# SamsungLabs/fcaf3d

Hardware: AMD Instinct MI355X
Metric: scenes/sec fwd+bwd, ScanNet 100k-pt 2cm voxels, 1/2/4/8 MI355X (higher is better)
Workload: dtype f32

## Files before the change

fcaf3d_amd/_lib.py:

```python
import ctypes
import os
import re
import threading
import time

import torch

_HERE = os.path.dirname(os.path.abspath(__file__))
LIB_PATH = os.environ.get('FC_LIB') or os.path.join(_HERE, 'libfcaf3d_hip.so')
HEADER = os.path.join(os.path.dirname(_HERE), 'include', 'fcaf3d_hip.h')

_SCALARS = {'int': ctypes.c_int, 'int64_t': ctypes.c_int64, 'float': ctypes.c_float,
            'hipStream_t': ctypes.c_void_p}


def parse_header(path=HEADER):
    txt = open(path).read()
    txt = re.sub(r'/\*.*?\*/', '', txt, flags=re.S)
    protos = {}
    for m in re.finditer(r'\b(int64_t|int)\s+(fc_\w+)\s*\(([^)]*)\)\s*;', txt):
        ret, name, args = m.group(1), m.group(2), m.group(3)
        argl = []
        for a in args.split(','):
            a = ' '.join(a.split())
            if not a or a == 'void':
                continue
            if '*' in a:
                argl.append((a.split('*')[-1].strip(), ctypes.c_void_p))
            else:
                ty, nm = a.rsplit(' ', 1)
                argl.append((nm, _SCALARS[ty.replace('const ', '')]))
        protos[name] = (_SCALARS[ret], argl)
    return protos


ABI_VERSION = 8
_lib = None
_protos = None


def lib():
    global _lib, _protos
    if _lib is None:
        if not os.path.exists(LIB_PATH):
            raise RuntimeError(
                f'{LIB_PATH} is missing: build it with `python -m fcaf3d_amd.build` '
                '(hipcc --offload-arch=gfx950).  There is no CPU fallback.')
        l = ctypes.CDLL(LIB_PATH)
        _protos = parse_header()
        for name, (ret, args) in _protos.items():
            fn = getattr(l, name)
            fn.restype = ret
            fn.argtypes = [t for _, t in args]
        if l.fc_abi_version() != ABI_VERSION:
            raise RuntimeError(f'{LIB_PATH} speaks ABI version {l.fc_abi_version()}, this host code was written for {ABI_VERSION}: rebuild '
                               'with `python -m fcaf3d_amd.build`')
        _lib = l
    return _lib


def ptr(t):
    if t is None:
        return None
    assert t.is_contiguous(), 'C ABI takes contiguous buffers'
    return t.data_ptr()


_raw_stream = getattr(torch._C, '_cuda_getCurrentRawStream', None)


def stream():
    if _raw_stream is not None:
        return _raw_stream(torch.cuda.current_device())
    return torch.cuda.current_stream().cuda_stream


_fns = {}


def call(name, *args):
    fn = _fns.get(name)
    if fn is None:
        fn = _fns[name] = getattr(lib(), name)
    rc = fn(*args)
    if rc != 0:
        kind = 'invalid argument' if rc == -1 else 'workspace too small' if rc == -2 else f'hipError {rc}'
        raise RuntimeError(f'{name} failed: {kind}')


_query_cache = {}


def query(name, *args):
    key = (name,) + args
    v = _query_cache.get(key)
    if v is None:
        if len(_query_cache) > 65536:
            _query_cache.clear()
        v = _query_cache[key] = int(getattr(lib(), name)(*args))
    return v


_ws_cache = {}


def workspace(nbytes, device):
    key = (device, stream())
    buf = _ws_cache.get(key)
    if buf is None or buf.numel() < nbytes:
        buf = torch.empty(max(int(nbytes), 1 << 20), dtype=torch.uint8, device=device)
        _ws_cache[key] = buf
    return buf


HOST_WAIT = [0.0]


class _PinnedRing:

    def __init__(self, n=16):
        self.bufs, self.evts, self.i = [None] * n, [None] * n, 0
        self.lock = threading.Lock()

    def upload(self, arr, device):
        with self.lock:
            i = self.i
            self.i = (i + 1) % len(self.bufs)
        if self.evts[i] is not None and not self.evts[i].query():
            t0 = time.perf_counter()
            self.evts[i].synchronize()
            HOST_WAIT[0] += time.perf_counter() - t0
        nb = max(int(arr.nbytes), 1)
        if self.bufs[i] is None or self.bufs[i].numel() < nb:
            self.bufs[i] = torch.empty(max(nb, 4096), dtype=torch.uint8).pin_memory()
        src = torch.from_numpy(arr)
        stage = self.bufs[i][:arr.nbytes].view(src.dtype).reshape(src.shape)
        stage.copy_(src)
        out = stage.to(device, non_blocking=True)
        e = torch.cuda.Event()
        e.record(torch.cuda.current_stream(out.device))
        self.evts[i] = e
        return out


_ring = _PinnedRing()


def upload(arr, device):
    return _ring.upload(arr, device)
```

fcaf3d_amd/csrc/exec.hip:

```cpp
#include "fc_common.h"
#include "../../include/fcaf3d_hip.h"
#include <vector>

namespace {

enum : int64_t {
  OP_STEM_FWD = 1, OP_COL_STATS, OP_NORM_FWD, OP_MAXPOOL_FWD, OP_CONV, OP_BN_FWD, OP_UNION_FWD, OP_HEAD_FWD, OP_RECORD, OP_WAIT,
  OP_HEAD_BWD, OP_WGRAD, OP_BN_BWD, OP_NORM_BWD, OP_MAXPOOL_BWD, OP_STEM_WGRAD, OP_GATHER, OP_ADD, OP_SMALL_GRADS,
  OP_PERMUTE_GENT, OP_HEAD_WFIN, OP_COPY, OP_COL_SUM, OP_ROW_SUM, OP_AMAX, OP_CLEAR
};
constexpr int OPW = 24;
constexpr int MAPW = 20;
constexpr int NSTREAM = 3;
constexpr int MAX_EVENTS = 64;

constexpr int MAX_DEVICES = 16;
hipEvent_t g_events_dev[MAX_DEVICES][MAX_EVENTS];
bool g_events_ready[MAX_DEVICES] = {};
thread_local hipEvent_t* g_events = nullptr;

int ensure_events() {
  int dev = 0;
  FC_HIP(hipGetDevice(&dev));
  if (dev < 0 || dev >= MAX_DEVICES) return FC_EINVAL;
  if (!g_events_ready[dev]) {
    for (int i = 0; i < MAX_EVENTS; ++i) FC_HIP(hipEventCreateWithFlags(&g_events_dev[dev][i], hipEventDisableTiming));
    g_events_ready[dev] = true;
  }
  g_events = g_events_dev[dev];
  return 0;
}

struct ProbeRec { hipEvent_t a, b; int64_t meta[8]; };
std::vector<ProbeRec> g_probe;
std::vector<hipEvent_t> g_probe_pool;

hipEvent_t probe_event() {
  if (!g_probe_pool.empty()) { hipEvent_t e = g_probe_pool.back(); g_probe_pool.pop_back(); return e; }
  hipEvent_t e = nullptr;
  if (hipEventCreate(&e) != hipSuccess) return nullptr;
  return e;
}

inline double as_double(int64_t v) { double d; __builtin_memcpy(&d, &v, 8); return d; }

__global__ void k_add_inplace(float* __restrict__ dst, const float* __restrict__ src, int64_t n4) {
  const int64_t t = (int64_t)blockIdx.x * blockDim.x + threadIdx.x;
  if (t >= n4) return;
  float4 a = reinterpret_cast<float4*>(dst)[t];
  const float4 b = reinterpret_cast<const float4*>(src)[t];
  a.x += b.x; a.y += b.y; a.z += b.z; a.w += b.w;
  reinterpret_cast<float4*>(dst)[t] = a;
}

__global__ void k_small_grads(const long long* __restrict__ desc, int n) {
  const int e = blockIdx.x;
  if (e >= n) return;
  const long long* d = desc + 8 * e;
  const float* src = reinterpret_cast<const float*>(d[0]);
  float* dst = reinterpret_cast<float*>(d[1]);
  const int C = (int)d[2], nseg = (int)d[3];
  const long long stride = d[4];
  for (int c = threadIdx.x; c < C; c += blockDim.x) {
    float s = 0.f;
    for (int k = 0; k < nseg; ++k) s += fc_ld(src + k * stride + c);
    dst[c] = s;
  }
}

__global__ void k_permute_gent(const float* __restrict__ src, float* __restrict__ dst, int Cin, int Cout) {
  const int64_t t = (int64_t)blockIdx.x * blockDim.x + threadIdx.x;
  const int64_t total = (int64_t)8 * Cin * Cout;
  if (t >= total) return;
  const int d = (int)(t % Cout), c = (int)((t / Cout) % Cin), k = (int)(t / ((int64_t)Cout * Cin));
  dst[t] = src[(int64_t)c * 8 * Cout + (int64_t)k * Cout + d];
}

__global__ void k_head_wfin(const float* __restrict__ part, int nl, int R, int ld, int n_reg, int n_cls, float* __restrict__ g_cent,
                            float* __restrict__ g_reg, float* __restrict__ g_cls, const float* __restrict__ bias_part,
                            float* __restrict__ g_bias) {
  const int t = blockIdx.x * blockDim.x + threadIdx.x;
  const int ncol = 1 + n_reg + n_cls;
  if (g_bias && t < n_cls) {
    float b = 0.f;
    for (int l = 0; l < nl; ++l) b += fc_ld(&bias_part[l * n_cls + t]);
    g_bias[t] = b;
  }
  if (t >= R * ncol) return;
  const int r = t / ncol, c = t % ncol;
  float s = 0.f;
  for (int l = 0; l < nl; ++l) s += part[((int64_t)l * R + r) * ld + c];
  if (c == 0) g_cent[r] = s;
  else if (c <= n_reg) g_reg[r * n_reg + c - 1] = s;
  else g_cls[r * n_cls + c - 1 - n_reg] = s;
}

__global__ __launch_bounds__(1024) void k_col_sum(const float* __restrict__ x, int64_t n, int C, float* __restrict__ dst) {
  __shared__ float red[1024];
  const int c = blockIdx.x;
  float a0 = 0.f, a1 = 0.f, a2 = 0.f, a3 = 0.f;
  int64_t r = threadIdx.x;
  for (; r + 3 * 1024 < n; r += 4 * 1024) {
    a0 += x[r * C + c]; a1 += x[(r + 1024) * C + c]; a2 += x[(r + 2048) * C + c]; a3 += x[(r + 3072) * C + c];
  }
  for (; r < n; r += 1024) a0 += x[r * C + c];
  red[threadIdx.x] = (a0 + a1) + (a2 + a3);
  __syncthreads();
  for (int w = 512; w > 0; w >>= 1) {
    if ((int)threadIdx.x < w) red[threadIdx.x] += red[threadIdx.x + w];
    __syncthreads();
  }
  if (threadIdx.x == 0) dst[c] = red[0];
}

struct Ctx {
  const int64_t* ops;
  const int64_t* addr;
  const int64_t* dims;
  const int64_t* maps;
  hipStream_t streams[NSTREAM];
  void* ws[NSTREAM];
  int64_t ws_bytes[NSTREAM];
  int64_t need[NSTREAM];
  bool dry;
  bool probe;
  int64_t bn_small_elems;
  int flags;
};

int run_op_impl(Ctx& c, const int64_t* op);

int run_op(Ctx& c, const int64_t* op) {
  if (c.dry || !c.probe || (op[0] != OP_CONV && op[0] != OP_AMAX)) return run_op_impl(c, op);
  ProbeRec r;
  r.a = probe_event(); r.b = probe_event();
  if (!r.a || !r.b) return run_op_impl(c, op);
  hipStream_t st = c.streams[op[1]];
  const int64_t Cin = op[8], Cout = op[9];
  if (op[0] == OP_AMAX) {
    const int64_t m[8] = {-2, 0, c.dims[op[3]], 0, 0, op[4], 0, 0};
    __builtin_memcpy(r.meta, m, sizeof m);
  } else if (op[4] < 0) {
    const int64_t n = c.dims[op[7]];
    const int64_t m[8] = {-1, op[5], n, n, 1, Cin, Cout, 0};
    __builtin_memcpy(r.meta, m, sizeof m);
  } else {
    const int64_t* mp = c.maps + op[4] * MAPW;
    const bool bwd = op[5] != 0;
    const int64_t m[8] = {op[4], op[5], bwd ? mp[1] : mp[0], bwd ? mp[0] : mp[1], mp[2], Cin, Cout, (mp[19] & (bwd ? 2 : 1)) ? 1 : 0};
    __builtin_memcpy(r.meta, m, sizeof m);
  }
  FC_HIP(hipEventRecord(r.a, st));
  const int rc = run_op_impl(c, op);
  FC_HIP(hipEventRecord(r.b, st));
  g_probe.push_back(r);
  return rc;
}

template <class T>
inline T* P(const Ctx& c, int64_t idx) { return idx < 0 ? nullptr : reinterpret_cast<T*>(c.addr[idx]); }

int64_t stats_blocks_of(const Ctx& c, const int64_t* pop) {
  const int Cin = (int)pop[8], Cout = (int)pop[9];
  const int fl = c.flags | FC_CONV_SPLIT | FC_CONV_IMAGE;
  if (pop[4] < 0) return fc_conv_stats_blocks(c.dims[pop[7]], 1, Cin, Cout, fl, 0);
  const int64_t* m = c.maps + pop[4] * MAPW;
  const bool bwd = pop[5] != 0;
  return fc_conv_stats_blocks(bwd ? m[0] : m[1], (int)m[2], Cin, Cout, fl, (m[19] & (bwd ? 2 : 1)) ? 1 : 0);
}

inline bool want_ws(Ctx& c, int s, int64_t bytes) {
  if (bytes > c.need[s]) c.need[s] = bytes;
  return !c.dry;
}

int run_op_impl(Ctx& c, const int64_t* op) {
  const int s = (int)op[1];
  hipStream_t st = c.streams[s];
#ifdef FC_KO_EXEC
  {
    static const int ko = getenv("FC_KO_OPS") ? atoi(getenv("FC_KO_OPS")) : 0;
    const int64_t o = op[0];
    if (!c.dry && (((ko & 1) && (o == OP_WGRAD || o == OP_STEM_WGRAD)) || ((ko & 2) && o == OP_CONV) ||
                   ((ko & 4) && (o == OP_BN_FWD || o == OP_BN_BWD || o == OP_NORM_FWD || o == OP_NORM_BWD || o == OP_COL_STATS))))
      return 0;
  }
#endif
  switch (op[0]) {
    case OP_STEM_FWD: {
      const int64_t* m = c.maps + op[4] * MAPW;
      if (c.dry) return 0;
      return fc_stem_conv_fwd(P<const float>(c, op[2]), P<const float>(c, op[3]), reinterpret_cast<const int*>(m[3]), P<float>(c, op[5]),
                              P<float>(c, op[6]), m[0], m[1], (int)m[2], st);
    }
    case OP_COL_STATS: {
      const int64_t n = c.dims[op[4]];
      const int C = (int)op[5], nseg = (int)c.dims[op[6]];
      if (!want_ws(c, s, fc_col_stats_ws_bytes(n, C, nseg))) return 0;
      return fc_col_stats(P<const float>(c, op[2]), P<const int>(c, op[3]), op[3] >= 0 ? 4 : 0, n, C, nseg, P<float>(c, op[7]),
                          P<float>(c, op[8]), P<float>(c, op[9]), c.ws[s], c.ws_bytes[s], st);
    }
    case OP_NORM_FWD: {
      if (c.dry) return 0;
      return fc_norm_act_fwd(P<const float>(c, op[2]), P<const int>(c, op[3]), op[3] >= 0 ? 4 : 0, c.dims[op[4]], (int)op[5],
                             P<const float>(c, op[6]), P<const float>(c, op[7]), (float)as_double(op[8]), P<const float>(c, op[9]),
                             P<const float>(c, op[10]), P<const float>(c, op[11]), (int)op[12], P<float>(c, op[13]), st);
    }
    case OP_MAXPOOL_FWD: {
      const int64_t* m = c.maps + op[3] * MAPW;
      if (c.dry) return 0;
      if (op[7] > 0) fc_amax_out_hint(P<unsigned>(c, op[7] - 1));
      return fc_maxpool_fwd(P<const float>(c, op[2]), reinterpret_cast<const int*>(m[3]), m[1], (int)m[2], (int)op[4], P<float>(c, op[5]),
                            P<int>(c, op[6]), st);
    }
    case OP_CONV: {
      const int Cin = (int)op[8], Cout = (int)op[9];
      const int fl = c.flags | FC_CONV_SPLIT | FC_CONV_IMAGE;
      float* stats = (op[10] > 0 && stats_blocks_of(c, op) > 0) ? P<float>(c, op[10] - 1) : nullptr;
      const float* bnx = (stats && op[11] > 0) ? P<const float>(c, op[11] - 1) : nullptr;
      const float *bmean = P<const float>(c, op[12]), *bvar = P<const float>(c, op[13]), *bga = P<const float>(c, op[14]),
                  *bbe = P<const float>(c, op[15]);
      const float beps = (float)as_double(op[16]);
      const int bact = (int)op[17];
      const float* badd = op[18] > 0 ? P<const float>(c, op[18] - 1) : nullptr;
      const float* bny = op[19] > 0 ? P<const float>(c, op[19] - 1) : nullptr;
      const float* in = P<const float>(c, op[2]);
      const float* img = P<const float>(c, op[3]);
      float* out = P<float>(c, op[6]);
      if (!c.dry && op[20] > 0) fc_conv_amax_hint(P<const unsigned>(c, op[20] - 1), nullptr);
      if (op[4] < 0) {
        const int64_t n = c.dims[op[7]];
        if (!want_ws(c, s, fc_conv_fwd_ws_bytes(n, 1, Cin, Cout, fl))) return 0;
        if (bnx)
          return fc_conv_fwd_bn_bwd_stats(in, img, nullptr, nullptr, out, n, n, 1, Cin, Cout, fl, c.ws[s], c.ws_bytes[s], stats, bnx, bmean, bvar,
                                          bga, bbe, beps, bact, badd, bny, st);
        return fc_conv_fwd_stats(in, img, nullptr, nullptr, out, n, n, 1, Cin, Cout, fl, c.ws[s], c.ws_bytes[s], stats, st);
      }
      const int64_t* m = c.maps + op[4] * MAPW;
      const bool bwd = op[5] != 0;
      const int64_t n_in = bwd ? m[1] : m[0], n_out = bwd ? m[0] : m[1];
      const int K = (int)m[2];
      if (m[19] & (bwd ? 2 : 1)) {
        const int b = bwd ? 14 : 9;
        const int *pi = reinterpret_cast<const int*>(m[b]), *pc = reinterpret_cast<const int*>(m[b + 3]),
                  *pp = reinterpret_cast<const int*>(m[b + 2]);
        if (!want_ws(c, s, fc_conv_fwd_pairs_ws_bytes(n_out, K, Cout))) return 0;
        if (bnx)
          return fc_conv_fwd_pairs_tiles_bn_bwd_stats(in, img, pi, pc, pp, out, n_in, n_out, K, Cin, Cout, m[b + 4], fl, c.ws[s], c.ws_bytes[s],
                                                      stats, bnx, bmean, bvar, bga, bbe, beps, bact, badd, bny, st);
        return fc_conv_fwd_pairs_tiles_stats(in, img, pi, pc, pp, out, n_in, n_out, K, Cin, Cout, m[b + 4], fl, c.ws[s], c.ws_bytes[s], stats,
                                             st);
      }
      const int *tab = reinterpret_cast<const int*>(m[bwd ? 7 : 5]), *oidx = reinterpret_cast<const int*>(m[bwd ? 8 : 6]);
      if (!want_ws(c, s, fc_conv_fwd_ws_bytes(n_out, K, Cin, Cout, fl))) return 0;
      if (bnx)
        return fc_conv_fwd_bn_bwd_stats(in, img, tab, oidx, out, n_in, n_out, K, Cin, Cout, fl, c.ws[s], c.ws_bytes[s], stats, bnx, bmean, bvar,
                                        bga, bbe, beps, bact, badd, bny, st);
      return fc_conv_fwd_stats(in, img, tab, oidx, out, n_in, n_out, K, Cin, Cout, fl, c.ws[s], c.ws_bytes[s], stats, st);
    }
    case OP_BN_FWD: {
      const int64_t n = c.dims[op[3]];
      const int C = (int)op[4];
      const float eps = (float)as_double(op[5]), mom = (float)as_double(op[10]);
      if (!op[18]) {
        if (c.dry) return 0;
        if (op[21] > 0) fc_amax_out_hint(P<unsigned>(c, op[21] - 1));
        return fc_norm_act_fwd(P<const float>(c, op[2]), nullptr, 0, n, C, P<const float>(c, op[15]), P<const float>(c, op[16]), eps,
                               P<const float>(c, op[6]), P<const float>(c, op[7]), P<const float>(c, op[8]), (int)op[9], P<float>(c, op[11]),
                               st);
      }
      const float* part = nullptr;
      int64_t nbp = 0;
      if (op[19] > 0) {
        const int64_t* pop = c.ops + (op[19] - 1) * OPW;
        nbp = pop[10] > 0 ? stats_blocks_of(c, pop) : 0;
        if (nbp > 0) part = P<const float>(c, pop[10] - 1);
      }
      if (!want_ws(c, s, fc_bn_train_ws_bytes(n, C))) return 0;
      if (op[21] > 0) fc_amax_out_hint(P<unsigned>(c, op[21] - 1));
      return fc_bn_train_fwd(P<const float>(c, op[2]), n, C, eps, P<const float>(c, op[6]), P<const float>(c, op[7]),
                             P<const float>(c, op[8]), (int)op[9], mom, P<float>(c, op[11]), P<float>(c, op[12]), P<float>(c, op[13]),
                             P<float>(c, op[14]), P<float>(c, op[15]), P<float>(c, op[16]), P<long long>(c, op[17]), part, nbp,
                             op[20] > 0 ? (int)op[20] : 1, c.bn_small_elems, c.ws[s], c.ws_bytes[s], st);
    }
    case OP_UNION_FWD: {
      if (c.dry) return 0;
      const int64_t n_a = c.dims[op[5]], n_b = c.dims[op[6]], n_u = c.dims[op[7]];
      const int C = (int)op[8];
      float* out = P<float>(c, op[9]);
      FC_HIP(hipMemcpyAsync(out, P<const float>(c, op[2]), sizeof(float) * n_a * C, hipMemcpyDeviceToDevice, st));
      if (n_u > n_a) FC_HIP(hipMemsetAsync(out + n_a * C, 0, sizeof(float) * (n_u - n_a) * C, st));
      return fc_scatter_rows_add(P<const float>(c, op[3]), P<const int>(c, op[4]), n_b, C, out, st);
    }
    case OP_HEAD_FWD: {
      if (c.dry) return 0;
      return fc_head_split_fwd(P<const float>(c, op[2]), (int)op[3], P<const float>(c, op[4]), P<const float>(c, op[5]), c.dims[op[6]],
                               (int)op[7], (int)op[8], P<float>(c, op[9]), P<float>(c, op[10]), P<float>(c, op[11]), P<float>(c, op[12]), st);
    }
    case OP_RECORD:
      if (c.dry) return 0;
      FC_HIP(hipEventRecord(g_events[op[2]], st));
      return 0;
    case OP_WAIT:
      if (c.dry) return 0;
      FC_HIP(hipStreamWaitEvent(st, g_events[op[2]], 0));
      return 0;
    case OP_HEAD_BWD: {
      if (op[13] < 0) {
        const int64_t n = c.dims[op[9]];
        if (!want_ws(c, s, fc_head_split_bwd_sums_ws_bytes(n))) return 0;
        if (op[16] > 0) fc_amax_out_hint(P<unsigned>(c, op[16] - 1));
        return fc_head_split_bwd_sums(P<const float>(c, op[2]), (int)op[3], P<const float>(c, op[4]), P<const float>(c, op[5]),
                                      P<const float>(c, op[6]), P<const float>(c, op[7]), P<const float>(c, op[8]), n, (int)op[10],
                                      (int)op[11], P<float>(c, op[12]), P<float>(c, op[15]), P<float>(c, op[14]), c.ws[s],
                                      c.ws_bytes[s], st);
      }
      if (c.dry) return 0;
      return fc_head_split_bwd(P<const float>(c, op[2]), (int)op[3], P<const float>(c, op[4]), P<const float>(c, op[5]),
                               P<const float>(c, op[6]), P<const float>(c, op[7]), P<const float>(c, op[8]), c.dims[op[9]], (int)op[10],
                               (int)op[11], P<float>(c, op[12]), P<float>(c, op[13]), st);
    }
    case OP_WGRAD: {
      const int Cin = (int)op[7], Cout = (int)op[8];
      const int fl = c.flags | FC_CONV_SPLIT;
      if (!c.dry && (op[9] > 0 || op[10] > 0))
        fc_conv_amax_hint(op[9] > 0 ? P<const unsigned>(c, op[9] - 1) : nullptr, op[10] > 0 ? P<const unsigned>(c, op[10] - 1) : nullptr);
      if (op[4] < 0) {
        const int64_t n = c.dims[op[6]];
        if (!want_ws(c, s, fc_conv_wgrad_ws_bytes(n, 1, Cin, Cout, fl))) return 0;
        return fc_conv_wgrad(P<const float>(c, op[2]), P<const float>(c, op[3]), nullptr, nullptr, P<float>(c, op[5]), n, n, 1, Cin, Cout, fl,
                             c.ws[s], c.ws_bytes[s], st);
      }
      const int64_t* m = c.maps + op[4] * MAPW;
      const int K = (int)m[2];
      if (!want_ws(c, s, fc_conv_wgrad_ws_bytes(m[1], K, Cin, Cout, fl))) return 0;
      if ((m[19] & 4) && Cin % 64 == 0 && Cout % 64 == 0)
        return fc_conv_wgrad_pairs(P<const float>(c, op[2]), P<const float>(c, op[3]), reinterpret_cast<const int*>(m[9]),
                                   reinterpret_cast<const int*>(m[10]), reinterpret_cast<const int*>(m[12]), P<float>(c, op[5]), m[0], m[1],
                                   K, Cin, Cout, fl, c.ws[s], c.ws_bytes[s], st);
      return fc_conv_wgrad(P<const float>(c, op[2]), P<const float>(c, op[3]), reinterpret_cast<const int*>(m[3]), nullptr,
                           P<float>(c, op[5]), m[0], m[1], K, Cin, Cout, fl, c.ws[s], c.ws_bytes[s], st);
    }
    case OP_BN_BWD: {
      const int64_t n = c.dims[op[5]];
      const int C = (int)op[6];
      const float eps = (float)as_double(op[10]);
      const float* part = nullptr;
      int64_t nbp = 0;
      if (op[18] > 0) {
        const int64_t* pop = c.ops + (op[18] - 1) * OPW;
        nbp = (pop[10] > 0 && pop[11] > 0) ? stats_blocks_of(c, pop) : 0;
        if (nbp > 0) part = P<const float>(c, pop[10] - 1);
      }
      if (!want_ws(c, s, fc_bn_train_ws_bytes(n, C))) return 0;
      if (op[19] > 0) fc_amax_out_hint(P<unsigned>(c, op[19] - 1));
      return fc_bn_train_bwd(P<const float>(c, op[2]), P<const float>(c, op[3]), P<const float>(c, op[4]),
                             op[17] > 0 ? P<const float>(c, op[17] - 1) : nullptr, n, C, P<const float>(c, op[7]), P<const float>(c, op[8]),
                             P<const float>(c, op[9]), eps, P<const float>(c, op[11]), P<const float>(c, op[12]), (int)op[13],
                             P<float>(c, op[14]), P<float>(c, op[15]), P<float>(c, op[16]), part, nbp, c.bn_small_elems, c.ws[s],
                             c.ws_bytes[s], st);
    }
    case OP_NORM_BWD: {
      const int64_t n = c.dims[op[6]];
      const int C = (int)op[7], nseg = (int)c.dims[op[8]];
      if (!want_ws(c, s, fc_norm_act_bwd_ws_bytes(n, C, nseg))) return 0;
      return fc_norm_act_bwd(P<const float>(c, op[2]), P<const float>(c, op[3]), P<const float>(c, op[4]), P<const int>(c, op[5]),
                             op[5] >= 0 ? 4 : 0, n, C, nseg, P<const float>(c, op[9]), P<const float>(c, op[10]), P<const float>(c, op[11]),
                             (float)as_double(op[12]), P<const float>(c, op[13]), P<const float>(c, op[14]), (int)op[15], P<float>(c, op[16]),
                             P<float>(c, op[17]), P<float>(c, op[18]), c.ws[s], c.ws_bytes[s], st);
    }
    case OP_MAXPOOL_BWD: {
      const int64_t* m = c.maps + op[4] * MAPW;
      if (c.dry) return 0;
      const int C = (int)op[5];
      FC_HIP(hipMemsetAsync(P<float>(c, op[6]), 0, sizeof(float) * m[0] * C, st));
      return fc_maxpool_bwd(P<const float>(c, op[2]), P<const int>(c, op[3]), m[1], C, P<float>(c, op[6]), st);
    }
    case OP_STEM_WGRAD: {
      const int64_t* m = c.maps + op[4] * MAPW;
      if (!want_ws(c, s, fc_stem_conv_wgrad_ws_bytes(m[1], (int)m[2]))) return 0;
      return fc_stem_conv_wgrad(P<const float>(c, op[2]), P<const float>(c, op[3]), P<float>(c, op[5]), m[1], (int)m[2], c.ws[s],
                                c.ws_bytes[s], st);
    }
    case OP_GATHER: {
      if (c.dry) return 0;
      return fc_gather_rows(P<const float>(c, op[2]), P<const int>(c, op[3]), c.dims[op[4]], (int)op[5], P<float>(c, op[6]), st);
    }
    case OP_ADD: {
      if (c.dry) return 0;
      const int64_t n4 = c.dims[op[4]] * op[5] / 4;
      if (n4 > 0) k_add_inplace<<<(unsigned)fc_cdiv(n4, 256), 256, 0, st>>>(P<float>(c, op[2]), P<const float>(c, op[3]), n4);
      FC_CHECK_LAUNCH();
      return 0;
    }
    case OP_SMALL_GRADS: {
      if (c.dry) return 0;
      if (op[4] > 0) k_small_grads<<<(unsigned)op[4], 128, 0, st>>>(P<const long long>(c, op[2]) + 8 * op[3], (int)op[4]);
      FC_CHECK_LAUNCH();
      return 0;
    }
    case OP_COL_SUM: {
      if (c.dry) return 0;
      k_col_sum<<<(unsigned)op[4], 1024, 0, st>>>(P<const float>(c, op[2]), c.dims[op[3]], (int)op[4], P<float>(c, op[5]));
      FC_CHECK_LAUNCH();
      return 0;
    }
    case OP_ROW_SUM: {
      if (c.dry) return 0;
      k_col_sum<<<1, 1024, 0, st>>>(P<const float>(c, op[2]), c.dims[op[3]], 1, P<float>(c, op[4]));
      FC_CHECK_LAUNCH();
      return 0;
    }
    case OP_PERMUTE_GENT: {
      if (c.dry) return 0;
      const int64_t total = 8 * op[4] * op[5];
      k_permute_gent<<<(unsigned)fc_cdiv(total, 256), 256, 0, st>>>(P<const float>(c, op[2]), P<float>(c, op[3]), (int)op[4], (int)op[5]);
      FC_CHECK_LAUNCH();
      return 0;
    }
    case OP_HEAD_WFIN: {
      if (c.dry) return 0;
      const int total = (int)(op[4] * (1 + op[6] + op[7]));
      k_head_wfin<<<(unsigned)fc_cdiv(total, 256), 256, 0, st>>>(P<const float>(c, op[2]), (int)op[3], (int)op[4], (int)op[5], (int)op[6],
                                                                 (int)op[7], P<float>(c, op[8]), P<float>(c, op[9]), P<float>(c, op[10]),
                                                                 P<const float>(c, op[11]), P<float>(c, op[12]));
      FC_CHECK_LAUNCH();
      return 0;
    }
    case OP_AMAX: {
      if (c.dry) return 0;
      return fc_amax(P<const float>(c, op[2]), c.dims[op[3]] * op[4], P<unsigned>(c, op[5]), st);
    }
    case OP_CLEAR: {
      if (c.dry) return 0;
      FC_HIP(hipMemsetAsync(P<void>(c, op[2]), 0, (size_t)op[3], st));
      return 0;
    }
    case OP_COPY: {
      if (c.dry) return 0;
      FC_HIP(hipMemcpyAsync(P<float>(c, op[2]), P<const float>(c, op[3]), sizeof(float) * c.dims[op[4]] * op[5], hipMemcpyDeviceToDevice, st));
      return 0;
    }
    default:
      return FC_EINVAL;
  }
}

}

extern "C" {

int fc_exec_op_words(void) { return OPW; }
int fc_exec_map_words(void) { return MAPW; }

int fc_exec(const int64_t* ops, int64_t op_begin, int64_t op_end, const int64_t* addr, const int64_t* dims, const int64_t* maps,
            const int64_t* streams, const int64_t* ws, const int64_t* ws_bytes, int64_t* ws_need, const int64_t* cfg) {
  if (!ops || op_begin < 0 || op_end < op_begin) return FC_EINVAL;
  int rc = ensure_events();
  if (rc) return rc;
  Ctx c;
  c.ops = ops;
  c.addr = addr; c.dims = dims; c.maps = maps;
  for (int i = 0; i < NSTREAM; ++i) {
    c.streams[i] = reinterpret_cast<hipStream_t>(streams[i]);
    c.ws[i] = reinterpret_cast<void*>(ws[i]);
    c.ws_bytes[i] = ws_bytes[i];
    c.need[i] = 0;
  }
  c.bn_small_elems = cfg[0];
  c.flags = (int)cfg[1];
  c.probe = cfg[2] != 0;
  c.dry = true;
  for (int64_t i = op_begin; i < op_end; ++i) {
    rc = run_op(c, ops + i * OPW);
    if (rc) return rc;
  }
  bool ok = true;
  for (int i = 0; i < NSTREAM; ++i) {
    if (ws_need) ws_need[i] = c.need[i];
    if (c.need[i] > c.ws_bytes[i]) ok = false;
  }
  if (!ok) return FC_EWS;
  if (cfg[3]) return 0;
  c.dry = false;
  for (int64_t i = op_begin; i < op_end; ++i) {
    rc = run_op(c, ops + i * OPW);
    if (rc) return rc;
  }
  return 0;
}

int64_t fc_exec_probe_read(float* ms, int64_t* meta, int64_t cap) {
  const int64_t n = (int64_t)g_probe.size();
  for (int64_t i = 0; i < n; ++i) {
    ProbeRec& r = g_probe[i];
    if (i < cap) {
      float t = 0.f;
      if (hipEventElapsedTime(&t, r.a, r.b) != hipSuccess) t = -1.f;
      ms[i] = t;
      __builtin_memcpy(meta + 8 * i, r.meta, sizeof r.meta);
    }
    g_probe_pool.push_back(r.a);
    g_probe_pool.push_back(r.b);
  }
  g_probe.clear();
  return n;
}

}
```

fcaf3d_amd/csrc/norm.hip:

```cpp
#include "fc_common.h"
#include "../../include/fcaf3d_hip.h"

#define MAXSEG 64
#define MAXBLOCKS 1024

__device__ static inline int seg_of(const int* seg, int seg_stride, int64_t row) {
  return seg ? seg[row * seg_stride] : 0;
}

__device__ static inline void seg_range(const int* seg, int seg_stride, int64_t r0, int64_t r1, int* lo, int* hi,
                                        int* sh ) {
  if (!seg) { *lo = 0; *hi = 0; return; }
  if (threadIdx.x == 0) { sh[0] = 0x7fffffff; sh[1] = -1; }
  __syncthreads();
  int l = 0x7fffffff, h = -1;
  for (int64_t r = r0 + threadIdx.x; r < r1; r += blockDim.x) {
    int s = seg[r * seg_stride];
    l = s < l ? s : l;
    h = s > h ? s : h;
  }
  if (h >= 0) { atomicMin(&sh[0], l); atomicMax(&sh[1], h); }
  __syncthreads();
  *lo = sh[0]; *hi = sh[1];
  __syncthreads();
}

__global__ void k_stats_partial(const float* __restrict__ x, const int* __restrict__ seg, int seg_stride, int64_t n, int C,
                                int nseg, const float* __restrict__ mean, int mode, int64_t rpb, float* __restrict__ part,
                                float* __restrict__ part_cnt) {
  extern __shared__ float sm[];
  __shared__ int srange[2];
  const int c4n = C / 4;
  const int cl = threadIdx.x % c4n, rl = threadIdx.x / c4n;
  const int nrl = blockDim.x / c4n;
  const int64_t r0 = (int64_t)blockIdx.x * rpb;
  int64_t r1 = r0 + rpb;
  if (r1 > n) r1 = n;
  int s_lo, s_hi;
  seg_range(seg, seg_stride, r0, r1, &s_lo, &s_hi, srange);
  const bool chk = seg && s_lo != s_hi;
  for (int s = 0; s < nseg; ++s) {
    float4 acc[4];
    float4 sq = make_float4(0.f, 0.f, 0.f, 0.f);
    float cnt = 0.f;
#pragma unroll
    for (int u = 0; u < 4; ++u) acc[u] = make_float4(0.f, 0.f, 0.f, 0.f);
    if (s >= s_lo && s <= s_hi) {
      float4 mu = make_float4(0.f, 0.f, 0.f, 0.f);
      if (mode == 1) mu = *reinterpret_cast<const float4*>(mean + (int64_t)s * C + cl * 4);
      for (int64_t rb = r0 + rl; rb < r1; rb += 4 * nrl) {
        float4 vv[4];
        bool ok[4];
#pragma unroll
        for (int u = 0; u < 4; ++u) {
          const int64_t r = rb + (int64_t)u * nrl;
          ok[u] = r < r1;
          const int64_t rc = ok[u] ? r : r0;
          if (chk) ok[u] = ok[u] && seg[rc * seg_stride] == s;
          vv[u] = *reinterpret_cast<const float4*>(x + rc * C + cl * 4);
        }
#pragma unroll
        for (int u = 0; u < 4; ++u) {
          if (!ok[u]) continue;
          float4 v = vv[u];
          if (mode == 1) {
            v.x -= mu.x; v.y -= mu.y; v.z -= mu.z; v.w -= mu.w;
            v.x *= v.x; v.y *= v.y; v.z *= v.z; v.w *= v.w;
          }
          if (mode == 2) { sq.x += v.x * v.x; sq.y += v.y * v.y; sq.z += v.z * v.z; sq.w += v.w * v.w; }
          acc[u].x += v.x; acc[u].y += v.y; acc[u].z += v.z; acc[u].w += v.w;
          cnt += 1.f;
        }
      }
    }
    float4 a;
    a.x = (acc[0].x + acc[1].x) + (acc[2].x + acc[3].x);
    a.y = (acc[0].y + acc[1].y) + (acc[2].y + acc[3].y);
    a.z = (acc[0].z + acc[1].z) + (acc[2].z + acc[3].z);
    a.w = (acc[0].w + acc[1].w) + (acc[2].w + acc[3].w);
    __syncthreads();
    *reinterpret_cast<float4*>(&sm[(rl * c4n + cl) * 4]) = a;
    float* smc = sm + nrl * C;
    if (cl == 0) smc[rl] = cnt;
    __syncthreads();
    const int64_t slot = (int64_t)blockIdx.x * nseg + s;
    float* dst = mode == 2 ? part + slot * 2 * C : part + slot * C;
    if (rl == 0) {
      float4 t = make_float4(0.f, 0.f, 0.f, 0.f);
      for (int j = 0; j < nrl; ++j) {
        float4 u = *reinterpret_cast<const float4*>(&sm[(j * c4n + cl) * 4]);
        t.x += u.x; t.y += u.y; t.z += u.z; t.w += u.w;
      }
      *reinterpret_cast<float4*>(dst + cl * 4) = t;
      if (cl == 0 && part_cnt) {
        float c = 0.f;
        for (int j = 0; j < nrl; ++j) c += smc[j];
        part_cnt[slot] = c;
      }
    }
    if (mode == 2) {
      __syncthreads();
      *reinterpret_cast<float4*>(&sm[(rl * c4n + cl) * 4]) = sq;
      __syncthreads();
      if (rl == 0) {
        float4 t = make_float4(0.f, 0.f, 0.f, 0.f);
        for (int j = 0; j < nrl; ++j) {
          float4 u = *reinterpret_cast<const float4*>(&sm[(j * c4n + cl) * 4]);
          t.x += u.x; t.y += u.y; t.z += u.z; t.w += u.w;
        }
        *reinterpret_cast<float4*>(dst + C + cl * 4) = t;
      }
    }
  }
}

__global__ __launch_bounds__(256) void k_seg_meanvar_final(const float* __restrict__ part, const float* __restrict__ part_cnt,
                                                           int64_t nblocks, int nseg, int C, float* __restrict__ mean,
                                                           float* __restrict__ var, float* __restrict__ cnt_out) {
  __shared__ double r1[64][5], r2[64][5], rc[64];
  const int cgroups = (C + 3) / 4;
  const int s = blockIdx.x / cgroups, cg = blockIdx.x % cgroups;
  const int cl = threadIdx.x & 3, j = threadIdx.x >> 2;
  const int c = cg * 4 + cl;
  double a1 = 0., a2 = 0., ac = 0.;
  if (c < C) {
    for (int64_t b = j; b < nblocks; b += 64) {
      const float* src = part + ((b * nseg + s) * 2) * C;
      a1 += fc_ld(&src[c]);
      a2 += fc_ld(&src[C + c]);
      if (cl == 0) ac += fc_ld(&part_cnt[b * nseg + s]);
    }
  }
  r1[j][cl] = a1; r2[j][cl] = a2;
  if (cl == 0) rc[j] = ac;
  __syncthreads();
  if (j == 0 && c < C) {
    double s1 = 0., s2 = 0., n = 0.;
    for (int q = 0; q < 64; ++q) { s1 += r1[q][cl]; s2 += r2[q][cl]; n += rc[q]; }
    double m = 0., v = 0.;
    if (n > 0.) {
      m = s1 / n;
      v = s2 / n - m * m;
      if (v < 0.) v = 0.;
    }
    mean[(int64_t)s * C + c] = (float)m;
    var[(int64_t)s * C + c] = (float)v;
    if (c == 0) cnt_out[s] = (float)n;
  }
}

#define FIN_CB 4
#define FIN_SL 64
__global__ __launch_bounds__(256) void k_stats_final(const float* __restrict__ part, const float* __restrict__ part_cnt,
                                                      int64_t nblocks, int nseg, int C, int mode, float* __restrict__ out,
                                                      float* __restrict__ cnt_io) {
  __shared__ float red[FIN_SL][FIN_CB + 1];
  __shared__ float redc[FIN_SL];
  const int cgroups = (C + FIN_CB - 1) / FIN_CB;
  const int s = blockIdx.x / cgroups, cg = blockIdx.x % cgroups;
  const int cl = threadIdx.x & (FIN_CB - 1), j = threadIdx.x / FIN_CB;
  const int c = cg * FIN_CB + cl;
  float a0 = 0.f, a1 = 0.f, a2 = 0.f, a3 = 0.f;
  if (c < C) {
    int64_t b = j;
    for (; b + 3 * FIN_SL < nblocks; b += 4 * FIN_SL) {
      const float v0 = fc_ld(&part[(b * nseg + s) * C + c]), v1 = fc_ld(&part[((b + FIN_SL) * nseg + s) * C + c]);
      const float v2 = fc_ld(&part[((b + 2 * FIN_SL) * nseg + s) * C + c]), v3 = fc_ld(&part[((b + 3 * FIN_SL) * nseg + s) * C + c]);
      a0 += v0; a1 += v1; a2 += v2; a3 += v3;
    }
    for (; b < nblocks; b += FIN_SL) a0 += fc_ld(&part[(b * nseg + s) * C + c]);
  }
  float acc = (a0 + a1) + (a2 + a3);
  red[j][cl] = acc;
  if (mode == 0 && cl == 0) {
    float cc = 0.f;
    for (int64_t b = j; b < nblocks; b += FIN_SL) cc += fc_ld(&part_cnt[b * nseg + s]);
    redc[j] = cc;
  }
  __syncthreads();
  if (j == 0 && c < C) {
    float t = 0.f;
    for (int q = 0; q < FIN_SL; ++q) t += red[q][cl];
    float cnt = 1.f;
    if (mode == 0) {
      float cc = 0.f;
      for (int q = 0; q < FIN_SL; ++q) cc += redc[q];
      if (c == 0) cnt_io[s] = cc;
      cnt = cc;
    } else if (mode == 1) {
      cnt = cnt_io[s];
    }
    out[(int64_t)s * C + c] = (mode == 2) ? t : (cnt > 0.f ? t / cnt : 0.f);
  }
}

__device__ static inline float act_fwd(float v, int act) {
  if (act == 1) return v > 0.f ? v : 0.f;
  if (act == 2) return v > 0.f ? v : expm1f(v);
  return v;
}
__device__ static inline float act_bwd_from_y(float y, int act) {
  if (act == 1) return y > 0.f ? 1.f : 0.f;
  if (act == 2) return y > 0.f ? 1.f : y + 1.f;
  return 1.f;
}

__device__ static inline float bn_pre(float v, float mu, float is, float g, float b) { return fmaf((v - mu) * is, g, b); }
__device__ static inline float act_bwd_from_pre(float p, int act) {
  if (act == 1) return p > 0.f ? 1.f : 0.f;
  if (act == 2) return p > 0.f ? 1.f : expf(p);
  return 1.f;
}

thread_local unsigned* t_fc_amax_out = nullptr;

__global__ void k_norm_act_fwd(const float* __restrict__ x, const int* __restrict__ seg, int seg_stride, int64_t n, int C,
                               const float* __restrict__ mean, const float* __restrict__ var, float eps,
                               const float* __restrict__ gamma, const float* __restrict__ beta,
                               const float* __restrict__ residual, int act, float* __restrict__ y, unsigned* __restrict__ amax_out) {
  int64_t t = (int64_t)blockIdx.x * blockDim.x + threadIdx.x;
  const int c4n = C / 4;
  unsigned am = 0u;
  if (t < n * c4n) {
  int64_t r = t / c4n;
  int c = (int)(t % c4n) * 4;
  int s = seg_of(seg, seg_stride, r);
  float4 v = *reinterpret_cast<const float4*>(x + r * C + c);
  float4 mu = *reinterpret_cast<const float4*>(mean + (int64_t)s * C + c);
  float4 va = *reinterpret_cast<const float4*>(var + (int64_t)s * C + c);
  float4 g = gamma ? *reinterpret_cast<const float4*>(gamma + c) : make_float4(1.f, 1.f, 1.f, 1.f);
  float4 b = beta ? *reinterpret_cast<const float4*>(beta + c) : make_float4(0.f, 0.f, 0.f, 0.f);
  float4 o;
  o.x = bn_pre(v.x, mu.x, 1.f / sqrtf(va.x + eps), g.x, b.x);
  o.y = bn_pre(v.y, mu.y, 1.f / sqrtf(va.y + eps), g.y, b.y);
  o.z = bn_pre(v.z, mu.z, 1.f / sqrtf(va.z + eps), g.z, b.z);
  o.w = bn_pre(v.w, mu.w, 1.f / sqrtf(va.w + eps), g.w, b.w);
  if (residual) {
    float4 rs = *reinterpret_cast<const float4*>(residual + r * C + c);
    o.x += rs.x; o.y += rs.y; o.z += rs.z; o.w += rs.w;
  }
  o.x = act_fwd(o.x, act); o.y = act_fwd(o.y, act); o.z = act_fwd(o.z, act); o.w = act_fwd(o.w, act);
  *reinterpret_cast<float4*>(y + r * C + c) = o;
  amax_fold(am, o.x); amax_fold(am, o.y); amax_fold(am, o.z); amax_fold(am, o.w);
  }
  if (amax_out) amax_commit(am, amax_out);
}

__global__ void k_norm_bwd_partial(const float* __restrict__ x, const float* __restrict__ y, const float* __restrict__ gy,
                                   const float* __restrict__ gy2, const int* __restrict__ seg, int seg_stride, int64_t n, int C, int nseg,
                                   const float* __restrict__ mean, const float* __restrict__ var, float eps, int act,
                                   const float* __restrict__ gamma, const float* __restrict__ beta,
                                   int64_t rpb, float* __restrict__ part) {
  extern __shared__ float sm[];
  __shared__ int srange[2];
  const int c4n = C / 4;
  const int cl = threadIdx.x % c4n, rl = threadIdx.x / c4n;
  const int nrl = blockDim.x / c4n;
  const int64_t r0 = (int64_t)blockIdx.x * rpb;
  int64_t r1 = r0 + rpb;
  if (r1 > n) r1 = n;
  int s_lo, s_hi;
  seg_range(seg, seg_stride, r0, r1, &s_lo, &s_hi, srange);
  const bool chk = seg && s_lo != s_hi;
  for (int s = 0; s < nseg; ++s) {
    float4 a1[4], a2[4];
#pragma unroll
    for (int u = 0; u < 4; ++u) { a1[u] = make_float4(0.f, 0.f, 0.f, 0.f); a2[u] = a1[u]; }
    if (s >= s_lo && s <= s_hi) {
      float4 mu = *reinterpret_cast<const float4*>(mean + (int64_t)s * C + cl * 4);
      float4 va = *reinterpret_cast<const float4*>(var + (int64_t)s * C + cl * 4);
      float4 is = make_float4(1.f / sqrtf(va.x + eps), 1.f / sqrtf(va.y + eps), 1.f / sqrtf(va.z + eps),
                              1.f / sqrtf(va.w + eps));
      const float4 gm = gamma ? *reinterpret_cast<const float4*>(gamma + cl * 4) : make_float4(1.f, 1.f, 1.f, 1.f);
      const float4 bt = beta ? *reinterpret_cast<const float4*>(beta + cl * 4) : make_float4(0.f, 0.f, 0.f, 0.f);
      const bool from_y = act && y;
      for (int64_t rb = r0 + rl; rb < r1; rb += 4 * nrl) {
        float4 xv[4], gv[4], yv[4], g2[4];
        bool ok[4];
#pragma unroll
        for (int u = 0; u < 4; ++u) {
          const int64_t r = rb + (int64_t)u * nrl;
          ok[u] = r < r1;
          const int64_t rc = ok[u] ? r : r0;
          if (chk) ok[u] = ok[u] && seg[rc * seg_stride] == s;
          xv[u] = *reinterpret_cast<const float4*>(x + rc * C + cl * 4);
          gv[u] = *reinterpret_cast<const float4*>(gy + rc * C + cl * 4);
          if (gy2) g2[u] = *reinterpret_cast<const float4*>(gy2 + rc * C + cl * 4);
          if (from_y) yv[u] = *reinterpret_cast<const float4*>(y + rc * C + cl * 4);
        }
#pragma unroll
        for (int u = 0; u < 4; ++u) {
          if (!ok[u]) continue;
          float4 g = gv[u];
          if (gy2) { g.x += g2[u].x; g.y += g2[u].y; g.z += g2[u].z; g.w += g2[u].w; }
          if (from_y) {
            g.x *= act_bwd_from_y(yv[u].x, act); g.y *= act_bwd_from_y(yv[u].y, act);
            g.z *= act_bwd_from_y(yv[u].z, act); g.w *= act_bwd_from_y(yv[u].w, act);
          } else if (act) {
            g.x *= act_bwd_from_pre(bn_pre(xv[u].x, mu.x, is.x, gm.x, bt.x), act);
            g.y *= act_bwd_from_pre(bn_pre(xv[u].y, mu.y, is.y, gm.y, bt.y), act);
            g.z *= act_bwd_from_pre(bn_pre(xv[u].z, mu.z, is.z, gm.z, bt.z), act);
            g.w *= act_bwd_from_pre(bn_pre(xv[u].w, mu.w, is.w, gm.w, bt.w), act);
          }
          a1[u].x += g.x; a1[u].y += g.y; a1[u].z += g.z; a1[u].w += g.w;
          a2[u].x += g.x * (xv[u].x - mu.x) * is.x; a2[u].y += g.y * (xv[u].y - mu.y) * is.y;
          a2[u].z += g.z * (xv[u].z - mu.z) * is.z; a2[u].w += g.w * (xv[u].w - mu.w) * is.w;
        }
      }
    }
    float4 b1 = make_float4((a1[0].x + a1[1].x) + (a1[2].x + a1[3].x), (a1[0].y + a1[1].y) + (a1[2].y + a1[3].y),
                            (a1[0].z + a1[1].z) + (a1[2].z + a1[3].z), (a1[0].w + a1[1].w) + (a1[2].w + a1[3].w));
    float4 b2 = make_float4((a2[0].x + a2[1].x) + (a2[2].x + a2[3].x), (a2[0].y + a2[1].y) + (a2[2].y + a2[3].y),
                            (a2[0].z + a2[1].z) + (a2[2].z + a2[3].z), (a2[0].w + a2[1].w) + (a2[2].w + a2[3].w));
    __syncthreads();
    *reinterpret_cast<float4*>(&sm[(rl * 2 + 0) * C + cl * 4]) = b1;
    *reinterpret_cast<float4*>(&sm[(rl * 2 + 1) * C + cl * 4]) = b2;
    __syncthreads();
    if (rl == 0) {
      float4 t1 = make_float4(0.f, 0.f, 0.f, 0.f), t2 = t1;
      for (int j = 0; j < nrl; ++j) {
        float4 u = *reinterpret_cast<const float4*>(&sm[(j * 2 + 0) * C + cl * 4]);
        float4 w = *reinterpret_cast<const float4*>(&sm[(j * 2 + 1) * C + cl * 4]);
        t1.x += u.x; t1.y += u.y; t1.z += u.z; t1.w += u.w;
        t2.x += w.x; t2.y += w.y; t2.z += w.z; t2.w += w.w;
      }
      float* dst = part + (((int64_t)blockIdx.x * nseg + s) * 2) * C;
      *reinterpret_cast<float4*>(dst + cl * 4) = t1;
      *reinterpret_cast<float4*>(dst + C + cl * 4) = t2;
    }
  }
}

__global__ void k_norm_bwd_apply(const float* __restrict__ x, const float* __restrict__ y, const float* __restrict__ gy,
                                 const float* __restrict__ gy2, const int* __restrict__ seg, int seg_stride, int64_t n, int C,
                                 const float* __restrict__ mean, const float* __restrict__ var, float eps,
                                 const float* __restrict__ gamma, const float* __restrict__ beta,
                                 const float* __restrict__ sums ,
                                 const float* __restrict__ cnt, int act, float* __restrict__ gx, float* __restrict__ gres,
                                 unsigned* __restrict__ amax_out) {
  int64_t t = (int64_t)blockIdx.x * blockDim.x + threadIdx.x;
  const int c4n = C / 4;
  unsigned am = 0u;
  if (t < n * c4n) {
  int64_t r = t / c4n;
  int c = (int)(t % c4n) * 4;
  int s = seg_of(seg, seg_stride, r);
  float inv_n = 1.f / cnt[s];
  float xv[4], gv[4], muv[4], vav[4], gam[4], bet[4] = {0.f, 0.f, 0.f, 0.f}, s1[4], s2[4], yv[4], o[4], gr[4];
  *reinterpret_cast<float4*>(xv) = *reinterpret_cast<const float4*>(x + r * C + c);
  *reinterpret_cast<float4*>(gv) = *reinterpret_cast<const float4*>(gy + r * C + c);
  if (gy2) {
    const float4 t2 = *reinterpret_cast<const float4*>(gy2 + r * C + c);
    gv[0] += t2.x; gv[1] += t2.y; gv[2] += t2.z; gv[3] += t2.w;
  }
  *reinterpret_cast<float4*>(muv) = *reinterpret_cast<const float4*>(mean + (int64_t)s * C + c);
  *reinterpret_cast<float4*>(vav) = *reinterpret_cast<const float4*>(var + (int64_t)s * C + c);
  *reinterpret_cast<float4*>(s1) = *reinterpret_cast<const float4*>(sums + ((int64_t)s * 2) * C + c);
  *reinterpret_cast<float4*>(s2) = *reinterpret_cast<const float4*>(sums + ((int64_t)s * 2 + 1) * C + c);
  if (gamma) *reinterpret_cast<float4*>(gam) = *reinterpret_cast<const float4*>(gamma + c);
  else gam[0] = gam[1] = gam[2] = gam[3] = 1.f;
  const bool from_y = act && y;
  if (from_y) *reinterpret_cast<float4*>(yv) = *reinterpret_cast<const float4*>(y + r * C + c);
  if (beta) *reinterpret_cast<float4*>(bet) = *reinterpret_cast<const float4*>(beta + c);
#pragma unroll
  for (int j = 0; j < 4; ++j) {
    float g = gv[j];
    float is = 1.f / sqrtf(vav[j] + eps);
    if (from_y) g *= act_bwd_from_y(yv[j], act);
    else if (act) g *= act_bwd_from_pre(bn_pre(xv[j], muv[j], is, gam[j], bet[j]), act);
    float xh = (xv[j] - muv[j]) * is;
    gr[j] = g;
    o[j] = gam[j] * is * (g - s1[j] * inv_n - xh * s2[j] * inv_n);
  }
  *reinterpret_cast<float4*>(gx + r * C + c) = *reinterpret_cast<float4*>(o);
  if (gres) *reinterpret_cast<float4*>(gres + r * C + c) = *reinterpret_cast<float4*>(gr);
#pragma unroll
  for (int j = 0; j < 4; ++j) amax_fold(am, o[j]);
  }
  if (amax_out) amax_commit(am, amax_out);
}

__global__ void k_maxpool_fwd(const float* __restrict__ in, const int* __restrict__ nbr, int64_t n_out, int K, int C,
                              float* __restrict__ out, int* __restrict__ argrow) {
  int64_t t = (int64_t)blockIdx.x * blockDim.x + threadIdx.x;
  if (t >= n_out * C) return;
  int64_t o = t / C;
  int c = (int)(t % C);
  float best = -INFINITY;
  int arg = -1;
  for (int k = 0; k < K; ++k) {
    int i = nbr[(int64_t)k * n_out + o];
    if (i < 0) continue;
    float v = in[(int64_t)i * C + c];
    if (arg < 0 || v > best) { best = v; arg = i; }
  }
  out[t] = arg < 0 ? 0.f : best;
  argrow[t] = arg;
}

__global__ void k_maxpool8_fwd(const float* __restrict__ in, const int* __restrict__ nbr, int64_t n_out, int C,
                               float* __restrict__ out, int* __restrict__ argrow, unsigned* __restrict__ amax_out) {
  const int c4n = C / 4;
  int64_t t = (int64_t)blockIdx.x * blockDim.x + threadIdx.x;
  unsigned am = 0u;
  if (t < n_out * c4n) {
  const int64_t o = t / c4n;
  const int c = (int)(t % c4n) * 4;
  int idx[8];
#pragma unroll
  for (int k = 0; k < 8; ++k) idx[k] = nbr[(int64_t)k * n_out + o];
  float4 v[8];
#pragma unroll
  for (int k = 0; k < 8; ++k) {
    const int i = idx[k] < 0 ? 0 : idx[k];
    v[k] = *reinterpret_cast<const float4*>(in + (int64_t)i * C + c);
  }
  float best[4] = {-INFINITY, -INFINITY, -INFINITY, -INFINITY};
  int arg[4] = {-1, -1, -1, -1};
#pragma unroll
  for (int k = 0; k < 8; ++k) {
    if (idx[k] < 0) continue;
    const float e[4] = {v[k].x, v[k].y, v[k].z, v[k].w};
#pragma unroll
    for (int j = 0; j < 4; ++j)
      if (arg[j] < 0 || e[j] > best[j]) { best[j] = e[j]; arg[j] = idx[k]; }
  }
  float4 ob = make_float4(arg[0] < 0 ? 0.f : best[0], arg[1] < 0 ? 0.f : best[1], arg[2] < 0 ? 0.f : best[2], arg[3] < 0 ? 0.f : best[3]);
  *reinterpret_cast<float4*>(out + o * C + c) = ob;
  *reinterpret_cast<int4*>(argrow + o * C + c) = make_int4(arg[0], arg[1], arg[2], arg[3]);
  amax_fold(am, ob.x); amax_fold(am, ob.y); amax_fold(am, ob.z); amax_fold(am, ob.w);
  }
  if (amax_out) amax_commit(am, amax_out);
}

__global__ void k_maxpool_bwd(const float* __restrict__ gout, const int* __restrict__ argrow, int64_t n_out, int C,
                              float* __restrict__ gin) {
  int64_t t = (int64_t)blockIdx.x * blockDim.x + threadIdx.x;
  if (t >= n_out * C) return;
  int i = argrow[t];
  if (i >= 0) gin[(int64_t)i * C + (t % C)] = gout[t];
}

__global__ void k_gather_rows(const float* __restrict__ src, const int* __restrict__ idx, int64_t n, int C,
                              float* __restrict__ dst) {
  int64_t t = (int64_t)blockIdx.x * blockDim.x + threadIdx.x;
  if (t >= n * C) return;
  int64_t r = t / C;
  int i = idx[r];
  dst[t] = i >= 0 ? src[(int64_t)i * C + (t % C)] : 0.f;
}

__global__ void k_scatter_rows_add(const float* __restrict__ src, const int* __restrict__ idx, int64_t n, int C,
                                   float* __restrict__ dst) {
  int64_t t = (int64_t)blockIdx.x * blockDim.x + threadIdx.x;
  if (t >= n * C) return;
  int64_t r = t / C;
  int i = idx[r];
  if (i >= 0) dst[(int64_t)i * C + (t % C)] += src[t];
}

#define BN1_MAXB 64

__global__ void k_bn1_partial(const float* __restrict__ x, int64_t n, int C, int64_t rpb, float* __restrict__ part) {
  extern __shared__ float sm[];
  const int c4n = C / 4;
  const int cl = threadIdx.x % c4n, rl = threadIdx.x / c4n;
  const int nrl = blockDim.x / c4n;
  const int64_t r0 = (int64_t)blockIdx.x * rpb;
  int64_t r1 = r0 + rpb;
  if (r1 > n) r1 = n;
  const float4 sh = *reinterpret_cast<const float4*>(x + cl * 4);
  float4 a1 = make_float4(0.f, 0.f, 0.f, 0.f), a2 = a1;
  for (int64_t rb = r0 + rl; rb < r1; rb += 4 * (int64_t)nrl) {
    float4 v[4];
#pragma unroll
    for (int u = 0; u < 4; ++u) {
      const int64_t r = rb + (int64_t)u * nrl;
      v[u] = r < r1 ? *reinterpret_cast<const float4*>(x + r * C + cl * 4) : sh;
    }
#pragma unroll
    for (int u = 0; u < 4; ++u) {
      v[u].x -= sh.x; v[u].y -= sh.y; v[u].z -= sh.z; v[u].w -= sh.w;
      a1.x += v[u].x; a1.y += v[u].y; a1.z += v[u].z; a1.w += v[u].w;
      a2.x += v[u].x * v[u].x; a2.y += v[u].y * v[u].y; a2.z += v[u].z * v[u].z; a2.w += v[u].w * v[u].w;
    }
  }
  *reinterpret_cast<float4*>(&sm[(rl * 2 + 0) * C + cl * 4]) = a1;
  *reinterpret_cast<float4*>(&sm[(rl * 2 + 1) * C + cl * 4]) = a2;
  __syncthreads();
  if (rl == 0) {
    float4 t1 = make_float4(0.f, 0.f, 0.f, 0.f), t2 = t1;
    for (int j = 0; j < nrl; ++j) {
      float4 u = *reinterpret_cast<const float4*>(&sm[(j * 2 + 0) * C + cl * 4]);
      float4 w = *reinterpret_cast<const float4*>(&sm[(j * 2 + 1) * C + cl * 4]);
      t1.x += u.x; t1.y += u.y; t1.z += u.z; t1.w += u.w;
      t2.x += w.x; t2.y += w.y; t2.z += w.z; t2.w += w.w;
    }
    float* dst = part + ((int64_t)blockIdx.x * 2) * C;
    *reinterpret_cast<float4*>(dst + cl * 4) = t1;
    *reinterpret_cast<float4*>(dst + C + cl * 4) = t2;
  }
}

__device__ static inline void bn1_reduce_parts(const float* __restrict__ part, int nb, int C, int cl, int rl, int nrl,
                                               float* sm , float4* s1, float4* s2, int CG, int c0) {
  float4 a1 = make_float4(0.f, 0.f, 0.f, 0.f), a2 = a1;
  const bool past_l1 = (int64_t)nb * C * 8 <= 32768;
  for (int b = rl; b < nb; b += nrl) {
    const float* src = part + ((int64_t)b * 2) * C + c0;
    float4 u = past_l1 ? fc_ld4(src + cl * 4) : *reinterpret_cast<const float4*>(src + cl * 4);
    float4 w = past_l1 ? fc_ld4(src + C + cl * 4) : *reinterpret_cast<const float4*>(src + C + cl * 4);
    a1.x += u.x; a1.y += u.y; a1.z += u.z; a1.w += u.w;
    a2.x += w.x; a2.y += w.y; a2.z += w.z; a2.w += w.w;
  }
  *reinterpret_cast<float4*>(&sm[(rl * 2 + 0) * CG + cl * 4]) = a1;
  *reinterpret_cast<float4*>(&sm[(rl * 2 + 1) * CG + cl * 4]) = a2;
  __syncthreads();
  float4 t1 = make_float4(0.f, 0.f, 0.f, 0.f), t2 = t1;
  for (int j = 0; j < nrl; ++j) {
    float4 u = *reinterpret_cast<const float4*>(&sm[(j * 2 + 0) * CG + cl * 4]);
    float4 w = *reinterpret_cast<const float4*>(&sm[(j * 2 + 1) * CG + cl * 4]);
    t1.x += u.x; t1.y += u.y; t1.z += u.z; t1.w += u.w;
    t2.x += w.x; t2.y += w.y; t2.z += w.z; t2.w += w.w;
  }
  *s1 = t1; *s2 = t2;
}

__global__ void k_bn1_apply(const float* __restrict__ x, int64_t n, int C, int64_t rpb, const float* __restrict__ part, int nb,
                            float eps, const float* __restrict__ gamma, const float* __restrict__ beta,
                            const float* __restrict__ residual, int act, float momentum, float* __restrict__ y,
                            float* __restrict__ mean_out, float* __restrict__ var_out, float* __restrict__ cnt_out,
                            float* __restrict__ rmean, float* __restrict__ rvar, long long* __restrict__ nbt) {
  extern __shared__ float sm[];
  const int c4n = C / 4;
  const int cl = threadIdx.x % c4n, rl = threadIdx.x / c4n;
  const int nrl = blockDim.x / c4n;
  float4 s1, s2;
  bn1_reduce_parts(part, nb, C, cl, rl, nrl, sm, &s1, &s2, C, 0);
  const float4 sh = *reinterpret_cast<const float4*>(x + cl * 4);
  const float inv_n = 1.f / (float)n;
  float d[4] = {s1.x * inv_n, s1.y * inv_n, s1.z * inv_n, s1.w * inv_n};
  float q[4] = {s2.x * inv_n, s2.y * inv_n, s2.z * inv_n, s2.w * inv_n};
  float shv[4] = {sh.x, sh.y, sh.z, sh.w};
  float mu[4], va[4], is[4], g[4], bt[4];
#pragma unroll
  for (int j = 0; j < 4; ++j) {
    mu[j] = shv[j] + d[j];
    va[j] = fmaxf(q[j] - d[j] * d[j], 0.f);
    is[j] = 1.f / sqrtf(va[j] + eps);
    g[j] = gamma ? gamma[cl * 4 + j] : 1.f;
    bt[j] = beta ? beta[cl * 4 + j] : 0.f;
  }
  if (blockIdx.x == 0 && rl == 0) {
    *reinterpret_cast<float4*>(mean_out + cl * 4) = make_float4(mu[0], mu[1], mu[2], mu[3]);
    *reinterpret_cast<float4*>(var_out + cl * 4) = make_float4(va[0], va[1], va[2], va[3]);
    if (cl == 0) { cnt_out[0] = (float)n; if (nbt) nbt[0] += 1; }
    if (rmean) {
      float unbias = (float)n / fmaxf((float)n - 1.f, 1.f);
#pragma unroll
      for (int j = 0; j < 4; ++j) {
        rmean[cl * 4 + j] = (1.f - momentum) * rmean[cl * 4 + j] + momentum * mu[j];
        rvar[cl * 4 + j] = (1.f - momentum) * rvar[cl * 4 + j] + momentum * va[j] * unbias;
      }
    }
  }
  const int64_t r0 = (int64_t)blockIdx.x * rpb;
  int64_t r1 = r0 + rpb;
  if (r1 > n) r1 = n;
  for (int64_t rb = r0 + rl; rb < r1; rb += 4 * (int64_t)nrl) {
    float v[4][4], rs[4][4];
#pragma unroll
    for (int u = 0; u < 4; ++u) {
      const int64_t r = rb + (int64_t)u * nrl;
      const int64_t rc = r < r1 ? r : r0;
      *reinterpret_cast<float4*>(v[u]) = *reinterpret_cast<const float4*>(x + rc * C + cl * 4);
      if (residual) *reinterpret_cast<float4*>(rs[u]) = *reinterpret_cast<const float4*>(residual + rc * C + cl * 4);
    }
#pragma unroll
    for (int u = 0; u < 4; ++u) {
      const int64_t r = rb + (int64_t)u * nrl;
      if (r >= r1) continue;
      float o[4];
#pragma unroll
      for (int j = 0; j < 4; ++j) {
        o[j] = bn_pre(v[u][j], mu[j], is[j], g[j], bt[j]);
        if (residual) o[j] += rs[u][j];
        o[j] = act_fwd(o[j], act);
      }
      *reinterpret_cast<float4*>(y + r * C + cl * 4) = *reinterpret_cast<float4*>(o);
    }
  }
}

__global__ __launch_bounds__(1024) void k_bn_finalize(const float* __restrict__ part, int nb, int C, int64_t n,
                                                      const float* __restrict__ x, float momentum, float* __restrict__ mean,
                                                      float* __restrict__ var, float* __restrict__ cnt,
                                                      float* __restrict__ rmean, float* __restrict__ rvar,
                                                      long long* __restrict__ nbt) {
  __shared__ float r1[16][65], r2[16][65];
  const int c = blockIdx.x * 64 + (threadIdx.x & 63), j = threadIdx.x >> 6;
  float a1 = 0.f, a2 = 0.f;
  if (c < C) {
    float p1[4] = {0.f, 0.f, 0.f, 0.f}, p2[4] = {0.f, 0.f, 0.f, 0.f};
    int b = j;
    for (; b + 48 < nb; b += 64) {
      float u[4], w[4];
#pragma unroll
      for (int q = 0; q < 4; ++q) {
        u[q] = fc_ld(&part[((int64_t)(b + 16 * q) * 2) * C + c]);
        w[q] = fc_ld(&part[((int64_t)(b + 16 * q) * 2 + 1) * C + c]);
      }
#pragma unroll
      for (int q = 0; q < 4; ++q) { p1[q] += u[q]; p2[q] += w[q]; }
    }
    for (; b < nb; b += 16) {
      p1[0] += fc_ld(&part[((int64_t)b * 2) * C + c]);
      p2[0] += fc_ld(&part[((int64_t)b * 2 + 1) * C + c]);
    }
    a1 = (p1[0] + p1[1]) + (p1[2] + p1[3]);
    a2 = (p2[0] + p2[1]) + (p2[2] + p2[3]);
  }
  r1[j][threadIdx.x & 63] = a1;
  r2[j][threadIdx.x & 63] = a2;
  __syncthreads();
  if (j == 0 && c < C) {
    float s1 = 0.f, s2 = 0.f;
    for (int q = 0; q < 16; ++q) { s1 += r1[q][threadIdx.x & 63]; s2 += r2[q][threadIdx.x & 63]; }
    const float inv_n = 1.f / (float)n;
    float d = s1 * inv_n;
    float mu = x[c] + d;
    float va = fmaxf(s2 * inv_n - d * d, 0.f);
    mean[c] = mu;
    var[c] = va;
    if (c == 0) { cnt[0] = (float)n; if (nbt) nbt[0] += 1; }
    if (rmean) {
      float unbias = (float)n / fmaxf((float)n - 1.f, 1.f);
      rmean[c] = (1.f - momentum) * rmean[c] + momentum * mu;
      rvar[c] = (1.f - momentum) * rvar[c] + momentum * va * unbias;
    }
  }
}

__global__ void k_bn1_bwd_apply(const float* __restrict__ x, const float* __restrict__ y, const float* __restrict__ gy,
                                const float* __restrict__ gy2, int64_t n, int C, int64_t rpb, const float* __restrict__ part, int nb,
                                const float* __restrict__ mean, const float* __restrict__ var, float eps,
                                const float* __restrict__ gamma, const float* __restrict__ beta, int act,
                                float* __restrict__ gx, float* __restrict__ gres, float* __restrict__ sums , int CG,
                                unsigned* __restrict__ amax_out) {
  extern __shared__ float sm[];
  const int c0 = blockIdx.y * CG;
  x += c0; gy += c0; gx += c0; mean += c0; var += c0;
  if (y) y += c0;
  if (gy2) gy2 += c0;
  if (gres) gres += c0;
  if (gamma) gamma += c0;
  if (beta) beta += c0;
  const int c4n = CG / 4;
  const int cl = threadIdx.x % c4n, rl = threadIdx.x / c4n;
  const int nrl = blockDim.x / c4n;
  float4 t1, t2;
  bn1_reduce_parts(part, nb, C, cl, rl, nrl, sm, &t1, &t2, CG, c0);
  if (blockIdx.x == 0 && rl == 0) {
    *reinterpret_cast<float4*>(sums + c0 + cl * 4) = t1;
    *reinterpret_cast<float4*>(sums + C + c0 + cl * 4) = t2;
  }
  const float inv_n = 1.f / (float)n;
  float s1[4] = {t1.x * inv_n, t1.y * inv_n, t1.z * inv_n, t1.w * inv_n};
  float s2[4] = {t2.x * inv_n, t2.y * inv_n, t2.z * inv_n, t2.w * inv_n};
  float mu[4], is[4], g[4], bt[4];
#pragma unroll
  for (int j = 0; j < 4; ++j) {
    mu[j] = mean[cl * 4 + j];
    is[j] = 1.f / sqrtf(var[cl * 4 + j] + eps);
    g[j] = gamma ? gamma[cl * 4 + j] : 1.f;
    bt[j] = beta ? beta[cl * 4 + j] : 0.f;
  }
  const bool from_y = act && y;
  const int64_t r0 = (int64_t)blockIdx.x * rpb;
  int64_t r1 = r0 + rpb;
  if (r1 > n) r1 = n;
  unsigned am = 0u;
  for (int64_t rb = r0 + rl; rb < r1; rb += 4 * (int64_t)nrl) {
    float xv[4][4], gv[4][4], yv[4][4];
#pragma unroll
    for (int u = 0; u < 4; ++u) {
      const int64_t r = rb + (int64_t)u * nrl;
      const int64_t rc = r < r1 ? r : r0;
      *reinterpret_cast<float4*>(xv[u]) = *reinterpret_cast<const float4*>(x + rc * C + cl * 4);
      *reinterpret_cast<float4*>(gv[u]) = *reinterpret_cast<const float4*>(gy + rc * C + cl * 4);
      if (gy2) {
        const float4 t2 = *reinterpret_cast<const float4*>(gy2 + rc * C + cl * 4);
        gv[u][0] += t2.x; gv[u][1] += t2.y; gv[u][2] += t2.z; gv[u][3] += t2.w;
      }
      if (from_y) *reinterpret_cast<float4*>(yv[u]) = *reinterpret_cast<const float4*>(y + rc * C + cl * 4);
    }
#pragma unroll
    for (int u = 0; u < 4; ++u) {
      const int64_t r = rb + (int64_t)u * nrl;
      if (r >= r1) continue;
      float o[4], gr[4];
#pragma unroll
      for (int j = 0; j < 4; ++j) {
        float gg = gv[u][j];
        if (from_y) gg *= act_bwd_from_y(yv[u][j], act);
        else if (act) gg *= act_bwd_from_pre(bn_pre(xv[u][j], mu[j], is[j], g[j], bt[j]), act);
        float xh = (xv[u][j] - mu[j]) * is[j];
        gr[j] = gg;
        o[j] = g[j] * is[j] * (gg - s1[j] - xh * s2[j]);
      }
      *reinterpret_cast<float4*>(gx + r * C + cl * 4) = *reinterpret_cast<float4*>(o);
      if (gres) *reinterpret_cast<float4*>(gres + r * C + cl * 4) = *reinterpret_cast<float4*>(gr);
#pragma unroll
      for (int j = 0; j < 4; ++j) amax_fold(am, o[j]);
    }
  }
  if (amax_out) amax_commit(am, amax_out);
}

__device__ static inline void bn2_stats(double s1, double s2, int64_t n, float* mu, float* va) {
  const double m = s1 / (double)n;
  double v = s2 / (double)n - m * m;
  if (v < 0.0) v = 0.0;
  *mu = (float)m;
  *va = (float)v;
}

__global__ void k_bn2_apply(const float* __restrict__ x, int64_t n, int C, int64_t rpb, const float* __restrict__ part, int nb, int G,
                            float eps, const float* __restrict__ gamma, const float* __restrict__ beta,
                            const float* __restrict__ residual, int act, float momentum, float* __restrict__ y,
                            float* __restrict__ mean_out, float* __restrict__ var_out, float* __restrict__ cnt_out,
                            float* __restrict__ rmean, float* __restrict__ rvar, long long* __restrict__ nbt, int CG,
                            unsigned* __restrict__ amax_out) {
  extern __shared__ double smd[];
  const int c0 = blockIdx.y * CG;
  x += c0; y += c0; part += c0; mean_out += c0; var_out += c0;
  if (residual) residual += c0;
  if (gamma) gamma += c0;
  if (beta) beta += c0;
  if (rmean) { rmean += c0; rvar += c0; }
  const int c4n = CG / 4;
  const int cl = threadIdx.x % c4n, rl = threadIdx.x / c4n;
  const int nrl = blockDim.x / c4n;
  double a1[4] = {0., 0., 0., 0.}, a2[4] = {0., 0., 0., 0.};
  const int GC = G * C;
  for (int t = rl; t < nb * G; t += nrl) {
    const int b = t / G, g = t % G;
    const float* src = part + ((int64_t)b * 2) * GC + g * C + cl * 4;
    const float4 u = fc_ld4(src), w = fc_ld4(src + GC);
    a1[0] += u.x; a1[1] += u.y; a1[2] += u.z; a1[3] += u.w;
    a2[0] += w.x; a2[1] += w.y; a2[2] += w.z; a2[3] += w.w;
  }
#pragma unroll
  for (int j = 0; j < 4; ++j) {
    smd[(rl * 2 + 0) * CG + cl * 4 + j] = a1[j];
    smd[(rl * 2 + 1) * CG + cl * 4 + j] = a2[j];
  }
  __syncthreads();
  float mu[4], va[4], is[4], g[4], bt[4];
#pragma unroll
  for (int j = 0; j < 4; ++j) {
    double t1 = 0., t2 = 0.;
    for (int q = 0; q < nrl; ++q) { t1 += smd[(q * 2 + 0) * CG + cl * 4 + j]; t2 += smd[(q * 2 + 1) * CG + cl * 4 + j]; }
    bn2_stats(t1, t2, n, &mu[j], &va[j]);
    is[j] = 1.f / sqrtf(va[j] + eps);
    g[j] = gamma ? gamma[cl * 4 + j] : 1.f;
    bt[j] = beta ? beta[cl * 4 + j] : 0.f;
  }
  if (blockIdx.x == 0 && rl == 0) {
    *reinterpret_cast<float4*>(mean_out + cl * 4) = make_float4(mu[0], mu[1], mu[2], mu[3]);
    *reinterpret_cast<float4*>(var_out + cl * 4) = make_float4(va[0], va[1], va[2], va[3]);
    if (cl == 0 && blockIdx.y == 0) { cnt_out[0] = (float)n; if (nbt) nbt[0] += 1; }
    if (rmean) {
      float unbias = (float)n / fmaxf((float)n - 1.f, 1.f);
#pragma unroll
      for (int j = 0; j < 4; ++j) {
        rmean[cl * 4 + j] = (1.f - momentum) * rmean[cl * 4 + j] + momentum * mu[j];
        rvar[cl * 4 + j] = (1.f - momentum) * rvar[cl * 4 + j] + momentum * va[j] * unbias;
      }
    }
  }
  const int64_t r0 = (int64_t)blockIdx.x * rpb;
  int64_t r1 = r0 + rpb;
  if (r1 > n) r1 = n;
  unsigned am = 0u;
  for (int64_t rb = r0 + rl; rb < r1; rb += 4 * (int64_t)nrl) {
    float v[4][4], rs[4][4];
#pragma unroll
    for (int u = 0; u < 4; ++u) {
      const int64_t r = rb + (int64_t)u * nrl;
      const int64_t rc = r < r1 ? r : r0;
      *reinterpret_cast<float4*>(v[u]) = *reinterpret_cast<const float4*>(x + rc * C + cl * 4);
      if (residual) *reinterpret_cast<float4*>(rs[u]) = *reinterpret_cast<const float4*>(residual + rc * C + cl * 4);
    }
#pragma unroll
    for (int u = 0; u < 4; ++u) {
      const int64_t r = rb + (int64_t)u * nrl;
      if (r >= r1) continue;
      float o[4];
#pragma unroll
      for (int j = 0; j < 4; ++j) {
        o[j] = bn_pre(v[u][j], mu[j], is[j], g[j], bt[j]);
        if (residual) o[j] += rs[u][j];
        o[j] = act_fwd(o[j], act);
      }
      *reinterpret_cast<float4*>(y + r * C + cl * 4) = *reinterpret_cast<float4*>(o);
#pragma unroll
      for (int j = 0; j < 4; ++j) amax_fold(am, o[j]);
    }
  }
  if (amax_out) amax_commit(am, amax_out);
}

__global__ __launch_bounds__(256) void k_bn2_finalize(const float* __restrict__ part, int nb, int C, int G, int64_t n, float momentum,
                                                       float* __restrict__ mean, float* __restrict__ var, float* __restrict__ cnt,
                                                       float* __restrict__ rmean, float* __restrict__ rvar,
                                                       long long* __restrict__ nbt) {
  __shared__ double r1[FIN_SL][FIN_CB + 1], r2[FIN_SL][FIN_CB + 1];
  const int cl = threadIdx.x & (FIN_CB - 1), j = threadIdx.x / FIN_CB;
  const int c = blockIdx.x * FIN_CB + cl;
  const int GC = G * C;
  double a1 = 0., a2 = 0.;
  if (c < C) {
    double p1[4] = {0., 0., 0., 0.}, p2[4] = {0., 0., 0., 0.};
    const int total = nb * G;
    int t = j;
    for (; t + 3 * FIN_SL < total; t += 4 * FIN_SL) {
      float u[4], w[4];
#pragma unroll
      for (int q = 0; q < 4; ++q) {
        const int tt = t + FIN_SL * q, b = tt / G, g = tt % G;
        u[q] = fc_ld(&part[((int64_t)b * 2) * GC + g * C + c]);
        w[q] = fc_ld(&part[((int64_t)b * 2 + 1) * GC + g * C + c]);
      }
#pragma unroll
      for (int q = 0; q < 4; ++q) { p1[q] += u[q]; p2[q] += w[q]; }
    }
    for (; t < total; t += FIN_SL) {
      const int b = t / G, g = t % G;
      p1[0] += fc_ld(&part[((int64_t)b * 2) * GC + g * C + c]);
      p2[0] += fc_ld(&part[((int64_t)b * 2 + 1) * GC + g * C + c]);
    }
    a1 = (p1[0] + p1[1]) + (p1[2] + p1[3]);
    a2 = (p2[0] + p2[1]) + (p2[2] + p2[3]);
  }
  r1[j][cl] = a1;
  r2[j][cl] = a2;
  __syncthreads();
  if (j == 0 && c < C) {
    double s1 = 0., s2 = 0.;
    for (int q = 0; q < FIN_SL; ++q) { s1 += r1[q][cl]; s2 += r2[q][cl]; }
    float mu, va;
    bn2_stats(s1, s2, n, &mu, &va);
    mean[c] = mu;
    var[c] = va;
    if (c == 0) { cnt[0] = (float)n; if (nbt) nbt[0] += 1; }
    if (rmean) {
      float unbias = (float)n / fmaxf((float)n - 1.f, 1.f);
      rmean[c] = (1.f - momentum) * rmean[c] + momentum * mu;
      rvar[c] = (1.f - momentum) * rvar[c] + momentum * va * unbias;
    }
  }
}

extern "C" {

static int stats_geometry(int C, int* threads, size_t* smem_fwd, size_t* smem_bwd) {
  if (C < 4 || C % 4 || C > 1024) return FC_EINVAL;
  int c4n = C / 4;
  int nrl = 256 / c4n;
  if (nrl < 1) nrl = 1;
  if (nrl > 16) nrl = 16;
  *threads = nrl * c4n;
  *smem_fwd = (size_t)(nrl * C + nrl) * sizeof(float);
  *smem_bwd = (size_t)(nrl * 2 * C) * sizeof(float);
  return FC_OK;
}

static void red_plan(int64_t n, int64_t* nb, int64_t* rpb) {
  int64_t m = n > 0 ? n : 1;
  int64_t g = fc_cdiv(m, 64);
  if (g > MAXBLOCKS) g = MAXBLOCKS;
  *rpb = fc_cdiv(m, g);
  *nb = fc_cdiv(m, *rpb);
}

int64_t fc_col_stats_ws_bytes(int64_t n, int C, int nseg) {
  int64_t nb, rpb;
  red_plan(n, &nb, &rpb);
  return nb * nseg * (2 * (int64_t)C + 1) * (int64_t)sizeof(float);
}

int fc_col_stats(const float* x, const int* seg, int seg_stride, int64_t n, int C, int nseg, float* mean, float* var,
                 float* cnt, void* ws, int64_t ws_bytes, hipStream_t stream) {
  if (n < 0 || nseg < 1 || nseg > MAXSEG) return FC_EINVAL;
  int threads; size_t sf, sb;
  if (stats_geometry(C, &threads, &sf, &sb)) return FC_EINVAL;
  if (ws_bytes < fc_col_stats_ws_bytes(n, C, nseg)) return FC_EWS;
  int64_t nb, rpb;
  red_plan(n, &nb, &rpb);
  float* part = (float*)ws;
  float* part_cnt = part + nb * nseg * 2 * C;
  if (n == 0) {
    FC_HIP(hipMemsetAsync(mean, 0, sizeof(float) * nseg * C, stream));
    FC_HIP(hipMemsetAsync(var, 0, sizeof(float) * nseg * C, stream));
    FC_HIP(hipMemsetAsync(cnt, 0, sizeof(float) * nseg, stream));
    return FC_OK;
  }
  k_stats_partial<<<(unsigned)nb, threads, sf, stream>>>(x, seg, seg_stride, n, C, nseg, nullptr, 2, rpb, part, part_cnt);
  FC_CHECK_LAUNCH();
  k_seg_meanvar_final<<<(unsigned)(nseg * ((C + 3) / 4)), 256, 0, stream>>>(part, part_cnt, nb, nseg, C, mean, var, cnt);
  FC_CHECK_LAUNCH();
  return FC_OK;
}

int fc_seg_col_sums(const float* x, const int* seg, int seg_stride, int64_t n, int C, int nseg, float* out, void* ws,
                    int64_t ws_bytes, hipStream_t stream) {
  if (n < 0 || nseg < 1 || nseg > MAXSEG) return FC_EINVAL;
  int threads; size_t sf, sb;
  if (stats_geometry(C, &threads, &sf, &sb)) return FC_EINVAL;
  if (ws_bytes < fc_col_stats_ws_bytes(n, C, nseg)) return FC_EWS;
  if (n == 0) {
    FC_HIP(hipMemsetAsync(out, 0, sizeof(float) * nseg * C, stream));
    return FC_OK;
  }
  int64_t nb, rpb;
  red_plan(n, &nb, &rpb);
  float* part = (float*)ws;
  k_stats_partial<<<(unsigned)nb, threads, sf, stream>>>(x, seg, seg_stride, n, C, nseg, nullptr, 0, rpb, part, nullptr);
  FC_CHECK_LAUNCH();
  k_stats_final<<<(unsigned)(nseg * ((C + FIN_CB - 1) / FIN_CB)), FIN_CB * FIN_SL, 0, stream>>>(part, nullptr, nb, nseg, C, 2, out, nullptr);
  FC_CHECK_LAUNCH();
  return FC_OK;
}

__global__ void k_bn_running(const float* __restrict__ mean, const float* __restrict__ var, const float* __restrict__ cnt,
                             float momentum, int C, float* __restrict__ rmean, float* __restrict__ rvar,
                             long long* __restrict__ nbt) {
  int c = blockIdx.x * blockDim.x + threadIdx.x;
  if (c == 0 && nbt) nbt[0] += 1;
  if (c >= C) return;
  float n = cnt[0];
  float unbias = n / fmaxf(n - 1.f, 1.f);
  rmean[c] = (1.f - momentum) * rmean[c] + momentum * mean[c];
  rvar[c] = (1.f - momentum) * rvar[c] + momentum * var[c] * unbias;
}

int fc_bn_running_update(const float* mean, const float* var, const float* cnt, float momentum, int C, float* running_mean,
                         float* running_var, long long* num_batches_tracked, hipStream_t stream) {
  if (C < 1) return FC_EINVAL;
  k_bn_running<<<(unsigned)fc_cdiv(C, 256), 256, 0, stream>>>(mean, var, cnt, momentum, C, running_mean, running_var,
                                                             num_batches_tracked);
  FC_CHECK_LAUNCH();
  return FC_OK;
}

static void bn1_plan(int64_t n, int64_t* nb, int64_t* rpb) {
  int64_t m = n > 0 ? n : 1;
  int64_t g = fc_cdiv(m, 64);
  if (g > BN1_MAXB) g = BN1_MAXB;
  *rpb = fc_cdiv(m, g);
  *nb = fc_cdiv(m, *rpb);
}

int64_t fc_bn_small_ws_bytes(int C) { return (int64_t)BN1_MAXB * 2 * C * (int64_t)sizeof(float); }

int64_t fc_bn_stats_ws_bytes(int64_t n, int C) {
  int64_t nb, rpb;
  red_plan(n, &nb, &rpb);
  return nb * 2 * (int64_t)C * (int64_t)sizeof(float);
}

int fc_bn_stats_train(const float* x, int64_t n, int C, float momentum, float* mean, float* var, float* cnt,
                      float* running_mean, float* running_var, long long* num_batches_tracked, void* ws,
                      int64_t ws_bytes, hipStream_t stream) {
  if (n < 1) return FC_EINVAL;
  int threads; size_t sf, sb;
  if (stats_geometry(C, &threads, &sf, &sb)) return FC_EINVAL;
  if (ws_bytes < fc_bn_stats_ws_bytes(n, C)) return FC_EWS;
  int64_t nb, rpb;
  red_plan(n, &nb, &rpb);
  float* part = (float*)ws;
  k_bn1_partial<<<(unsigned)nb, threads, sb, stream>>>(x, n, C, rpb, part);
  FC_CHECK_LAUNCH();
  k_bn_finalize<<<(unsigned)((C + 63) / 64), 1024, 0, stream>>>(part, (int)nb, C, n, x, momentum, mean, var, cnt, running_mean,
                                                                running_var, num_batches_tracked);
  FC_CHECK_LAUNCH();
  return FC_OK;
}

int fc_bn_act_train_fwd(const float* x, int64_t n, int C, float eps, const float* gamma, const float* beta,
                        const float* residual, int act, float momentum, float* y, float* mean, float* var, float* cnt,
                        float* running_mean, float* running_var, long long* num_batches_tracked, void* ws,
                        int64_t ws_bytes, hipStream_t stream) {
  if (n < 1 || act < 0 || act > 2) return FC_EINVAL;
  int threads; size_t sf, sb;
  if (stats_geometry(C, &threads, &sf, &sb)) return FC_EINVAL;
  if (ws_bytes < fc_bn_small_ws_bytes(C)) return FC_EWS;
  int64_t nb, rpb;
  bn1_plan(n, &nb, &rpb);
  float* part = (float*)ws;
  k_bn1_partial<<<(unsigned)nb, threads, sb, stream>>>(x, n, C, rpb, part);
  FC_CHECK_LAUNCH();
  k_bn1_apply<<<(unsigned)nb, threads, sb, stream>>>(x, n, C, rpb, part, (int)nb, eps, gamma, beta, residual, act, momentum, y,
                                                    mean, var, cnt, running_mean, running_var, num_batches_tracked);
  FC_CHECK_LAUNCH();
  return FC_OK;
}

int fc_bn_act_train_bwd(const float* x, const float* y, const float* gy, int64_t n, int C, const float* mean,
                        const float* var, float eps, const float* gamma, const float* beta, int act, float* gx, float* gres,
                        float* sums, void* ws, int64_t ws_bytes, hipStream_t stream) {
  if (n < 1 || act < 0 || act > 2) return FC_EINVAL;
  int threads; size_t sf, sb;
  if (stats_geometry(C, &threads, &sf, &sb)) return FC_EINVAL;
  if (ws_bytes < fc_bn_small_ws_bytes(C)) return FC_EWS;
  int64_t nb, rpb;
  bn1_plan(n, &nb, &rpb);
  float* part = (float*)ws;
  k_norm_bwd_partial<<<(unsigned)nb, threads, sb, stream>>>(x, y, gy, nullptr, nullptr, 0, n, C, 1, mean, var, eps, act, gamma, beta, rpb, part);
  FC_CHECK_LAUNCH();
  unsigned* ao = take_amax_out();
  k_bn1_bwd_apply<<<(unsigned)nb, threads, sb, stream>>>(x, y, gy, nullptr, n, C, rpb, part, (int)nb, mean, var, eps, gamma, beta, act, gx,
                                                        gres, sums, C, ao);
  FC_CHECK_LAUNCH();
  return FC_OK;
}

int fc_norm_act_fwd(const float* x, const int* seg, int seg_stride, int64_t n, int C, const float* mean, const float* var,
                    float eps, const float* gamma, const float* beta, const float* residual, int act, float* y,
                    hipStream_t stream) {
  unsigned* ao = take_amax_out();
  if (n < 0 || C < 4 || C % 4 || act < 0 || act > 2) return FC_EINVAL;
  if (n == 0) return FC_OK;
  k_norm_act_fwd<<<(unsigned)fc_cdiv(n * (C / 4), 256), 256, 0, stream>>>(x, seg, seg_stride, n, C, mean, var, eps, gamma,
                                                                         beta, residual, act, y, ao);
  FC_CHECK_LAUNCH();
  return FC_OK;
}

int64_t fc_norm_act_bwd_ws_bytes(int64_t n, int C, int nseg) {
  int64_t nb, rpb;
  red_plan(n, &nb, &rpb);
  return nb * nseg * 2 * (int64_t)C * (int64_t)sizeof(float);
}

int fc_norm_act_bwd(const float* x, const float* y, const float* gy, const int* seg, int seg_stride, int64_t n, int C,
                    int nseg, const float* mean, const float* var, const float* cnt, float eps, const float* gamma,
                    const float* beta, int act, float* gx, float* gres, float* sums, void* ws, int64_t ws_bytes,
                    hipStream_t stream) {
  unsigned* ao = take_amax_out();
  if (n < 0 || nseg < 1 || nseg > MAXSEG || act < 0 || act > 2) return FC_EINVAL;
  int threads; size_t sf, sb;
  if (stats_geometry(C, &threads, &sf, &sb)) return FC_EINVAL;
  if (ws_bytes < fc_norm_act_bwd_ws_bytes(n, C, nseg)) return FC_EWS;
  if (n == 0) {
    FC_HIP(hipMemsetAsync(sums, 0, sizeof(float) * nseg * 2 * C, stream));
    return FC_OK;
  }
  int64_t nb, rpb;
  red_plan(n, &nb, &rpb);
  float* part = (float*)ws;
  k_norm_bwd_partial<<<(unsigned)nb, threads, sb, stream>>>(x, y, gy, nullptr, seg, seg_stride, n, C, nseg, mean, var, eps, act, gamma,
                                                          beta, rpb, part);
  FC_CHECK_LAUNCH();
  k_stats_final<<<(unsigned)(nseg * ((2 * C + FIN_CB - 1) / FIN_CB)), FIN_CB * FIN_SL, 0, stream>>>(part, nullptr, nb, nseg, 2 * C, 2, sums, nullptr);
  FC_CHECK_LAUNCH();
  k_norm_bwd_apply<<<(unsigned)fc_cdiv(n * (C / 4), 256), 256, 0, stream>>>(x, y, gy, nullptr, seg, seg_stride, n, C, mean, var, eps,
                                                                           gamma, beta, sums, cnt, act, gx, gres, ao);
  FC_CHECK_LAUNCH();
  return FC_OK;
}

static int ap_window(int64_t n, int C) { return (C >= 128 && C % 64 == 0 && fc_cdiv(n > 0 ? n : 1, 64) * (C / 64) <= 1024 && fc_cdiv(n > 0 ? n : 1, 64) < 128) ? 64 : C; }
static void ap_plan(int64_t n, int64_t* nb, int64_t* rpb) {
  int64_t m = n > 0 ? n : 1;
  int64_t g = fc_cdiv(m, 64);
  if (g > 256) g = 256;
  *rpb = fc_cdiv(m, g);
  *nb = fc_cdiv(m, *rpb);
}

int64_t fc_bn_train_ws_bytes(int64_t n, int C) {
  const int64_t a = fc_bn_stats_ws_bytes(n, C), b = fc_norm_act_bwd_ws_bytes(n, C, 1), c = fc_bn_small_ws_bytes(C);
  return a > b ? (a > c ? a : c) : (b > c ? b : c);
}

int fc_bn_train_fwd(const float* x, int64_t n, int C, float eps, const float* gamma, const float* beta, const float* residual,
                    int act, float momentum, float* y, float* mean, float* var, float* cnt, float* running_mean,
                    float* running_var, long long* num_batches_tracked, const float* part, int64_t nb_part, int groups,
                    int64_t small_elems, void* ws, int64_t ws_bytes, hipStream_t stream) {
  unsigned* ao = take_amax_out();
  if (n < 1 || act < 0 || act > 2) return FC_EINVAL;
  if (!part) {
    if (n * C <= small_elems) {
      int rc = fc_bn_act_train_fwd(x, n, C, eps, gamma, beta, residual, act, momentum, y, mean, var, cnt, running_mean, running_var,
                                   num_batches_tracked, ws, ws_bytes, stream);
      if (rc == FC_OK && ao) rc = fc_amax(y, n * (int64_t)C, ao, stream);
      return rc;
    }
    int rc = fc_bn_stats_train(x, n, C, momentum, mean, var, cnt, running_mean, running_var, num_batches_tracked, ws, ws_bytes, stream);
    if (rc) return rc;
    t_fc_amax_out = ao;
    return fc_norm_act_fwd(x, nullptr, 0, n, C, mean, var, eps, gamma, beta, residual, act, y, stream);
  }
  int threads; size_t sf, sb;
  if (stats_geometry(C, &threads, &sf, &sb)) return FC_EINVAL;
  if (nb_part < 1 || nb_part > 0x7fffffff / 64 || groups < 1 || groups > 64) return FC_EINVAL;
  if (nb_part <= BN1_MAXB) {
    int64_t nb, rpb;
    ap_plan(n, &nb, &rpb);
    const int CG = ap_window(n, C);
    if (CG != C && stats_geometry(CG, &threads, &sf, &sb)) return FC_EINVAL;
    const size_t smem = (size_t)(threads / (CG / 4)) * 2 * CG * sizeof(double);
    k_bn2_apply<<<dim3((unsigned)nb, C / CG), threads, smem, stream>>>(x, n, C, rpb, part, (int)nb_part, groups, eps, gamma, beta, residual, act,
                                                        momentum, y, mean, var, cnt, running_mean, running_var, num_batches_tracked, CG, ao);
    FC_CHECK_LAUNCH();
    return FC_OK;
  }
  k_bn2_finalize<<<(unsigned)((C + FIN_CB - 1) / FIN_CB), FIN_CB * FIN_SL, 0, stream>>>(part, (int)nb_part, C, groups, n, momentum, mean, var, cnt,
                                                                 running_mean, running_var, num_batches_tracked);
  FC_CHECK_LAUNCH();
  t_fc_amax_out = ao;
  return fc_norm_act_fwd(x, nullptr, 0, n, C, mean, var, eps, gamma, beta, residual, act, y, stream);
}

int fc_bn_train_bwd(const float* x, const float* y, const float* gy, const float* gy2, int64_t n, int C, const float* mean,
                    const float* var, const float* cnt, float eps, const float* gamma, const float* beta, int act, float* gx,
                    float* gres, float* sums, const float* part, int64_t nb_part, int64_t small_elems, void* ws, int64_t ws_bytes,
                    hipStream_t stream) {
  unsigned* ao = take_amax_out();
  if (n < 1 || act < 0 || act > 2) return FC_EINVAL;
  int threads; size_t sf, sb;
  if (stats_geometry(C, &threads, &sf, &sb)) return FC_EINVAL;
  const float* p = part;
  int64_t np = nb_part;
  if (!p) {
    const bool small = n * C <= small_elems;
    if (ws_bytes < (small ? fc_bn_small_ws_bytes(C) : fc_norm_act_bwd_ws_bytes(n, C, 1))) return FC_EWS;
    int64_t rpb;
    if (small) bn1_plan(n, &np, &rpb); else red_plan(n, &np, &rpb);
    k_norm_bwd_partial<<<(unsigned)np, threads, sb, stream>>>(x, y, gy, gy2, nullptr, 0, n, C, 1, mean, var, eps, act, gamma, beta, rpb,
                                                            (float*)ws);
    FC_CHECK_LAUNCH();
    p = (const float*)ws;
  }
  if (np < 1) return FC_EINVAL;
  if (np <= BN1_MAXB) {
    int64_t nb, rpb;
    if (!part) bn1_plan(n, &nb, &rpb); else ap_plan(n, &nb, &rpb);
    const int CG = ap_window(n, C);
    if (CG != C && stats_geometry(CG, &threads, &sf, &sb)) return FC_EINVAL;
    k_bn1_bwd_apply<<<dim3((unsigned)nb, C / CG), threads, sb, stream>>>(x, y, gy, gy2, n, C, rpb, p, (int)np, mean, var, eps, gamma, beta, act, gx,
                                                          gres, sums, CG, ao);
    FC_CHECK_LAUNCH();
    return FC_OK;
  }
  k_stats_final<<<(unsigned)((2 * C + FIN_CB - 1) / FIN_CB), FIN_CB * FIN_SL, 0, stream>>>(p, nullptr, np, 1, 2 * C, 2, sums, nullptr);
  FC_CHECK_LAUNCH();
  k_norm_bwd_apply<<<(unsigned)fc_cdiv(n * (C / 4), 256), 256, 0, stream>>>(x, y, gy, gy2, nullptr, 0, n, C, mean, var, eps, gamma, beta,
                                                                           sums, cnt, act, gx, gres, ao);
  FC_CHECK_LAUNCH();
  return FC_OK;
}

int fc_amax_out_hint(unsigned* amax_word) {
  t_fc_amax_out = amax_word;
  return FC_OK;
}

int fc_maxpool_fwd(const float* in, const int* nbr, int64_t n_out, int K, int C, float* out, int* argrow,
                   hipStream_t stream) {
  unsigned* ao = take_amax_out();
  if (n_out < 0 || K < 1 || C < 1) return FC_EINVAL;
  if (n_out == 0) return FC_OK;
  if (K == 8 && C % 4 == 0) k_maxpool8_fwd<<<(unsigned)fc_cdiv(n_out * (C / 4), 256), 256, 0, stream>>>(in, nbr, n_out, C, out, argrow, ao);
  else k_maxpool_fwd<<<(unsigned)fc_cdiv(n_out * C, 256), 256, 0, stream>>>(in, nbr, n_out, K, C, out, argrow);
  FC_CHECK_LAUNCH();
  if (ao && !(K == 8 && C % 4 == 0)) return fc_amax(out, n_out * (int64_t)C, ao, stream);
  return FC_OK;
}

int fc_maxpool_bwd(const float* gout, const int* argrow, int64_t n_out, int C, float* gin, hipStream_t stream) {
  if (n_out < 0 || C < 1) return FC_EINVAL;
  if (n_out == 0) return FC_OK;
  k_maxpool_bwd<<<(unsigned)fc_cdiv(n_out * C, 256), 256, 0, stream>>>(gout, argrow, n_out, C, gin);
  FC_CHECK_LAUNCH();
  return FC_OK;
}

int fc_gather_rows(const float* src, const int* idx, int64_t n, int C, float* dst, hipStream_t stream) {
  if (n < 0 || C < 1) return FC_EINVAL;
  if (n == 0) return FC_OK;
  k_gather_rows<<<(unsigned)fc_cdiv(n * C, 256), 256, 0, stream>>>(src, idx, n, C, dst);
  FC_CHECK_LAUNCH();
  return FC_OK;
}

int fc_scatter_rows_add(const float* src, const int* idx, int64_t n, int C, float* dst, hipStream_t stream) {
  if (n < 0 || C < 1) return FC_EINVAL;
  if (n == 0) return FC_OK;
  k_scatter_rows_add<<<(unsigned)fc_cdiv(n * C, 256), 256, 0, stream>>>(src, idx, n, C, dst);
  FC_CHECK_LAUNCH();
  return FC_OK;
}

}
```

fcaf3d_amd/executor.py:

```python
import os
import struct

import numpy as np
import torch

from . import _lib as L
from . import functional as Fn
from . import nn as MEnn

ENABLED = os.environ.get('FC_EXEC', '1') != '0'
PROBE = None
TRUSTED = None
KEEP_STATE = False

(OP_STEM_FWD, OP_COL_STATS, OP_NORM_FWD, OP_MAXPOOL_FWD, OP_CONV, OP_BN_FWD, OP_UNION_FWD, OP_HEAD_FWD, OP_RECORD, OP_WAIT,
 OP_HEAD_BWD, OP_WGRAD, OP_BN_BWD, OP_NORM_BWD, OP_MAXPOOL_BWD, OP_STEM_WGRAD, OP_GATHER, OP_ADD, OP_SMALL_GRADS,
 OP_PERMUTE_GENT, OP_HEAD_WFIN, OP_COPY, OP_COL_SUM, OP_ROW_SUM, OP_AMAX, OP_CLEAR) = range(1, 27)
OPW, MAPW = 24, 20
ALIGN = 256
S_MAIN, S_HEAD, S_WGRAD = 0, 1, 2
EV_FORK, EV_HEAD_DONE, EV_W0, EV_W1, EV_WEND, EV_BWD0, EV_HB = 0, 8, 9, 10, 11, 12, 16


def _f(x):
    return struct.unpack('<q', struct.pack('<d', float(x)))[0]


def supported(det):
    bb, nh = det.backbone, det.neck_with_head
    if not (ENABLED and Fn.X6 and not (Fn.FLAGS & Fn.CONV_FMA) and Fn.STEM_COL and Fn.DGRAD_WT):
        return False
    if getattr(bb.BLOCK, 'expansion', 1) != 1 or det.spatial_sort:
        return False
    if 1 + nh.n_reg_outs + nh.n_classes > 64 or bb.conv1[0].in_channels != 3:
        return False
    return type(nh).forward_single is _FORWARD_SINGLE and type(nh).forward is _NECK_FORWARD


_FORWARD_SINGLE = _NECK_FORWARD = None


class NetProgram:
    def __init__(self, det, training, wgrad_async, head_overlap, tail0=False):
        self.det = det
        self.tail0 = tail0
        self.training = training
        self.wgrad_async = wgrad_async and training
        bb, nh = det.backbone, det.neck_with_head
        self.nl = min(bb.n_outs, 4)
        self.head_overlap = head_overlap and self.nl > 1
        self.dev = next(det.parameters()).device
        self.ops_f, self.ops_b = [], []
        self.n_addr = 0
        self.static = []
        self.arena = {'f': [], 'b': []}
        self.alias = []
        self.dyn = {}
        self.dim_names = {}
        self.map_names = {}
        self.grad_refs = []
        self.keep = []
        self._params = [p for p in det.parameters() if p.requires_grad]
        self._goff, off = {}, 0
        flat = getattr(self._params[0], '_fc_flat', None)
        self.flat = flat[0] if flat is not None else None
        for p in self._params:
            if self.flat is not None:
                assert p._fc_flat[0] is self.flat
                self._goff[id(p)] = p._fc_flat[1]
            else:
                self._goff[id(p)] = off
                off += -(-p.numel() // 64) * 64
        self._gtotal = self.flat.n if self.flat is not None else off
        self._sig = self.signature(det)
        self._build_weights()
        self._build()
        self._finalise()

    @staticmethod
    def signature(det):
        from .flat import GENERATION
        return GENERATION[0]

    def _new(self):
        self.n_addr += 1
        return self.n_addr - 1

    def D(self, name):
        if name not in self.dim_names:
            self.dim_names[name] = len(self.dim_names)
        return self.dim_names[name]

    def M(self, name):
        if name not in self.map_names:
            self.map_names[name] = len(self.map_names)
        return self.map_names[name]

    def T(self, rows, cols, arena='f', elem=4, extra=0):
        i = self._new()
        self.arena[arena].append((i, self.D(rows), cols * elem, extra))
        return i

    def S(self, tensor):
        i = self._new()
        self.static.append((i, tensor.data_ptr()))
        self.keep.append(tensor)
        return i

    def SA(self, address):
        i = self._new()
        self.static.append((i, int(address)))
        return i

    def DY(self, name):
        if name not in self.dyn:
            self.dyn[name] = self._new()
        return self.dyn[name]

    def AL(self, parent, off_dim, cols, elem=4):
        i = self._new()
        self.alias.append((i, parent, self.D(off_dim), cols * elem))
        return i

    def G(self, p):
        i = self._new()
        self.grad_refs.append((i, self._goff[id(p)]))
        return i

    def emit(self, lst, *words):
        w = list(words) + [0] * (OPW - len(words))
        assert len(w) == OPW, len(w)
        lst.append(w)

    AMAX_SLOTS = 1024
    AMAX_SLOT_BYTES = 2048

    def amax_slot(self):
        if getattr(self, '_amax_buf', None) is None:
            self._amax_buf = torch.zeros(self.AMAX_SLOTS * self.AMAX_SLOT_BYTES // 4, dtype=torch.int32, device=self.dev)
            self._amax_used = 0
            self.keep.append(self._amax_buf)
        assert self._amax_used < self.AMAX_SLOTS
        i = self.SA(self._amax_buf.data_ptr() + self.AMAX_SLOT_BYTES * self._amax_used)
        self._amax_used += 1
        return i

    def amax_op(self, lst, stream, x, rows, cols):
        slot = self.amax_slot()
        self.emit(lst, OP_AMAX, stream, x, self.D(rows), cols, slot)
        return slot

    def _build_weights(self):
        holder = self.det.__dict__.get('_exec_weights')
        if holder is None or holder.sig != self._sig:
            holder = self.det.__dict__['_exec_weights'] = _Weights(self.det, self.dev, self._sig)
        self.w = holder
        self.packed, self.gent_w, self.gents, self.images, self.ncol = holder.packed, holder.gent_w, holder.gents, holder.images, holder.ncol

    @property
    def weights_fresh(self):
        return self.w.fresh

    @weights_fresh.setter
    def weights_fresh(self, v):
        self.w.fresh = v

    def refresh_weights(self):
        self.w.refresh()

    def IMG(self, w, transposed):
        v = self.w.img_of[w.data_ptr()]
        assert v is not None and v[1 if transposed else 0] is not None, 'no split-bf16 image for this kernel shape'
        return self.S(v[1 if transposed else 0])

    def _build(self):
        det = self.det
        bb, nh = det.backbone, det.neck_with_head
        tr = self.training
        F, Bk = self.ops_f, self.ops_b
        tape = []
        self.relu_outs = []
        self.small = []
        relu, elu, none = Fn.ACT['relu'], Fn.ACT['elu'], Fn.ACT['none']
        grad = {}
        head_grads = {}
        self._pready = {}
        small_rows = []
        flushed = [0]

        head_lvl = [None]
        head_written = {}

        def wrote(*params):
            for prm in params:
                self._pready[id(prm)] = len(Bk)
            if head_lvl[0] is not None:
                head_written.setdefault(head_lvl[0], []).extend(params)

        def flush_small(stream):
            n = len(small_rows) - flushed[0]
            if n:
                self.emit(Bk, OP_SMALL_GRADS, stream, self.DY('small_desc'), 2 * flushed[0], 2 * n)
                for _, _, _, w_, b_ in small_rows[flushed[0]:]:
                    wrote(w_, b_)
                flushed[0] = len(small_rows)
        head_wgrads = [0]

        def head_wfin(stream):
            lo = 1 if self.tail0 else 0
            self.emit(Bk, OP_HEAD_WFIN, stream, self.SA(head_part[lo].data_ptr()), self.nl - lo, Cn, 64, n_reg, n_cls,
                      self.G(nh.centerness_conv.kernel), self.G(nh.reg_conv.kernel), self.G(nh.cls_conv.kernel),
                      self.SA(bias_part[lo].data_ptr()), self.G(nh.cls_conv.bias))
            wrote(nh.centerness_conv.kernel, nh.reg_conv.kernel, nh.cls_conv.kernel, nh.cls_conv.bias)

        def wstream(cur):
            return S_WGRAD if self.wgrad_async else cur

        grad2 = {}

        def flush2(t):
            g2, rows, cols, stream = grad2.pop(t)
            self.emit(Bk, OP_ADD, stream, grad[t], g2, self.D(rows), cols)
            grad_src.pop(grad[t], None)
            amax_of.pop(grad[t], None)

        def accumulate(t, g, rows, cols, stream):
            if t not in grad:
                grad[t] = g
            elif Fn.BN_FUSE and t not in grad2:
                grad2[t] = (g, rows, cols, stream)
            else:
                if t in grad2:
                    flush2(t)
                self.emit(Bk, OP_ADD, stream, grad[t], g, self.D(rows), cols)
                grad_src.pop(grad[t], None)
                amax_of.pop(grad[t], None)

        def take(t, rows, cols, pair=False):
            if t in head_grads:
                g, lvl = head_grads.pop(t)
                self.emit(Bk, OP_WAIT, S_MAIN, EV_HB + lvl)
                for prm in head_written.pop(lvl, ()):
                    self._pready[id(prm)] = max(self._pready[id(prm)], len(Bk))
                accumulate(t, g, rows, cols, S_MAIN)
            if pair:
                return grad[t], (grad2.pop(t)[0] if t in grad2 else None)
            if t in grad2:
                flush2(t)
            return grad[t]

        def got(t):
            if t in grad2:
                flush2(t)
            return grad[t]

        def emit_wgrad(cur, *words):
            if self.wgrad_async:
                ev = EV_W0 if cur == S_MAIN else EV_W1
                self.emit(Bk, OP_RECORD, cur, ev)
                self.emit(Bk, OP_WAIT, S_WGRAD, ev)
            self.emit(Bk, OP_WGRAD, wstream(cur), *words)

        AMAX = Fn.X6 and Fn.split_mode() == 2
        amax_f = {}
        amax_of = {}
        if AMAX:
            self.amax_slot()
            self.emit(F, OP_CLEAR, S_MAIN, self.SA(self._amax_buf.data_ptr()), 0)

        def fwd_amax(x, rows, cols, stream):
            if not AMAX:
                return -1
            if x in amax_of:
                return amax_of[x]
            if (x, stream) not in amax_f:
                amax_f[(x, stream)] = self.amax_op(F, stream, x, rows, cols)
            return amax_f[(x, stream)]

        producer = {}
        grad_src = {}

        def conv(x, mod, mname, rows_in, rows_out, stream=S_MAIN):
            Cin, Cout = mod.in_channels, mod.out_channels
            y = self.T(rows_out, Cout)
            m = self.M(mname)
            ax = fwd_amax(x, rows_in, Cin, stream)
            self.emit(F, OP_CONV, stream, x, self.IMG(mod.kernel, False), m, 0, y, -1, Cin, Cout, *([0] * 10), ax + 1)
            producer[y] = (len(F) - 1, rows_out, Cout)
            if tr:
                def bwd():
                    gy = take(y, rows_out, Cout) if stream == S_MAIN else got(y)
                    gx = self.T(rows_in, Cin, 'b')
                    ag = (amax_of[gy] if gy in amax_of else self.amax_op(Bk, stream, gy, rows_out, Cout)) if AMAX else -1
                    self.emit(Bk, OP_CONV, stream, gy, self.IMG(mod.kernel, True), m, 1, gx, -1, Cout, Cin, *([0] * 10), ag + 1)
                    grad_src[gx] = (len(Bk) - 1, rows_in, Cin, stream)
                    emit_wgrad(stream, x, gy, m, self.G(mod.kernel), -1, Cin, Cout, ax + 1, ag + 1)
                    wrote(mod.kernel)
                    accumulate(x, gx, rows_in, Cin, stream)
                tape.append((stream, bwd))
            return y

        def gemm(x, w_tensor, rows, Cin, Cout, gw_dst, stream=S_MAIN):
            y = self.T(rows, Cout)
            ax = fwd_amax(x, rows, Cin, stream)
            self.emit(F, OP_CONV, stream, x, self.IMG(w_tensor, False), -1, 0, y, self.D(rows), Cin, Cout, *([0] * 10), ax + 1)
            producer[y] = (len(F) - 1, rows, Cout)
            if tr:
                def bwd():
                    gy = take(y, rows, Cout) if stream == S_MAIN else got(y)
                    gx = self.T(rows, Cin, 'b')
                    ag = (amax_of[gy] if gy in amax_of else self.amax_op(Bk, stream, gy, rows, Cout)) if AMAX else -1
                    self.emit(Bk, OP_CONV, stream, gy, self.IMG(w_tensor, True), -1, 1, gx, self.D(rows), Cout, Cin, *([0] * 10), ag + 1)
                    grad_src[gx] = (len(Bk) - 1, rows, Cin, stream)
                    emit_wgrad(stream, x, gy, -1, gw_dst, self.D(rows), Cin, Cout, ax + 1, ag + 1)
                    if w_tensor is self.packed:
                        head_wgrads[0] += 1
                        if head_wgrads[0] == self.nl - (1 if self.tail0 else 0) and self.wgrad_async:
                            head_wfin(S_WGRAD)
                    accumulate(x, gx, rows, Cin, stream)
                tape.append((stream, bwd))
            return y

        def bn(x, mod, act, rows, res=None, stream=S_MAIN):
            b = mod.bn
            C = b.num_features
            y = self.T(rows, C)
            mean, var, cnt = (self.T('one', C), self.T('one', C), self.T('one', 1)) if tr else (-1, -1, -1)
            if act == relu:
                self.relu_outs.append((y, rows, C))
            prod_word, groups = 0, 1
            if tr and Fn.BN_FUSE and x in producer:
                pi, prows, pcols = producer[x]
                groups = pcols // C
                assert pcols == groups * C and groups in (1, 8)
                F[pi][10] = self.T(prows, pcols // 8, extra=8 * pcols + 256) + 1
                prod_word = pi + 1
            ay = -1
            if AMAX:
                ay = amax_of[y] = self.amax_slot()
            self.emit(F, OP_BN_FWD, stream, x, self.D(rows), C, _f(b.eps), self.S(b.weight), self.S(b.bias), -1 if res is None else res, act,
                      _f(b.momentum), y, mean, var, cnt, self.S(b.running_mean), self.S(b.running_var), self.S(b.num_batches_tracked),
                      1 if tr else 0, prod_word, groups, ay + 1)
            if tr:
                sums = torch.zeros((2, C), dtype=torch.float32, device=self.dev)
                si = self.S(sums)

                def bwd():
                    small_rows.append((sums.data_ptr(), None, C, b.weight, b.bias))
                    gy, gy2 = take(y, rows, C, pair=True) if stream == S_MAIN else (got(y), None)
                    gx = self.T(rows, C, 'b')
                    gres = self.T(rows, C, 'b') if res is not None else -1
                    prod = 0
                    last, first = (gy, None) if gy2 is None else (gy2, gy)
                    src = grad_src.get(last)
                    if Fn.BN_FUSE and src is not None and src[3] == stream and src[1:3] == (rows, C):
                        pi = src[0]
                        Bk[pi][10] = self.T(rows, C // 8, 'b', extra=8 * C + 256) + 1
                        Bk[pi][11:20] = [x + 1, mean, var, self.S(b.weight), self.S(b.bias), _f(b.eps), act,
                                         0 if first is None else first + 1, 0 if res is None else y + 1]
                        prod = pi + 1
                    agx = -1
                    if AMAX:
                        agx = amax_of[gx] = self.amax_slot()
                    self.emit(Bk, OP_BN_BWD, stream, x, y if res is not None else -1, gy, self.D(rows), C, mean, var, cnt, _f(b.eps),
                              self.S(b.weight), self.S(b.bias), act, gx, gres, si, 0 if gy2 is None else gy2 + 1, prod, agx + 1)
                    accumulate(x, gx, rows, C, stream)
                    if res is not None:
                        accumulate(res, gres, rows, C, stream)
                tape.append((stream, bwd))
            return y

        x0 = self.DY('x0')
        seg1 = self.DY('seg1')
        stem, inorm = bb.conv1[0], bb.conv1[1]
        t_stem = self.T('n1', 64)
        col = self.T('n1', 84) if tr else -1
        self.emit(F, OP_STEM_FWD, S_MAIN, x0, self.S(stem.kernel), self.M('stem'), t_stem, col)
        mean_in, var_in, cnt_in = self.T('B', 64), self.T('B', 64), self.T('B', 1)
        self.emit(F, OP_COL_STATS, S_MAIN, t_stem, seg1, self.D('n1'), 64, self.D('B'), mean_in, var_in, cnt_in)
        t_in = self.T('n1', 64)
        self.emit(F, OP_NORM_FWD, S_MAIN, t_stem, seg1, self.D('n1'), 64, mean_in, var_in, _f(inorm.eps), self.S(inorm.weight),
                  self.S(inorm.bias), -1, relu, t_in)
        self.relu_outs.append((t_in, 'n1', 64))
        t_pool, arg = self.T('n2', 64), self.T('n2', 64)
        self.pool_arg = (arg, 'n2', 64)
        ap = -1
        if AMAX:
            ap = amax_of[t_pool] = self.amax_slot()
        self.emit(F, OP_MAXPOOL_FWD, S_MAIN, t_in, self.M('pool'), 64, t_pool, arg, ap + 1)
        if tr:
            in_sums = self.T('B', 2 * 64, 'b')
            self.in_sums = in_sums

            def bwd_stem():
                small_rows.append((None, 'B', 64, inorm.weight, inorm.bias))
                g_pool = take(t_pool, 'n2', 64)
                g_in = self.T('n1', 64, 'b')
                self.emit(Bk, OP_MAXPOOL_BWD, S_MAIN, g_pool, arg, self.M('pool'), 64, g_in)
                g_stem = self.T('n1', 64, 'b')
                self.emit(Bk, OP_NORM_BWD, S_MAIN, t_stem, -1, g_in, seg1, self.D('n1'), 64, self.D('B'), mean_in, var_in, cnt_in,
                          _f(inorm.eps), self.S(inorm.weight), self.S(inorm.bias), relu, g_stem, -1, in_sums)
                if self.wgrad_async:
                    self.emit(Bk, OP_RECORD, S_MAIN, EV_W0)
                    self.emit(Bk, OP_WAIT, S_WGRAD, EV_W0)
                self.emit(Bk, OP_STEM_WGRAD, wstream(S_MAIN), col, g_stem, self.M('stem'), self.G(stem.kernel))
                wrote(stem.kernel)
            tape.append((S_MAIN, bwd_stem))
        cur, cur_rows, cur_C = t_pool, 'n2', 64
        levels = []
        for li in range(1, self.nl + 1):
            rows = f'L{li}'
            if tr:
                tape.append((S_MAIN, lambda: flush_small(S_MAIN)))
            for j, blk in enumerate(getattr(bb, f'layer{li}')):
                planes = blk.conv1.out_channels
                if j == 0:
                    assert blk.downsample is not None and blk.conv1.stride == 2
                    t_ds = conv(cur, blk.downsample[0], f'ds{li}', cur_rows, rows)
                    res = bn(t_ds, blk.downsample[1], none, rows)
                    t1 = conv(cur, blk.conv1, f'down{li}', cur_rows, rows)
                else:
                    assert blk.downsample is None
                    res = cur
                    t1 = conv(cur, blk.conv1, f'same{li}', rows, rows)
                t1 = bn(t1, blk.norm1, relu, rows)
                t2 = conv(t1, blk.conv2, f'same{li}', rows, rows)
                cur = bn(t2, blk.norm2, relu, rows, res=res)
                cur_rows, cur_C = rows, planes
            levels.append((cur, rows, cur_C))
        n_reg, n_cls = nh.n_reg_outs, nh.n_classes
        Cn = nh.centerness_conv.in_channels
        cent_all, bbox_all = self.T('Nall', 1), self.T('Nall', n_reg)
        cls_all, cmax_all = self.T('Nall', n_cls), self.T('Nall', 1)
        self.out_idx = (cent_all, bbox_all, cls_all, cmax_all)
        head_part = None
        if tr:
            tape.append((S_MAIN, lambda: flush_small(S_MAIN)))
            self.gout_idx = (self.DY('g_cent'), self.DY('g_bbox'), self.DY('g_cls'))
            head_part = torch.zeros((self.nl, Cn, 64), dtype=torch.float32, device=self.dev)
            bias_part = torch.zeros((self.nl, n_cls), dtype=torch.float32, device=self.dev)
            self.keep += [head_part, bias_part]
        x, x_rows, x_C = levels[-1]
        for i in range(self.nl - 1, -1, -1):
            if i < self.nl - 1:
                up = getattr(nh, f'up_block_{i + 1}')
                gi = self.gents.index(up[0])
                g_rows = f'g{i}'
                Ci = up[0].out_channels
                gw_tmp = torch.zeros((x_C, 8 * Ci), dtype=torch.float32, device=self.dev)
                self.keep.append(gw_tmp)
                gw_i = self.S(gw_tmp)
                if tr:
                    def bwd_perm(gw_i=gw_i, mod=up[0], Cin=x_C, Ci=Ci):
                        self.emit(Bk, OP_PERMUTE_GENT, wstream(S_MAIN), gw_i, self.G(mod.kernel), Cin, Ci)
                        wrote(mod.kernel)
                        flush_small(S_MAIN)
                    tape.append((S_MAIN, bwd_perm))
                t = gemm(x, self.gent_w[gi], x_rows, x_C, 8 * Ci, gw_i)
                t = bn(t, up[1], elu, g_rows)
                t = conv(t, up[3], f'gsame{i}', g_rows, g_rows)
                t = bn(t, up[4], elu, g_rows)
                fb, fb_rows, fb_C = levels[i]
                u = self.T(g_rows, Ci)
                rows_i = self.DY(f'rows{i}')
                self.emit(F, OP_UNION_FWD, S_MAIN, t, fb, rows_i, self.D(g_rows), self.D(fb_rows), self.D(g_rows), Ci, u)
                if AMAX:
                    amax_of[u] = self.amax_op(F, S_MAIN, u, g_rows, Ci)
                if tr:
                    def bwd_union(u=u, t=t, fb=fb, fb_rows=fb_rows, rows_i=rows_i, g_rows=g_rows, Ci=Ci):
                        gu = take(u, g_rows, Ci)
                        accumulate(t, gu, g_rows, Ci, S_MAIN)
                        gfb = self.T(fb_rows, Ci, 'b')
                        self.emit(Bk, OP_GATHER, S_MAIN, gu, rows_i, self.D(fb_rows), Ci, gfb)
                        accumulate(fb, gfb, fb_rows, Ci, S_MAIN)
                    tape.append((S_MAIN, bwd_union))
                x, x_rows, x_C = u, g_rows, Ci
                kname = f'gsame{i}'
            else:
                kname = f'same{self.nl}'
            if i == 0 and self.tail0:
                self.x0_idx = (x, x_rows, x_C)
                if tr:
                    grad[x] = self.DY('g_x0')
                continue
            hs = S_HEAD if (self.head_overlap and i > 0) else S_MAIN
            if hs == S_HEAD:
                self.emit(F, OP_RECORD, S_MAIN, EV_FORK + i)
                self.emit(F, OP_WAIT, S_HEAD, EV_FORK + i)
            ob = getattr(nh, f'out_block_{i}')
            o = conv(x, ob[0], kname, x_rows, x_rows, stream=hs)
            o = bn(o, ob[1], elu, x_rows, stream=hs)
            gw_head = self.SA(head_part[i].data_ptr()) if tr else -1
            y = gemm(o, self.packed, x_rows, Cn, 64, gw_head, stream=hs)
            off = f'off{i}'
            outs = [self.AL(cent_all, off, 1), self.AL(bbox_all, off, n_reg), self.AL(cls_all, off, n_cls), self.AL(cmax_all, off, 1)]
            self.emit(F, OP_HEAD_FWD, hs, y, 64, self.S(nh.cls_conv.bias), self.S(nh.scales[i].scale), self.D(x_rows), n_reg, n_cls, *outs)
            if tr:
                def bwd_head(y=y, outs=outs, off=off, hs=hs, rows=x_rows, lvl=i):
                    gy = self.T(rows, 64, 'b')
                    gin = [self.AL(g, off, c) for g, c in zip(self.gout_idx, (1, n_reg, n_cls))]
                    agy = -1
                    if AMAX:
                        agy = amax_of[gy] = self.amax_slot()
                    self.emit(Bk, OP_HEAD_BWD, hs, y, 64, self.S(nh.scales[lvl].scale), outs[1], gin[0], gin[1], gin[2], self.D(rows), n_reg,
                              n_cls, gy, -1, self.G(nh.scales[lvl].scale), self.SA(bias_part[lvl].data_ptr()), agy + 1)
                    wrote(nh.scales[lvl].scale)
                    grad[y] = gy
                tape.append((hs, bwd_head))
                if hs == S_HEAD:
                    tape.append((S_HEAD, ('join', x, x_rows, x_C, i)))
        if self.head_overlap:
            self.emit(F, OP_RECORD, S_HEAD, EV_HEAD_DONE)
            self.emit(F, OP_WAIT, S_MAIN, EV_HEAD_DONE)
        if AMAX:
            n_fwd_slots = self._amax_used
            F[0][3] = self.AMAX_SLOT_BYTES * n_fwd_slots
            if tr:
                self.emit(Bk, OP_CLEAR, S_MAIN, self.SA(self._amax_buf.data_ptr() + self.AMAX_SLOT_BYTES * n_fwd_slots), 0)
                clear_b = len(Bk) - 1
        if tr:
            if self.head_overlap:
                self.emit(Bk, OP_RECORD, S_MAIN, EV_BWD0)
                self.emit(Bk, OP_WAIT, S_HEAD, EV_BWD0)
                branches, cur_b = [], None
                for s, e in reversed(tape):
                    if s != S_HEAD:
                        continue
                    if isinstance(e, tuple):
                        cur_b = [e, []]
                        branches.append(cur_b)
                    else:
                        cur_b[1].append(e)
                for (_, xt, rows, C, lvl), ems in sorted(branches, key=lambda b: b[0][4]):
                    saved = grad.pop(xt, None)
                    assert saved is None
                    head_lvl[0] = lvl
                    for e in ems:
                        e()
                    flush_small(S_HEAD)
                    head_lvl[0] = None
                    self.emit(Bk, OP_RECORD, S_HEAD, EV_HB + lvl)
                    head_grads[xt] = (got(xt), lvl)
                    grad.pop(xt)
            for s, e in reversed(tape):
                if s == S_MAIN:
                    e()
            assert not head_grads and not head_written, 'a head branch was never joined'
            if not self.wgrad_async:
                head_wfin(S_MAIN)
            flush_small(S_MAIN)
            assert head_wgrads[0] == self.nl - (1 if self.tail0 else 0)
            self.small = small_rows
            missing = [n for n, prm in det.named_parameters() if prm.requires_grad and id(prm) not in self._pready]
            if self.tail0:
                missing = [n for n in missing if not (n.startswith('neck_with_head.out_block_0.') or n == 'neck_with_head.scales.0.scale')]
            assert not missing, missing
            if self.wgrad_async:
                self.emit(Bk, OP_RECORD, S_WGRAD, EV_WEND)
                self.emit(Bk, OP_WAIT, S_MAIN, EV_WEND)
            if AMAX:
                Bk[clear_b][3] = self.AMAX_SLOT_BYTES * (self._amax_used - n_fwd_slots)

    def _finalise(self):
        self.ops_f = np.ascontiguousarray(np.asarray(self.ops_f, dtype=np.int64).reshape(-1, OPW))
        self.ops_b = np.ascontiguousarray(np.asarray(self.ops_b, dtype=np.int64).reshape(-1, OPW)) if self.ops_b else np.zeros((0, OPW), np.int64)
        self.addr0 = np.zeros(self.n_addr, dtype=np.int64)
        for i, a in self.static:
            self.addr0[i] = a
        self._ar = {}
        for k in ('f', 'b'):
            a = self.arena[k]
            self._ar[k] = (np.array([t[0] for t in a], dtype=np.int64), np.array([t[1] for t in a], dtype=np.int64),
                           np.array([t[2] for t in a], dtype=np.int64), np.array([t[3] for t in a], dtype=np.int64))
        self._al = (np.array([t[0] for t in self.alias], dtype=np.int64), np.array([t[1] for t in self.alias], dtype=np.int64),
                    np.array([t[2] for t in self.alias], dtype=np.int64), np.array([t[3] for t in self.alias], dtype=np.int64))
        self._gr = (np.array([t[0] for t in self.grad_refs], dtype=np.int64), np.array([t[1] for t in self.grad_refs], dtype=np.int64) * 4)
        self.n_dims, self.n_maps = len(self.dim_names), len(self.map_names)
        self._ws = [None, None, None]
        self._need = np.zeros(3, dtype=np.int64)
        self._cfg = np.array([Fn.BN_SMALL_ELEMS, Fn.FLAGS, 0, 0], dtype=np.int64)
        self.n_conv_f = int((self.ops_f[:, 0] == OP_CONV).sum())
        self.n_conv_b = int((self.ops_b[:, 0] == OP_CONV).sum()) if len(self.ops_b) else 0
        self.n_amax = int((self.ops_f[:, 0] == OP_AMAX).sum()) + (int((self.ops_b[:, 0] == OP_AMAX).sum()) if len(self.ops_b) else 0)
        self._anchor = torch.zeros(1, device=self.dev, requires_grad=True)
        if self.training:
            n = len(self.small)
            self._small = np.zeros((2 * n, 8), dtype=np.int64)
            self._small_goff = np.zeros(2 * n, dtype=np.int64)
            self._small_in = None
            for k, (src, nseg, C, w, b) in enumerate(self.small):
                for h, p in ((0, b), (1, w)):
                    r = 2 * k + h
                    self._small[r, 2], self._small[r, 3], self._small[r, 4] = C, 1, 2 * C
                    self._small_goff[r] = self._goff[id(p)] * 4
                    if src is not None:
                        self._small[r, 0] = src + 4 * C * h
                    else:
                        self._small_in = (2 * k, C)

    def _fill_arena(self, addr, dims, which, base):
        idx, di, bpr, ext = self._ar[which]
        if len(idx) == 0:
            return
        sizes = (dims[di] * bpr + ext + (ALIGN - 1)) // ALIGN * ALIGN
        offs = np.cumsum(sizes) - sizes
        addr[idx] = base + offs

    def _arena_bytes(self, dims, which):
        idx, di, bpr, ext = self._ar[which]
        return int(((dims[di] * bpr + ext + (ALIGN - 1)) // ALIGN * ALIGN).sum()) + ALIGN

    def bind(self, x, batch_size, backward):
        nl = self.nl
        cm0 = x.cmap
        dims = np.zeros(self.n_dims, dtype=np.int64)
        maps = np.zeros((self.n_maps, MAPW), dtype=np.int64)
        dn, mn = self.dim_names, self.map_names

        def setd(k, v):
            if k in dn:
                dims[dn[k]] = v
        m1 = cm0.strided(2)
        m2 = m1.strided(2)
        maps[mn['stem']] = cm0.kernel_map(m1, 3).desc(conv=False)
        maps[mn['pool']] = m1.kernel_map(m2, 2).desc(conv=False)
        kms = {}
        setd('n0', cm0.n); setd('n1', m1.n); setd('n2', m2.n); setd('B', batch_size); setd('one', 1)
        prev, lv = m2, []
        for li in range(1, nl + 1):
            mi = prev.strided(2)
            kms[f'down{li}'], kms[f'ds{li}'], kms[f'same{li}'] = prev.kernel_map(mi, 3), prev.kernel_map(mi, 1), mi.kernel_map(mi, 3)
            for k in (f'down{li}', f'ds{li}', f'same{li}'):
                maps[mn[k]] = kms[k].desc(True, backward)
            setd(f'L{li}', mi.n)
            lv.append(mi)
            prev = mi
        xm = lv[-1]
        head_maps = [xm]
        dyn = {}
        for i in range(nl - 2, -1, -1):
            g = xm.generate()
            u, rows, swapped = lv[i].union(g)
            if not swapped or u is not g:
                return None
            kms[f'gsame{i}'] = g.kernel_map(g, 3)
            maps[mn[f'gsame{i}']] = kms[f'gsame{i}'].desc(True, backward)
            setd(f'g{i}', g.n)
            dyn[f'rows{i}'] = rows
            xm = g
            head_maps.append(g)
        head_maps = head_maps[::-1]
        off = 0
        for i, cm in enumerate(head_maps):
            if i == 0 and self.tail0:
                continue
            setd(f'off{i}', off)
            off += cm.n
        setd('Nall', off)
        st = dict(dims=dims, maps=maps, dyn=dyn, head_maps=head_maps, x=x, seg1=m1.coords, n_all=off)
        if PROBE is not None:
            from .sparse import _rec
            st['pairs'] = {mn[k]: _rec(km._pairs[3].sum() if km._pairs is not None else (km.nbr >= 0).sum()) for k, km in kms.items()}
            PROBE.append(dict(pairs=st['pairs'], nf=self.n_conv_f, nb=self.n_conv_b, na=self.n_amax))
        return st

    def _streams(self):
        dev = self.dev
        nh = self.det.neck_with_head
        main = L.stream()
        head = nh._head_stream(dev).cuda_stream if self.head_overlap else main
        wg = Fn.wgrad_stream(dev).cuda_stream if self.wgrad_async else main
        return np.array([main, head, wg], dtype=np.int64)

    def _run(self, ops, addr, st, begin=0, end=None, size_only=False):
        streams = self._streams()
        self._cfg[2] = 1 if 'pairs' in st else 0
        self._cfg[3] = 1 if size_only else 0
        end = len(ops) if end is None else end
        while True:
            ws = np.array([w.data_ptr() if w is not None else 0 for w in self._ws], dtype=np.int64)
            wsb = np.array([w.numel() if w is not None else 0 for w in self._ws], dtype=np.int64)
            rc = L.lib().fc_exec(ops.ctypes.data, begin, end, addr.ctypes.data, st['dims'].ctypes.data, st['maps'].ctypes.data,
                                 streams.ctypes.data, ws.ctypes.data, wsb.ctypes.data, self._need.ctypes.data, self._cfg.ctypes.data)
            if rc == -2:
                for i in range(3):
                    if self._need[i] > wsb[i]:
                        self._ws[i] = torch.empty(int(self._need[i] * 5 // 4) + (1 << 20), dtype=torch.uint8, device=self.dev)
                continue
            if rc != 0:
                raise RuntimeError(f'fc_exec failed: {"invalid argument" if rc == -1 else "hipError %d" % rc}')
            return

    def decisions(self, st):
        fa, addr, dims = st['fa'], st['addr'], st['dims']

        def view(idx, rows, C, dtype):
            n = int(dims[self.dim_names[rows]])
            o = int(addr[idx] - fa.data_ptr())
            return fa[o:o + n * C * 4].view(dtype).view(n, C)
        relu = [(view(t, r, C, torch.float32) > 0).cpu() for t, r, C in self.relu_outs]
        return relu, view(*self.pool_arg, torch.int32).cpu()

    def forward(self, st):
        trusted = (TRUSTED is not None and TRUSTED.w is self.w) or (not self.training and getattr(self.det, 'static_weights', False))
        if not (self.weights_fresh and trusted):
            self.refresh_weights()
        ev = self.images.event
        if ev is not None:
            torch.cuda.current_stream().wait_event(ev)
        if self.training:
            return _NetFn.apply(self._anchor, self, st)
        return self._forward(st)

    def _forward(self, st):
        dims = st['dims']
        fa = torch.empty(self._arena_bytes(dims, 'f'), dtype=torch.uint8, device=self.dev)
        addr = self.addr0.copy()
        base = (fa.data_ptr() + ALIGN - 1) // ALIGN * ALIGN
        self._fill_arena(addr, dims, 'f', base)
        addr[self.dyn['x0']] = st['x'].F.data_ptr()
        addr[self.dyn['seg1']] = st['seg1'].data_ptr()
        for k, t in st['dyn'].items():
            addr[self.dyn[k]] = t.data_ptr()
        ai, ap, ad, ab = self._al
        fwd_alias = addr[ap] != 0
        addr[ai[fwd_alias]] = addr[ap[fwd_alias]] + dims[ad[fwd_alias]] * ab[fwd_alias]
        st['fa'], st['addr'] = fa, addr
        self._run(self.ops_f, addr, st)
        n = st['n_all']
        nh = self.det.neck_with_head
        outs = []
        for idx, c in zip(self.out_idx, (1, nh.n_reg_outs, nh.n_classes, 1)):
            o = int(addr[idx] - fa.data_ptr())
            outs.append(fa[o:o + n * c * 4].view(torch.float32).view(n, c))
        if self.tail0:
            t, rows, C = self.x0_idx
            n0 = int(dims[self.dim_names[rows]])
            o = int(addr[t] - fa.data_ptr())
            outs.append(fa[o:o + n0 * C * 4].view(torch.float32).view(n0, C))
        return tuple(outs)

    def _backward(self, st, g_cent, g_bbox, g_cls, g_x0=None):
        dims, addr = st['dims'], st['addr']
        n = st['n_all']
        nh = self.det.neck_with_head
        gs = []
        for g, c in zip((g_cent, g_bbox, g_cls), (1, nh.n_reg_outs, nh.n_classes)):
            gs.append(g.contiguous() if g is not None else torch.zeros((n, c), dtype=torch.float32, device=self.dev))
        if self.tail0:
            t, rows, C = self.x0_idx
            n0 = int(dims[self.dim_names[rows]])
            g_x0 = g_x0.contiguous() if g_x0 is not None else torch.zeros((n0, C), dtype=torch.float32, device=self.dev)
            gs.append(g_x0)
        ba = torch.empty(self._arena_bytes(dims, 'b'), dtype=torch.uint8, device=self.dev)
        base = (ba.data_ptr() + ALIGN - 1) // ALIGN * ALIGN
        self._fill_arena(addr, dims, 'b', base)
        for k, g in zip(('g_cent', 'g_bbox', 'g_cls', 'g_x0'), gs):
            addr[self.dyn[k]] = g.data_ptr()
        ai, ap, ad, ab = self._al
        addr[ai] = addr[ap] + dims[ad] * ab
        own = self._own_params()
        pre = [(p, p.grad) for p in own if p.grad is not None]
        aliased = self.flat is not None and any(g.data_ptr() == self.flat.grad_view(p).data_ptr() for p, g in pre)
        accum = bool(pre) and (self.flat is None or aliased or len(pre) > 16)
        if self.flat is not None and not accum:
            gbuf = self.flat.grad
        else:
            gbuf = torch.zeros(self._gtotal, dtype=torch.float32, device=self.dev)
        gi, go = self._gr
        addr[gi] = gbuf.data_ptr() + go
        desc = self._small.copy()
        desc[:, 1] = gbuf.data_ptr() + self._small_goff
        r, C = self._small_in
        B = int(dims[self.dim_names['B']])
        desc[r, 0], desc[r + 1, 0] = addr[self.in_sums], addr[self.in_sums] + 4 * C
        desc[r:r + 2, 3] = B
        desc_dev = L.upload(desc, self.dev)
        addr[self.dyn['small_desc']] = desc_dev.data_ptr()
        gv = self._grad_views(gbuf)
        if not accum:
            for p in own:
                p.grad = gv[id(p)]
        from . import dist as D
        av = D.ACTIVE
        if av is not None and av.buckets and av.flat is self.flat and self.flat is not None and not accum and not self.tail0:
            pos = 0
            self._run(self.ops_b, addr, st, size_only=True)
            for upto in self._bucket_ready(av):
                if upto > pos:
                    self._run(self.ops_b, addr, st, pos, upto)
                    pos = upto
                av.launch_next()
            if pos < len(self.ops_b):
                self._run(self.ops_b, addr, st, pos, len(self.ops_b))
        else:
            self._run(self.ops_b, addr, st)
        if accum:
            for p in own:
                if p.grad is None:
                    p.grad = gv[id(p)]
                else:
                    p.grad.add_(gv[id(p)])
        else:
            for p, g0 in pre:
                gv[id(p)].add_(g0)
            if self.flat is not None and not self.tail0:
                self.flat.complete = True
        st['ba'] = ba

    def _own_params(self):
        c = getattr(self, '_own', None)
        if c is None:
            c = self._own = [p for p in self._params if id(p) in self._pready]
        return c

    def _bucket_ready(self, av):
        key = id(av)
        c = getattr(self, '_br', None)
        if c is None or c[0] != key:
            out, run = [], 0
            for b in av.buckets:
                run = max(run, max(self._pready[id(p)] for p in b))
                out.append(run)
            c = self._br = (key, out)
        return c[1]

    def _grad_views(self, gbuf):
        key = gbuf.data_ptr()
        cache = getattr(self, '_gv', None)
        if cache is None or cache[0] != key:
            views = {id(p): gbuf[self._goff[id(p)]:self._goff[id(p)] + p.numel()].view(p.shape) for p in self._params}
            cache = self._gv = (key, views, gbuf)
        return cache[1]


class _Weights:

    def __init__(self, det, dev, sig):
        nh = det.neck_with_head
        self.det, self.sig = det, sig
        head = (nh.centerness_conv, nh.reg_conv, nh.cls_conv)
        convs = [m for m in det.modules() if isinstance(m, MEnn.MinkowskiConvolution) and m not in head]
        self.gents = [m for m in det.modules() if isinstance(m, MEnn.MinkowskiGenerativeConvolutionTranspose)]
        C = nh.centerness_conv.in_channels
        self.ncol = 1 + nh.n_reg_outs + nh.n_classes
        self.packed = torch.zeros((1, C, 64), dtype=torch.float32, device=dev)
        self.gent_w = [torch.empty((1, m.in_channels, 8 * m.out_channels), dtype=torch.float32, device=dev) for m in self.gents]
        ws = [m.kernel for m in convs] + [self.packed] + self.gent_w
        self.images = Fn.WeightImages(ws)
        self.img_of = {}
        for w in ws:
            K = 1 if w.dim() == 2 else w.shape[0]
            self.img_of[w.data_ptr()] = self.images.table.get((w.data_ptr(), K, w.shape[-2], w.shape[-1]))
        self.fresh = False

    @torch.no_grad()
    def refresh(self):
        nh = self.det.neck_with_head
        torch.cat((nh.centerness_conv.kernel, nh.reg_conv.kernel, nh.cls_conv.kernel), dim=1, out=self.packed[0][:, :self.ncol])
        for m, w in zip(self.gents, self.gent_w):
            w.view(m.in_channels, 8, m.out_channels).copy_(m.kernel.permute(1, 0, 2))
        self.images.build()
        self.fresh = True


class _NetFn(torch.autograd.Function):

    @staticmethod
    def forward(ctx, anchor, prog, st):
        ctx.prog, ctx.st = prog, st
        outs = prog._forward(st)
        ctx.mark_non_differentiable(outs[3])
        return outs

    @staticmethod
    def backward(ctx, g_cent, g_bbox, g_cls, _g_max, g_x0=None):
        ctx.prog._backward(ctx.st, g_cent, g_bbox, g_cls, g_x0)
        return None, None, None


def program_for(det, training, tail0=False):
    if not supported(det):
        return None
    nh = det.neck_with_head
    if tail0 and min(det.backbone.n_outs, 4) < 2:
        return None
    key = (bool(training), bool(Fn.WGRAD_ASYNC), bool(nh.head_overlap), bool(tail0))
    fuse = bool(Fn.BN_FUSE)
    mode = Fn.split_mode() if Fn.X6 else -1
    cache = det.__dict__.setdefault('_programs', {})
    sig = NetProgram.signature(det)
    prog = cache.get(key + (fuse, mode))
    if prog is None or prog._sig != sig:
        prog = cache[key + (fuse, mode)] = NetProgram(det, *key)
    if getattr(prog.w, 'split_mode', mode) != mode:
        prog.w.fresh = False
    prog.w.split_mode = mode
    return prog
```

include/fcaf3d_hip.h:

```cpp
#ifndef FCAF3D_HIP_H
#define FCAF3D_HIP_H
#include <stdint.h>

#ifndef __HIP_PLATFORM_AMD__
typedef struct ihipStream_t* hipStream_t;
#endif

#ifdef __cplusplus
extern "C" {
#endif

#define FC_ABI_VERSION 8
#ifndef FC_AMAX_SLOT_BYTES
#define FC_AMAX_SLOT_BYTES 2048
#endif
int fc_abi_version(void);


int fc_voxelize(const float* points, int64_t n, int pt_stride, int batch_idx, float voxel_size, float feat_div,
                int nfeat, int* coords, float* feats, hipStream_t stream);

int fc_augment_voxelize(const float* points, int64_t n_src, int pt_stride, const int* sample_idx, int64_t n_out,
                        const float* xform_host, int batch_idx, float voxel_size, float feat_div, int nfeat, int* coords,
                        float* feats, float* points_out, hipStream_t stream);

int fc_morton_keys(const int* coords, int64_t n, long long* keys, hipStream_t stream);

int fc_scan_flags(const unsigned char* flags, int64_t n, int* pos, int* total_dev, void* ws, int64_t ws_bytes,
                  hipStream_t stream);
int fc_compact_rows(const unsigned char* flags, const int* pos, int64_t n, int* kept, int64_t m, hipStream_t stream);

int64_t fc_hash_unique_ws_bytes(int64_t n);
int fc_hash_unique(const int* coords, int64_t n, int q, unsigned long long* table_keys, int* table_vals, int64_t cap,
                   int* out_coords, int* first_idx, int* inverse, int* n_out_dev, void* ws, int64_t ws_bytes,
                   hipStream_t stream);

int fc_kernel_map(const int* out_coords, int64_t n_out, const unsigned long long* table_keys, const int* table_vals,
                  int64_t cap, const int* offsets, int K, int* nbr, hipStream_t stream);
int fc_nbr_row_masks(const int* nbr, int64_t n_out, int K, int* masks, hipStream_t stream);
int fc_permute_nbr(const int* nbr, const int* order, int64_t n_out, int K, int* nbr_sorted, hipStream_t stream);
int64_t fc_kernel_map_pairs_ws_bytes(int64_t n_out, int K);
int fc_kernel_map_pairs(const int* nbr, int64_t n_out, int K, int* pair_in, int* pair_out, int* pair_pos, int* cnt,
                        void* ws, int64_t ws_bytes, hipStream_t stream);
int fc_kernel_map_transpose(const int* nbr, int64_t n_out, int64_t n_in, int K, int* nbr_t, hipStream_t stream);

int fc_gen_coords(const int* coords, int64_t n, int half_stride, int* out_coords, hipStream_t stream);

int fc_kernel_map_children(const int* parent_nbr, int64_t n_parent, int* nbr, hipStream_t stream);
int fc_child_rows(const int* query_coords, int64_t n, const unsigned long long* parent_keys, const int* parent_vals,
                  int64_t cap, int child_stride, int* rows, int* n_found_dev, hipStream_t stream);

int64_t fc_union_map_ws_bytes(int64_t n_b);
int fc_union_map(const int* coords_b, int64_t n_b, const unsigned long long* table_keys_a, const int* table_vals_a,
                 int64_t cap_a, int64_t n_a, int* row_b, int* new_coords, int* n_new_dev, void* ws, int64_t ws_bytes,
                 hipStream_t stream);

int fc_interp(const int* query_coords, int64_t n, const unsigned long long* table_keys, const int* table_vals, int64_t cap,
              const float* feats, int C, int tensor_stride, float* out, hipStream_t stream);

int fc_gather_coords(const int* src, const int* idx, int64_t n, int* dst, hipStream_t stream);


int fc_plan_cfg_words(void);
int fc_plan_out_words(int B, int nl);
int64_t fc_plan_stage1_bytes(int64_t total_points, int B, int nl, int nfeat);
int fc_plan_levels(const int64_t* cfg, const int64_t* scenes, void* arena1, int64_t arena1_bytes, int64_t* out, int* counts_host,
                   hipStream_t stream);
int64_t fc_plan_stage2_bytes(const int64_t* cfg, int64_t* out, const int* counts_host);
int fc_plan_maps(const int64_t* cfg, int64_t* out, const int* counts_host, void* arena2, int64_t arena2_bytes, int* cnt_host,
                 hipStream_t stream);
int64_t fc_plan_probe_read(float* ms, double* bytes, int* kind, int64_t cap);
int64_t fc_argsort27_ws_bytes(int64_t n);
int fc_argsort27(const int* keys, int64_t n, int* order, void* ws, int64_t ws_bytes, hipStream_t stream);


#define FC_CONV_FMA (1 << 0)
#define FC_CONV_BM_SHIFT 4
#define FC_CONV_BN_SHIFT 6
#define FC_CONV_TILE_MASK 3
#define FC_CONV_S_SHIFT 8
#define FC_CONV_S_MASK 255
#define FC_CONV_WGRAD_PIPE_OFF (1 << 16)
#define FC_CONV_PIPE_OFF (1 << 17)
#define FC_CONV_PIPE_ON (1 << 18)
#define FC_CONV_WGRAD_DEEP (1 << 19)
#define FC_CONV_WGRAD_PIPE_ON (1 << 20)
#define FC_CONV_GLDS (1 << 21)
#define FC_CONV_GLDS_OFF (1 << 22)
#define FC_CONV_WT (1 << 23)
#define FC_CONV_SPLIT (1 << 24)
#define FC_CONV_IMAGE (1 << 26)
#define FC_CONV_FLAT (1 << 27)
#define FC_CONV_WGRAD_MULTI_OFF (1 << 29)
#define FC_CONV_WGRAD_MULTI_FIRST (1 << 30)

int64_t fc_x6_weight_image_bytes(int K, int R, int C);
int fc_x6_weight_image(const float* W, void* img, int K, int R, int C, int transposed, hipStream_t stream);
int fc_x6_weight_images(const int64_t* desc, int n, int64_t total_blocks, hipStream_t stream);

int64_t fc_conv_fwd_ws_bytes(int64_t n_out, int K, int Cin, int Cout, int flags);
int fc_conv_fwd(const float* in, const float* W, const int* nbr, const int* out_index, float* out, int64_t n_in,
                int64_t n_out, int K, int Cin, int Cout, int flags, void* ws, int64_t ws_bytes, hipStream_t stream);

int64_t fc_conv_fwd_pairs_ws_bytes(int64_t n_out, int K, int Cout);
int fc_conv_fwd_pairs(const float* in, const float* W, const int* pair_in, const int* pair_cnt, const int* pair_pos,
                      float* out, int64_t n_in, int64_t n_out, int K, int Cin, int Cout, int flags, void* ws,
                      int64_t ws_bytes, hipStream_t stream);

int fc_conv_fwd_pairs_tiles(const float* in, const float* W, const int* pair_in, const int* pair_cnt, const int* pair_pos,
                            float* out, int64_t n_in, int64_t n_out, int K, int Cin, int Cout, int64_t live_tiles, int flags,
                            void* ws, int64_t ws_bytes, hipStream_t stream);

int64_t fc_conv_stats_blocks(int64_t n_out, int K, int Cin, int Cout, int flags, int pairs);
int fc_conv_fwd_stats(const float* in, const float* W, const int* nbr, const int* out_index, float* out, int64_t n_in,
                      int64_t n_out, int K, int Cin, int Cout, int flags, void* ws, int64_t ws_bytes, float* stats,
                      hipStream_t stream);
int fc_conv_fwd_pairs_tiles_stats(const float* in, const float* W, const int* pair_in, const int* pair_cnt, const int* pair_pos,
                                  float* out, int64_t n_in, int64_t n_out, int K, int Cin, int Cout, int64_t live_tiles, int flags,
                                  void* ws, int64_t ws_bytes, float* stats, hipStream_t stream);
int fc_conv_fwd_bn_bwd_stats(const float* in, const float* W, const int* nbr, const int* out_index, float* out, int64_t n_in,
                             int64_t n_out, int K, int Cin, int Cout, int flags, void* ws, int64_t ws_bytes, float* stats,
                             const float* bn_x, const float* mean, const float* var, const float* gamma, const float* beta, float eps,
                             int act, const float* add, const float* bn_y, hipStream_t stream);
int fc_conv_fwd_pairs_tiles_bn_bwd_stats(const float* in, const float* W, const int* pair_in, const int* pair_cnt, const int* pair_pos,
                                         float* out, int64_t n_in, int64_t n_out, int K, int Cin, int Cout, int64_t live_tiles, int flags,
                                         void* ws, int64_t ws_bytes, float* stats, const float* bn_x, const float* mean,
                                         const float* var, const float* gamma, const float* beta, float eps, int act,
                                         const float* add, const float* bn_y, hipStream_t stream);

int64_t fc_conv_wgrad_ws_bytes(int64_t n_out, int K, int Cin, int Cout, int flags);
int fc_conv_wgrad(const float* in, const float* gout, const int* nbr, const int* row_index, float* gW, int64_t n_in,
                  int64_t n_out, int K, int Cin, int Cout, int flags, void* ws, int64_t ws_bytes, hipStream_t stream);
int fc_conv_wgrad_pairs(const float* in, const float* gout, const int* pair_in, const int* pair_out, const int* pair_cnt,
                        float* gW, int64_t n_in, int64_t n_out, int K, int Cin, int Cout, int flags, void* ws,
                        int64_t ws_bytes, hipStream_t stream);

int fc_stem_conv_fwd(const float* in, const float* W, const int* nbr, float* out, float* col, int64_t n_in, int64_t n_out,
                     int K, hipStream_t stream);
int64_t fc_stem_conv_wgrad_ws_bytes(int64_t n_out, int K);
int fc_stem_conv_wgrad(const float* col, const float* gout, float* gW, int64_t n_out, int K, void* ws, int64_t ws_bytes,
                       hipStream_t stream);

int fc_transpose_weight(const float* W, float* Wt, int K, int Cin, int Cout, hipStream_t stream);


int64_t fc_col_stats_ws_bytes(int64_t n, int C, int nseg);
int fc_col_stats(const float* x, const int* seg, int seg_stride, int64_t n, int C, int nseg, float* mean, float* var,
                 float* cnt, void* ws, int64_t ws_bytes, hipStream_t stream);

int fc_seg_col_sums(const float* x, const int* seg, int seg_stride, int64_t n, int C, int nseg, float* out, void* ws,
                    int64_t ws_bytes, hipStream_t stream);
int fc_bn_running_update(const float* mean, const float* var, const float* cnt, float momentum, int C, float* running_mean,
                         float* running_var, long long* num_batches_tracked, hipStream_t stream);

int fc_norm_act_fwd(const float* x, const int* seg, int seg_stride, int64_t n, int C, const float* mean, const float* var,
                    float eps, const float* gamma, const float* beta, const float* residual, int act, float* y,
                    hipStream_t stream);
int64_t fc_norm_act_bwd_ws_bytes(int64_t n, int C, int nseg);
int fc_norm_act_bwd(const float* x, const float* y, const float* gy, const int* seg, int seg_stride, int64_t n, int C,
                    int nseg, const float* mean, const float* var, const float* cnt, float eps, const float* gamma,
                    const float* beta, int act, float* gx, float* gres, float* sums, void* ws, int64_t ws_bytes,
                    hipStream_t stream);

int64_t fc_bn_stats_ws_bytes(int64_t n, int C);
int fc_bn_stats_train(const float* x, int64_t n, int C, float momentum, float* mean, float* var, float* cnt,
                      float* running_mean, float* running_var, long long* num_batches_tracked, void* ws,
                      int64_t ws_bytes, hipStream_t stream);
int64_t fc_bn_small_ws_bytes(int C);
int fc_bn_act_train_fwd(const float* x, int64_t n, int C, float eps, const float* gamma, const float* beta,
                        const float* residual, int act, float momentum, float* y, float* mean, float* var, float* cnt,
                        float* running_mean, float* running_var, long long* num_batches_tracked, void* ws,
                        int64_t ws_bytes, hipStream_t stream);
int fc_bn_act_train_bwd(const float* x, const float* y, const float* gy, int64_t n, int C, const float* mean,
                        const float* var, float eps, const float* gamma, const float* beta, int act, float* gx, float* gres,
                        float* sums, void* ws, int64_t ws_bytes, hipStream_t stream);

int64_t fc_bn_train_ws_bytes(int64_t n, int C);
int fc_bn_train_fwd(const float* x, int64_t n, int C, float eps, const float* gamma, const float* beta, const float* residual,
                    int act, float momentum, float* y, float* mean, float* var, float* cnt, float* running_mean,
                    float* running_var, long long* num_batches_tracked, const float* part, int64_t nb_part, int groups,
                    int64_t small_elems, void* ws, int64_t ws_bytes, hipStream_t stream);
int fc_bn_train_bwd(const float* x, const float* y, const float* gy, const float* gy2, int64_t n, int C, const float* mean,
                    const float* var, const float* cnt, float eps, const float* gamma, const float* beta, int act, float* gx,
                    float* gres, float* sums, const float* part, int64_t nb_part, int64_t small_elems, void* ws, int64_t ws_bytes,
                    hipStream_t stream);

int fc_maxpool_fwd(const float* in, const int* nbr, int64_t n_out, int K, int C, float* out, int* argrow,
                   hipStream_t stream);
int fc_maxpool_bwd(const float* gout, const int* argrow, int64_t n_out, int C, float* gin, hipStream_t stream);

int fc_gather_rows(const float* src, const int* idx, int64_t n, int C, float* dst, hipStream_t stream);
int fc_scatter_rows_add(const float* src, const int* idx, int64_t n, int C, float* dst, hipStream_t stream);


int fc_focal_loss_fwd(const float* logits, const long long* labels, const float* row_weight, int64_t n, int C, float gamma,
                      float alpha, float* loss_rows, hipStream_t stream);
int fc_focal_loss_bwd(const float* logits, const long long* labels, const float* row_weight, int64_t n, int C, float gamma,
                      float alpha, const float* gscale_dev, float* glogits, hipStream_t stream);

int fc_aiou3d_fwd_bwd(const float* pred, const float* target, int target_stride, int64_t n, float eps, float* iou,
                      float* dpred, hipStream_t stream);

int64_t fc_fcaf3d_loss_ws_bytes(int64_t n);
int fc_fcaf3d_loss_fwd(const float* points, const float* bbox_pred, const float* centerness, const float* cls_score,
                       const float* centerness_t, const float* bbox_t, const long long* labels, const int* scene,
                       const float* inv_pos, const float* inv_den, int64_t n, int n_classes, float gamma, float alpha,
                       float lw_cls, float lw_centerness, float lw_bbox, float* loss_cls, float* loss_centerness,
                       float* loss_bbox, void* ws, int64_t ws_bytes, hipStream_t stream);
int fc_fcaf3d_loss_bwd(const float* points, const float* bbox_pred, const float* centerness, const float* cls_score,
                       const float* centerness_t, const float* bbox_t, const long long* labels, const int* scene,
                       const float* inv_pos, const float* inv_den, int64_t n, int n_classes, float gamma, float alpha,
                       float lw_cls, float lw_centerness, float lw_bbox, const float* g_cls, const float* g_centerness,
                       const float* g_bbox, float* grad_cls_score, float* grad_centerness, float* grad_bbox_pred,
                       hipStream_t stream);

int fc_riou3d_fwd_bwd(const float* pred, const float* target, const float* weight, int64_t n, float* iou, float* dpred,
                      hipStream_t stream);

int fc_head_split_fwd(const float* y, int ld, const float* bias, const float* scale_dev, int64_t n, int n_reg, int n_cls,
                      float* centerness, float* bbox_pred, float* cls_score, float* cls_max, hipStream_t stream);
int fc_head_split_bwd(const float* y, int ld, const float* scale_dev, const float* bbox_pred, const float* g_centerness,
                      const float* g_bbox, const float* g_cls, int64_t n, int n_reg, int n_cls, float* gy,
                      float* gscale_row, hipStream_t stream);
int64_t fc_head_split_bwd_sums_ws_bytes(int64_t n);
int fc_head_split_bwd_sums(const float* y, int ld, const float* scale_dev, const float* bbox_pred, const float* g_centerness,
                           const float* g_bbox, const float* g_cls, int64_t n, int n_reg, int n_cls, float* gy, float* gbias,
                           float* gscale, void* ws, int64_t ws_bytes, hipStream_t stream);

int fc_sort_v(const float* vertices, const unsigned char* mask, const int* num_valid, int64_t n_pairs, int* idx,
              hipStream_t stream);

int64_t fc_assign_ws_bytes(int B, int M, int L);
int fc_assign_targets(const float* points, const int* scene, const int* level, int64_t N, const float* boxes,
                      const long long* labels, const int* box_count, int B, int M, int L, const int* order,
                      const int* seg_start, int limit, int topk, float* centerness_t, float* bbox_t, long long* labels_out,
                      void* ws, int64_t ws_bytes, hipStream_t stream);


int64_t fc_nms_bev_ws_bytes(int nseg, int stride);
int fc_nms_bev(const float* boxes, const int* counts_dev, int nseg, int stride, float thresh, int rotated,
               unsigned long long* mask_ws, int64_t ws_bytes, int* keep, int* keep_count, hipStream_t stream);
int fc_boxes_iou_bev(const float* boxes_a, int n, const float* boxes_b, int m, int rotated, float* out,
                     hipStream_t stream);


#define FC_MERGE_TO_BOTTOM 1
#define FC_MERGE_WITH_YAW 2
#define FC_MERGE_XF_FLIP_H (1ull << 32)
#define FC_MERGE_XF_FLIP_V (1ull << 33)
int64_t fc_merge_sorted_segments_ws_bytes(int nseg_out, int max_total);
int fc_merge_sorted_segments(const int64_t* desc, int nseg_out, int K, const int* counts_dev, const int* keep, int keep_stride,
                             const int64_t* ord, int ord_stride, const float* scores, int score_stride, const float* boxes,
                             int flags, int max_total, int cap, float* out_boxes, float* out_scores, int* out_src,
                             int* out_count, int stride_out, void* ws, int64_t ws_bytes, hipStream_t stream);


int64_t fc_grad_norm_ws_bytes(int64_t n);
int fc_grad_norm(const float* g, int64_t n, float max_norm, float* out, void* ws, int64_t ws_bytes, hipStream_t stream);
int fc_adamw_step(float* p, const float* g, float* m, float* v, int64_t n, float lr, float beta1, float beta2, float eps,
                  float weight_decay, float bias_correction1, float bias_correction2, const float* norm_and_clip,
                  hipStream_t stream);

int fc_set_bf16_fast(int on);

int fc_set_split_mode(int mode);
int fc_get_split_mode(void);
int fc_amax(const float* x, int64_t n, unsigned* slot, hipStream_t stream);
int fc_conv_amax_hint(const unsigned* amax_in, const unsigned* amax_gout);
int fc_amax_out_hint(unsigned* amax_word);
int fc_debug_set_h3r(int mode);


int fc_exec_op_words(void);
int64_t fc_exec_probe_read(float* ms, int64_t* meta, int64_t cap);
int fc_exec_map_words(void);
int fc_exec(const int64_t* ops, int64_t op_begin, int64_t op_end, const int64_t* addr, const int64_t* dims, const int64_t* maps,
            const int64_t* streams, const int64_t* ws, const int64_t* ws_bytes, int64_t* ws_need, const int64_t* cfg);

#ifdef __cplusplus
}
#endif
#endif
```

Baseline: 513.3.

## Fuse stem instance-norm with maxpool and fold generative union into BN epilogue

The stem's instance norm + ReLU is fused into the 8-neighbour maxpool forward, which writes a pool-parent map instead of a full normalised activation tensor. The backward pass reconstructs the pooled gradient inline inside the norm backward kernels. In the neck, the union copy/memset/scatter-add is replaced by an inverse-row map and an add inside the BN forward epilogue. This removes several full-activation round trips through memory, but adds indirect loads, an extra inverse-rows kernel, and a hard requirement that the pool kernel has exactly 8 neighbours.

```diff
diff --git a/fcaf3d_amd/_lib.py b/fcaf3d_amd/_lib.py
--- a/fcaf3d_amd/_lib.py
+++ b/fcaf3d_amd/_lib.py
@@ -34,7 +34,7 @@
     return protos
 
 
-ABI_VERSION = 8
+ABI_VERSION = 9
 _lib = None
 _protos = None
 
diff --git a/fcaf3d_amd/csrc/exec.hip b/fcaf3d_amd/csrc/exec.hip
--- a/fcaf3d_amd/csrc/exec.hip
+++ b/fcaf3d_amd/csrc/exec.hip
@@ -7,7 +7,7 @@
 enum : int64_t {
   OP_STEM_FWD = 1, OP_COL_STATS, OP_NORM_FWD, OP_MAXPOOL_FWD, OP_CONV, OP_BN_FWD, OP_UNION_FWD, OP_HEAD_FWD, OP_RECORD, OP_WAIT,
   OP_HEAD_BWD, OP_WGRAD, OP_BN_BWD, OP_NORM_BWD, OP_MAXPOOL_BWD, OP_STEM_WGRAD, OP_GATHER, OP_ADD, OP_SMALL_GRADS,
-  OP_PERMUTE_GENT, OP_HEAD_WFIN, OP_COPY, OP_COL_SUM, OP_ROW_SUM, OP_AMAX, OP_CLEAR
+  OP_PERMUTE_GENT, OP_HEAD_WFIN, OP_COPY, OP_COL_SUM, OP_ROW_SUM, OP_AMAX, OP_CLEAR, OP_NORM_POOL_FWD, OP_POOL_NORM_BWD, OP_INV_ROWS
 };
 constexpr int OPW = 24;
 constexpr int MAPW = 20;
@@ -182,7 +182,7 @@
     static const int ko = getenv("FC_KO_OPS") ? atoi(getenv("FC_KO_OPS")) : 0;
     const int64_t o = op[0];
     if (!c.dry && (((ko & 1) && (o == OP_WGRAD || o == OP_STEM_WGRAD)) || ((ko & 2) && o == OP_CONV) ||
-                   ((ko & 4) && (o == OP_BN_FWD || o == OP_BN_BWD || o == OP_NORM_FWD || o == OP_NORM_BWD || o == OP_COL_STATS))))
+                   ((ko & 4) && (o == OP_BN_FWD || o == OP_BN_BWD || o == OP_COL_STATS || o == OP_NORM_POOL_FWD || o == OP_POOL_NORM_BWD))))
       return 0;
   }
 #endif
@@ -199,19 +199,6 @@
       if (!want_ws(c, s, fc_col_stats_ws_bytes(n, C, nseg))) return 0;
       return fc_col_stats(P<const float>(c, op[2]), P<const int>(c, op[3]), op[3] >= 0 ? 4 : 0, n, C, nseg, P<float>(c, op[7]),
                           P<float>(c, op[8]), P<float>(c, op[9]), c.ws[s], c.ws_bytes[s], st);
-    }
-    case OP_NORM_FWD: {
-      if (c.dry) return 0;
-      return fc_norm_act_fwd(P<const float>(c, op[2]), P<const int>(c, op[3]), op[3] >= 0 ? 4 : 0, c.dims[op[4]], (int)op[5],
-                             P<const float>(c, op[6]), P<const float>(c, op[7]), (float)as_double(op[8]), P<const float>(c, op[9]),
-                             P<const float>(c, op[10]), P<const float>(c, op[11]), (int)op[12], P<float>(c, op[13]), st);
-    }
-    case OP_MAXPOOL_FWD: {
-      const int64_t* m = c.maps + op[3] * MAPW;
-      if (c.dry) return 0;
-      if (op[7] > 0) fc_amax_out_hint(P<unsigned>(c, op[7] - 1));
-      return fc_maxpool_fwd(P<const float>(c, op[2]), reinterpret_cast<const int*>(m[3]), m[1], (int)m[2], (int)op[4], P<float>(c, op[5]),
-                            P<int>(c, op[6]), st);
     }
     case OP_CONV: {
       const int Cin = (int)op[8], Cout = (int)op[9];
@@ -262,12 +249,14 @@
       const int64_t n = c.dims[op[3]];
       const int C = (int)op[4];
       const float eps = (float)as_double(op[5]), mom = (float)as_double(op[10]);
+      const int* add_inv = op[22] > 0 ? P<const int>(c, op[22] - 1) : nullptr;
+      const float* add_src = op[22] > 0 ? P<const float>(c, op[23] - 1) : nullptr;
       if (!op[18]) {
         if (c.dry) return 0;
         if (op[21] > 0) fc_amax_out_hint(P<unsigned>(c, op[21] - 1));
-        return fc_norm_act_fwd(P<const float>(c, op[2]), nullptr, 0, n, C, P<const float>(c, op[15]), P<const float>(c, op[16]), eps,
-                               P<const float>(c, op[6]), P<const float>(c, op[7]), P<const float>(c, op[8]), (int)op[9], P<float>(c, op[11]),
-                               st);
+        return fc_norm_act_add_fwd(P<const float>(c, op[2]), nullptr, 0, n, C, P<const float>(c, op[15]), P<const float>(c, op[16]), eps,
+                                   P<const float>(c, op[6]), P<const float>(c, op[7]), P<const float>(c, op[8]), (int)op[9], add_inv, add_src,
+                                   P<float>(c, op[11]), st);
       }
       const float* part = nullptr;
       int64_t nbp = 0;
@@ -278,19 +267,10 @@
       }
       if (!want_ws(c, s, fc_bn_train_ws_bytes(n, C))) return 0;
       if (op[21] > 0) fc_amax_out_hint(P<unsigned>(c, op[21] - 1));
-      return fc_bn_train_fwd(P<const float>(c, op[2]), n, C, eps, P<const float>(c, op[6]), P<const float>(c, op[7]),
-                             P<const float>(c, op[8]), (int)op[9], mom, P<float>(c, op[11]), P<float>(c, op[12]), P<float>(c, op[13]),
-                             P<float>(c, op[14]), P<float>(c, op[15]), P<float>(c, op[16]), P<long long>(c, op[17]), part, nbp,
-                             op[20] > 0 ? (int)op[20] : 1, c.bn_small_elems, c.ws[s], c.ws_bytes[s], st);
-    }
-    case OP_UNION_FWD: {
-      if (c.dry) return 0;
-      const int64_t n_a = c.dims[op[5]], n_b = c.dims[op[6]], n_u = c.dims[op[7]];
-      const int C = (int)op[8];
-      float* out = P<float>(c, op[9]);
-      FC_HIP(hipMemcpyAsync(out, P<const float>(c, op[2]), sizeof(float) * n_a * C, hipMemcpyDeviceToDevice, st));
-      if (n_u > n_a) FC_HIP(hipMemsetAsync(out + n_a * C, 0, sizeof(float) * (n_u - n_a) * C, st));
-      return fc_scatter_rows_add(P<const float>(c, op[3]), P<const int>(c, op[4]), n_b, C, out, st);
+      return fc_bn_train_add_fwd(P<const float>(c, op[2]), n, C, eps, P<const float>(c, op[6]), P<const float>(c, op[7]),
+                                 P<const float>(c, op[8]), (int)op[9], mom, P<float>(c, op[11]), P<float>(c, op[12]), P<float>(c, op[13]),
+                                 P<float>(c, op[14]), P<float>(c, op[15]), P<float>(c, op[16]), P<long long>(c, op[17]), part, nbp,
+                                 op[20] > 0 ? (int)op[20] : 1, c.bn_small_elems, add_inv, add_src, c.ws[s], c.ws_bytes[s], st);
     }
     case OP_HEAD_FWD: {
       if (c.dry) return 0;
@@ -360,22 +340,6 @@
                              P<float>(c, op[14]), P<float>(c, op[15]), P<float>(c, op[16]), part, nbp, c.bn_small_elems, c.ws[s],
                              c.ws_bytes[s], st);
     }
-    case OP_NORM_BWD: {
-      const int64_t n = c.dims[op[6]];
-      const int C = (int)op[7], nseg = (int)c.dims[op[8]];
-      if (!want_ws(c, s, fc_norm_act_bwd_ws_bytes(n, C, nseg))) return 0;
-      return fc_norm_act_bwd(P<const float>(c, op[2]), P<const float>(c, op[3]), P<const float>(c, op[4]), P<const int>(c, op[5]),
-                             op[5] >= 0 ? 4 : 0, n, C, nseg, P<const float>(c, op[9]), P<const float>(c, op[10]), P<const float>(c, op[11]),
-                             (float)as_double(op[12]), P<const float>(c, op[13]), P<const float>(c, op[14]), (int)op[15], P<float>(c, op[16]),
-                             P<float>(c, op[17]), P<float>(c, op[18]), c.ws[s], c.ws_bytes[s], st);
-    }
-    case OP_MAXPOOL_BWD: {
-      const int64_t* m = c.maps + op[4] * MAPW;
-      if (c.dry) return 0;
-      const int C = (int)op[5];
-      FC_HIP(hipMemsetAsync(P<float>(c, op[6]), 0, sizeof(float) * m[0] * C, st));
-      return fc_maxpool_bwd(P<const float>(c, op[2]), P<const int>(c, op[3]), m[1], C, P<float>(c, op[6]), st);
-    }
     case OP_STEM_WGRAD: {
       const int64_t* m = c.maps + op[4] * MAPW;
       if (!want_ws(c, s, fc_stem_conv_wgrad_ws_bytes(m[1], (int)m[2]))) return 0;
@@ -435,6 +399,30 @@
       if (c.dry) return 0;
       FC_HIP(hipMemsetAsync(P<void>(c, op[2]), 0, (size_t)op[3], st));
       return 0;
+    }
+    case OP_NORM_POOL_FWD: {
+      const int64_t* m = c.maps + op[11] * MAPW;
+      if (c.dry) return 0;
+      if ((int)m[2] != 8) return FC_EINVAL;
+      if (op[15] > 0) fc_amax_out_hint(P<unsigned>(c, op[15] - 1));
+      return fc_norm_act_maxpool8_fwd(P<const float>(c, op[2]), P<const int>(c, op[3]), op[3] >= 0 ? 4 : 0, (int)op[4], P<const float>(c, op[5]),
+                                      P<const float>(c, op[6]), (float)as_double(op[7]), P<const float>(c, op[8]), P<const float>(c, op[9]),
+                                      (int)op[10], reinterpret_cast<const int*>(m[3]), m[1], P<float>(c, op[12]), P<int>(c, op[13]),
+                                      P<float>(c, op[14]), P<int>(c, op[16]), st);
+    }
+    case OP_POOL_NORM_BWD: {
+      const int64_t n = c.dims[op[7]];
+      const int C = (int)op[8], nseg = (int)c.dims[op[9]];
+      if (!want_ws(c, s, fc_maxpool8_norm_act_bwd_ws_bytes(n, C, nseg))) return 0;
+      return fc_maxpool8_norm_act_bwd(P<const float>(c, op[2]), P<const float>(c, op[3]), P<const int>(c, op[4]), P<const int>(c, op[5]),
+                                      P<const int>(c, op[6]), op[6] >= 0 ? 4 : 0, n, C, nseg, P<const float>(c, op[10]),
+                                      P<const float>(c, op[11]), P<const float>(c, op[12]), (float)as_double(op[13]),
+                                      P<const float>(c, op[14]), P<const float>(c, op[15]), (int)op[16], P<float>(c, op[17]),
+                                      P<float>(c, op[18]), c.ws[s], c.ws_bytes[s], st);
+    }
+    case OP_INV_ROWS: {
+      if (c.dry) return 0;
+      return fc_inverse_rows(P<const int>(c, op[2]), c.dims[op[3]], c.dims[op[4]], P<int>(c, op[5]), st);
     }
     case OP_COPY: {
       if (c.dry) return 0;
diff --git a/fcaf3d_amd/csrc/norm.hip b/fcaf3d_amd/csrc/norm.hip
--- a/fcaf3d_amd/csrc/norm.hip
+++ b/fcaf3d_amd/csrc/norm.hip
@@ -217,7 +217,8 @@
 __global__ void k_norm_act_fwd(const float* __restrict__ x, const int* __restrict__ seg, int seg_stride, int64_t n, int C,
                                const float* __restrict__ mean, const float* __restrict__ var, float eps,
                                const float* __restrict__ gamma, const float* __restrict__ beta,
-                               const float* __restrict__ residual, int act, float* __restrict__ y, unsigned* __restrict__ amax_out) {
+                               const float* __restrict__ residual, int act, const int* __restrict__ add_inv,
+                               const float* __restrict__ add_src, float* __restrict__ y, unsigned* __restrict__ amax_out) {
   int64_t t = (int64_t)blockIdx.x * blockDim.x + threadIdx.x;
   const int c4n = C / 4;
   unsigned am = 0u;
@@ -225,6 +226,7 @@
   int64_t r = t / c4n;
   int c = (int)(t % c4n) * 4;
   int s = seg_of(seg, seg_stride, r);
+  const int q = add_inv ? add_inv[r] : -1;
   float4 v = *reinterpret_cast<const float4*>(x + r * C + c);
   float4 mu = *reinterpret_cast<const float4*>(mean + (int64_t)s * C + c);
   float4 va = *reinterpret_cast<const float4*>(var + (int64_t)s * C + c);
@@ -240,14 +242,20 @@
     o.x += rs.x; o.y += rs.y; o.z += rs.z; o.w += rs.w;
   }
   o.x = act_fwd(o.x, act); o.y = act_fwd(o.y, act); o.z = act_fwd(o.z, act); o.w = act_fwd(o.w, act);
+  if (q >= 0) {
+    const float4 f = *reinterpret_cast<const float4*>(add_src + (int64_t)q * C + c);
+    o.x += f.x; o.y += f.y; o.z += f.z; o.w += f.w;
+  }
   *reinterpret_cast<float4*>(y + r * C + c) = o;
   amax_fold(am, o.x); amax_fold(am, o.y); amax_fold(am, o.z); amax_fold(am, o.w);
   }
   if (amax_out) amax_commit(am, amax_out);
 }
 
+template <bool POOL>
 __global__ void k_norm_bwd_partial(const float* __restrict__ x, const float* __restrict__ y, const float* __restrict__ gy,
-                                   const float* __restrict__ gy2, const int* __restrict__ seg, int seg_stride, int64_t n, int C, int nseg,
+                                   const float* __restrict__ gy2, const int* __restrict__ pool_parent,
+                                   const int* __restrict__ pool_arg, const int* __restrict__ seg, int seg_stride, int64_t n, int C, int nseg,
                                    const float* __restrict__ mean, const float* __restrict__ var, float eps, int act,
                                    const float* __restrict__ gamma, const float* __restrict__ beta,
                                    int64_t rpb, float* __restrict__ part) {
@@ -284,7 +292,15 @@
           const int64_t rc = ok[u] ? r : r0;
           if (chk) ok[u] = ok[u] && seg[rc * seg_stride] == s;
           xv[u] = *reinterpret_cast<const float4*>(x + rc * C + cl * 4);
-          gv[u] = *reinterpret_cast<const float4*>(gy + rc * C + cl * 4);
+          if (POOL) {
+            const int64_t o = pool_parent[rc];
+            const int4 a = *reinterpret_cast<const int4*>(pool_arg + o * C + cl * 4);
+            gv[u] = *reinterpret_cast<const float4*>(gy + o * C + cl * 4);
+            gv[u].x = a.x == rc ? gv[u].x : 0.f; gv[u].y = a.y == rc ? gv[u].y : 0.f;
+            gv[u].z = a.z == rc ? gv[u].z : 0.f; gv[u].w = a.w == rc ? gv[u].w : 0.f;
+          } else {
+            gv[u] = *reinterpret_cast<const float4*>(gy + rc * C + cl * 4);
+          }
           if (gy2) g2[u] = *reinterpret_cast<const float4*>(gy2 + rc * C + cl * 4);
           if (from_y) yv[u] = *reinterpret_cast<const float4*>(y + rc * C + cl * 4);
         }
@@ -331,8 +347,10 @@
   }
 }
 
+template <bool POOL>
 __global__ void k_norm_bwd_apply(const float* __restrict__ x, const float* __restrict__ y, const float* __restrict__ gy,
-                                 const float* __restrict__ gy2, const int* __restrict__ seg, int seg_stride, int64_t n, int C,
+                                 const float* __restrict__ gy2, const int* __restrict__ pool_parent,
+                                 const int* __restrict__ pool_arg, const int* __restrict__ seg, int seg_stride, int64_t n, int C,
                                  const float* __restrict__ mean, const float* __restrict__ var, float eps,
                                  const float* __restrict__ gamma, const float* __restrict__ beta,
                                  const float* __restrict__ sums ,
@@ -348,7 +366,14 @@
   float inv_n = 1.f / cnt[s];
   float xv[4], gv[4], muv[4], vav[4], gam[4], bet[4] = {0.f, 0.f, 0.f, 0.f}, s1[4], s2[4], yv[4], o[4], gr[4];
   *reinterpret_cast<float4*>(xv) = *reinterpret_cast<const float4*>(x + r * C + c);
-  *reinterpret_cast<float4*>(gv) = *reinterpret_cast<const float4*>(gy + r * C + c);
+  if (POOL) {
+    const int64_t o = pool_parent[r];
+    const int4 a = *reinterpret_cast<const int4*>(pool_arg + o * C + c);
+    *reinterpret_cast<float4*>(gv) = *reinterpret_cast<const float4*>(gy + o * C + c);
+    gv[0] = a.x == r ? gv[0] : 0.f; gv[1] = a.y == r ? gv[1] : 0.f; gv[2] = a.z == r ? gv[2] : 0.f; gv[3] = a.w == r ? gv[3] : 0.f;
+  } else {
+    *reinterpret_cast<float4*>(gv) = *reinterpret_cast<const float4*>(gy + r * C + c);
+  }
   if (gy2) {
     const float4 t2 = *reinterpret_cast<const float4*>(gy2 + r * C + c);
     gv[0] += t2.x; gv[1] += t2.y; gv[2] += t2.z; gv[3] += t2.w;
@@ -441,6 +466,72 @@
   if (i >= 0) gin[(int64_t)i * C + (t % C)] = gout[t];
 }
 
+__global__ void k_norm_act_maxpool8_fwd(const float* __restrict__ x, const int* __restrict__ seg, int seg_stride, int C,
+                                        const float* __restrict__ mean, const float* __restrict__ var, float eps,
+                                        const float* __restrict__ gamma, const float* __restrict__ beta, int act,
+                                        const int* __restrict__ nbr, int64_t n_out, float* __restrict__ out, int* __restrict__ argrow,
+                                        float* __restrict__ y, int* __restrict__ parent, unsigned* __restrict__ amax_out) {
+  const int c4n = C / 4;
+  int64_t t = (int64_t)blockIdx.x * blockDim.x + threadIdx.x;
+  unsigned am = 0u;
+  if (t < n_out * c4n) {
+  const int64_t o = t / c4n;
+  const int c = (int)(t % c4n) * 4;
+  int idx[8];
+#pragma unroll
+  for (int k = 0; k < 8; ++k) idx[k] = nbr[(int64_t)k * n_out + o];
+  if (parent) {
+    int mine = -1;
+#pragma unroll
+    for (int k = 0; k < 8; ++k) mine = (c == 4 * k) ? idx[k] : mine;
+    if (mine >= 0) parent[mine] = (int)o;
+  }
+  float4 v[8];
+  int first = -1;
+#pragma unroll
+  for (int k = 0; k < 8; ++k) {
+    const int i = idx[k] < 0 ? 0 : idx[k];
+    if (first < 0 && idx[k] >= 0) first = idx[k];
+    v[k] = *reinterpret_cast<const float4*>(x + (int64_t)i * C + c);
+  }
+  float best[4] = {-INFINITY, -INFINITY, -INFINITY, -INFINITY};
+  int arg[4] = {-1, -1, -1, -1};
+  if (first >= 0) {
+    const int s = seg_of(seg, seg_stride, first);
+    float mu[4], va[4], is[4], g[4] = {1.f, 1.f, 1.f, 1.f}, b[4] = {0.f, 0.f, 0.f, 0.f};
+    *reinterpret_cast<float4*>(mu) = *reinterpret_cast<const float4*>(mean + (int64_t)s * C + c);
+    *reinterpret_cast<float4*>(va) = *reinterpret_cast<const float4*>(var + (int64_t)s * C + c);
+    if (gamma) *reinterpret_cast<float4*>(g) = *reinterpret_cast<const float4*>(gamma + c);
+    if (beta) *reinterpret_cast<float4*>(b) = *reinterpret_cast<const float4*>(beta + c);
+#pragma unroll
+    for (int j = 0; j < 4; ++j) is[j] = 1.f / sqrtf(va[j] + eps);
+#pragma unroll
+    for (int k = 0; k < 8; ++k) {
+      if (idx[k] < 0) continue;
+      float e[4] = {v[k].x, v[k].y, v[k].z, v[k].w};
+#pragma unroll
+      for (int j = 0; j < 4; ++j) {
+        e[j] = act_fwd(bn_pre(e[j], mu[j], is[j], g[j], b[j]), act);
+        if (arg[j] < 0 || e[j] > best[j]) { best[j] = e[j]; arg[j] = idx[k]; }
+      }
+      if (y) *reinterpret_cast<float4*>(y + (int64_t)idx[k] * C + c) = make_float4(e[0], e[1], e[2], e[3]);
+    }
+  }
+  float4 ob = make_float4(arg[0] < 0 ? 0.f : best[0], arg[1] < 0 ? 0.f : best[1], arg[2] < 0 ? 0.f : best[2], arg[3] < 0 ? 0.f : best[3]);
+  *reinterpret_cast<float4*>(out + o * C + c) = ob;
+  *reinterpret_cast<int4*>(argrow + o * C + c) = make_int4(arg[0], arg[1], arg[2], arg[3]);
+  amax_fold(am, ob.x); amax_fold(am, ob.y); amax_fold(am, ob.z); amax_fold(am, ob.w);
+  }
+  if (amax_out) amax_commit(am, amax_out);
+}
+
+__global__ void k_inverse_rows(const int* __restrict__ rows, int64_t n, int64_t n_inv, int* __restrict__ inv) {
+  const int64_t i = (int64_t)blockIdx.x * blockDim.x + threadIdx.x;
+  if (i >= n) return;
+  const int r = rows[i];
+  if (r >= 0 && r < n_inv) inv[r] = (int)i;
+}
+
 __global__ void k_gather_rows(const float* __restrict__ src, const int* __restrict__ idx, int64_t n, int C,
                               float* __restrict__ dst) {
   int64_t t = (int64_t)blockIdx.x * blockDim.x + threadIdx.x;
@@ -530,7 +621,8 @@
                             float eps, const float* __restrict__ gamma, const float* __restrict__ beta,
                             const float* __restrict__ residual, int act, float momentum, float* __restrict__ y,
                             float* __restrict__ mean_out, float* __restrict__ var_out, float* __restrict__ cnt_out,
-                            float* __restrict__ rmean, float* __restrict__ rvar, long long* __restrict__ nbt) {
+                            float* __restrict__ rmean, float* __restrict__ rvar, long long* __restrict__ nbt,
+                            const int* __restrict__ add_inv, const float* __restrict__ add_src) {
   extern __shared__ float sm[];
   const int c4n = C / 4;
   const int cl = threadIdx.x % c4n, rl = threadIdx.x / c4n;
@@ -586,6 +678,11 @@
         o[j] = bn_pre(v[u][j], mu[j], is[j], g[j], bt[j]);
         if (residual) o[j] += rs[u][j];
         o[j] = act_fwd(o[j], act);
+      }
+      const int q = add_inv ? add_inv[r] : -1;
+      if (q >= 0) {
+        const float4 f = *reinterpret_cast<const float4*>(add_src + (int64_t)q * C + cl * 4);
+        o[0] += f.x; o[1] += f.y; o[2] += f.z; o[3] += f.w;
       }
       *reinterpret_cast<float4*>(y + r * C + cl * 4) = *reinterpret_cast<float4*>(o);
     }
@@ -730,10 +827,11 @@
                             const float* __restrict__ residual, int act, float momentum, float* __restrict__ y,
                             float* __restrict__ mean_out, float* __restrict__ var_out, float* __restrict__ cnt_out,
                             float* __restrict__ rmean, float* __restrict__ rvar, long long* __restrict__ nbt, int CG,
-                            unsigned* __restrict__ amax_out) {
+                            const int* __restrict__ add_inv, const float* __restrict__ add_src, unsigned* __restrict__ amax_out) {
   extern __shared__ double smd[];
   const int c0 = blockIdx.y * CG;
   x += c0; y += c0; part += c0; mean_out += c0; var_out += c0;
+  if (add_src) add_src += c0;
   if (residual) residual += c0;
   if (gamma) gamma += c0;
   if (beta) beta += c0;
@@ -785,12 +883,14 @@
   unsigned am = 0u;
   for (int64_t rb = r0 + rl; rb < r1; rb += 4 * (int64_t)nrl) {
     float v[4][4], rs[4][4];
+    int q[4];
 #pragma unroll
     for (int u = 0; u < 4; ++u) {
       const int64_t r = rb + (int64_t)u * nrl;
       const int64_t rc = r < r1 ? r : r0;
       *reinterpret_cast<float4*>(v[u]) = *reinterpret_cast<const float4*>(x + rc * C + cl * 4);
       if (residual) *reinterpret_cast<float4*>(rs[u]) = *reinterpret_cast<const float4*>(residual + rc * C + cl * 4);
+      q[u] = add_inv ? add_inv[rc] : -1;
     }
 #pragma unroll
     for (int u = 0; u < 4; ++u) {
@@ -802,6 +902,10 @@
         o[j] = bn_pre(v[u][j], mu[j], is[j], g[j], bt[j]);
         if (residual) o[j] += rs[u][j];
         o[j] = act_fwd(o[j], act);
+      }
+      if (q[u] >= 0) {
+        const float4 f = *reinterpret_cast<const float4*>(add_src + (int64_t)q[u] * C + cl * 4);
+        o[0] += f.x; o[1] += f.y; o[2] += f.z; o[3] += f.w;
       }
       *reinterpret_cast<float4*>(y + r * C + cl * 4) = *reinterpret_cast<float4*>(o);
 #pragma unroll
@@ -988,10 +1092,10 @@
   return FC_OK;
 }
 
-int fc_bn_act_train_fwd(const float* x, int64_t n, int C, float eps, const float* gamma, const float* beta,
-                        const float* residual, int act, float momentum, float* y, float* mean, float* var, float* cnt,
-                        float* running_mean, float* running_var, long long* num_batches_tracked, void* ws,
-                        int64_t ws_bytes, hipStream_t stream) {
+static int bn_act_train_fwd_add(const float* x, int64_t n, int C, float eps, const float* gamma, const float* beta,
+                                const float* residual, int act, float momentum, float* y, float* mean, float* var, float* cnt,
+                                float* running_mean, float* running_var, long long* num_batches_tracked, const int* add_inv,
+                                const float* add_src, void* ws, int64_t ws_bytes, hipStream_t stream) {
   if (n < 1 || act < 0 || act > 2) return FC_EINVAL;
   int threads; size_t sf, sb;
   if (stats_geometry(C, &threads, &sf, &sb)) return FC_EINVAL;
@@ -1002,9 +1106,17 @@
   k_bn1_partial<<<(unsigned)nb, threads, sb, stream>>>(x, n, C, rpb, part);
   FC_CHECK_LAUNCH();
   k_bn1_apply<<<(unsigned)nb, threads, sb, stream>>>(x, n, C, rpb, part, (int)nb, eps, gamma, beta, residual, act, momentum, y,
-                                                    mean, var, cnt, running_mean, running_var, num_batches_tracked);
-  FC_CHECK_LAUNCH();
-  return FC_OK;
+                                                    mean, var, cnt, running_mean, running_var, num_batches_tracked, add_inv, add_src);
+  FC_CHECK_LAUNCH();
+  return FC_OK;
+}
+
+int fc_bn_act_train_fwd(const float* x, int64_t n, int C, float eps, const float* gamma, const float* beta,
+                        const float* residual, int act, float momentum, float* y, float* mean, float* var, float* cnt,
+                        float* running_mean, float* running_var, long long* num_batches_tracked, void* ws,
+                        int64_t ws_bytes, hipStream_t stream) {
+  return bn_act_train_fwd_add(x, n, C, eps, gamma, beta, residual, act, momentum, y, mean, var, cnt, running_mean, running_var,
+                              num_batches_tracked, nullptr, nullptr, ws, ws_bytes, stream);
 }
 
 int fc_bn_act_train_bwd(const float* x, const float* y, const float* gy, int64_t n, int C, const float* mean,
@@ -1017,7 +1129,7 @@
   int64_t nb, rpb;
   bn1_plan(n, &nb, &rpb);
   float* part = (float*)ws;
-  k_norm_bwd_partial<<<(unsigned)nb, threads, sb, stream>>>(x, y, gy, nullptr, nullptr, 0, n, C, 1, mean, var, eps, act, gamma, beta, rpb, part);
+  k_norm_bwd_partial<false><<<(unsigned)nb, threads, sb, stream>>>(x, y, gy, nullptr, nullptr, nullptr, nullptr, 0, n, C, 1, mean, var, eps, act, gamma, beta, rpb, part);
   FC_CHECK_LAUNCH();
   unsigned* ao = take_amax_out();
   k_bn1_bwd_apply<<<(unsigned)nb, threads, sb, stream>>>(x, y, gy, nullptr, n, C, rpb, part, (int)nb, mean, var, eps, gamma, beta, act, gx,
@@ -1026,16 +1138,22 @@
   return FC_OK;
 }
 
+int fc_norm_act_add_fwd(const float* x, const int* seg, int seg_stride, int64_t n, int C, const float* mean, const float* var,
+                        float eps, const float* gamma, const float* beta, const float* residual, int act, const int* add_inv,
+                        const float* add_src, float* y, hipStream_t stream) {
+  unsigned* ao = take_amax_out();
+  if (n < 0 || C < 4 || C % 4 || act < 0 || act > 2 || (add_inv == nullptr) != (add_src == nullptr)) return FC_EINVAL;
+  if (n == 0) return FC_OK;
+  k_norm_act_fwd<<<(unsigned)fc_cdiv(n * (C / 4), 256), 256, 0, stream>>>(x, seg, seg_stride, n, C, mean, var, eps, gamma,
+                                                                         beta, residual, act, add_inv, add_src, y, ao);
+  FC_CHECK_LAUNCH();
+  return FC_OK;
+}
+
 int fc_norm_act_fwd(const float* x, const int* seg, int seg_stride, int64_t n, int C, const float* mean, const float* var,
                     float eps, const float* gamma, const float* beta, const float* residual, int act, float* y,
                     hipStream_t stream) {
-  unsigned* ao = take_amax_out();
-  if (n < 0 || C < 4 || C % 4 || act < 0 || act > 2) return FC_EINVAL;
-  if (n == 0) return FC_OK;
-  k_norm_act_fwd<<<(unsigned)fc_cdiv(n * (C / 4), 256), 256, 0, stream>>>(x, seg, seg_stride, n, C, mean, var, eps, gamma,
-                                                                         beta, residual, act, y, ao);
-  FC_CHECK_LAUNCH();
-  return FC_OK;
+  return fc_norm_act_add_fwd(x, seg, seg_stride, n, C, mean, var, eps, gamma, beta, residual, act, nullptr, nullptr, y, stream);
 }
 
 int64_t fc_norm_act_bwd_ws_bytes(int64_t n, int C, int nseg) {
@@ -1060,13 +1178,13 @@
   int64_t nb, rpb;
   red_plan(n, &nb, &rpb);
   float* part = (float*)ws;
-  k_norm_bwd_partial<<<(unsigned)nb, threads, sb, stream>>>(x, y, gy, nullptr, seg, seg_stride, n, C, nseg, mean, var, eps, act, gamma,
-                                                          beta, rpb, part);
+  k_norm_bwd_partial<false><<<(unsigned)nb, threads, sb, stream>>>(x, y, gy, nullptr, nullptr, nullptr, seg, seg_stride, n, C, nseg, mean, var, eps, act,
+                                                          gamma, beta, rpb, part);
   FC_CHECK_LAUNCH();
   k_stats_final<<<(unsigned)(nseg * ((2 * C + FIN_CB - 1) / FIN_CB)), FIN_CB * FIN_SL, 0, stream>>>(part, nullptr, nb, nseg, 2 * C, 2, sums, nullptr);
   FC_CHECK_LAUNCH();
-  k_norm_bwd_apply<<<(unsigned)fc_cdiv(n * (C / 4), 256), 256, 0, stream>>>(x, y, gy, nullptr, seg, seg_stride, n, C, mean, var, eps,
-                                                                           gamma, beta, sums, cnt, act, gx, gres, ao);
+  k_norm_bwd_apply<false><<<(unsigned)fc_cdiv(n * (C / 4), 256), 256, 0, stream>>>(x, y, gy, nullptr, nullptr, nullptr, seg, seg_stride, n, C, mean,
+                                                                           var, eps, gamma, beta, sums, cnt, act, gx, gres, ao);
   FC_CHECK_LAUNCH();
   return FC_OK;
 }
@@ -1085,23 +1203,24 @@
   return a > b ? (a > c ? a : c) : (b > c ? b : c);
 }
 
-int fc_bn_train_fwd(const float* x, int64_t n, int C, float eps, const float* gamma, const float* beta, const float* residual,
-                    int act, float momentum, float* y, float* mean, float* var, float* cnt, float* running_mean,
-                    float* running_var, long long* num_batches_tracked, const float* part, int64_t nb_part, int groups,
-                    int64_t small_elems, void* ws, int64_t ws_bytes, hipStream_t stream) {
+int fc_bn_train_add_fwd(const float* x, int64_t n, int C, float eps, const float* gamma, const float* beta, const float* residual,
+                        int act, float momentum, float* y, float* mean, float* var, float* cnt, float* running_mean,
+                        float* running_var, long long* num_batches_tracked, const float* part, int64_t nb_part, int groups,
+                        int64_t small_elems, const int* add_inv, const float* add_src, void* ws, int64_t ws_bytes,
+                        hipStream_t stream) {
   unsigned* ao = take_amax_out();
-  if (n < 1 || act < 0 || act > 2) return FC_EINVAL;
+  if (n < 1 || act < 0 || act > 2 || (add_inv == nullptr) != (add_src == nullptr)) return FC_EINVAL;
   if (!part) {
     if (n * C <= small_elems) {
-      int rc = fc_bn_act_train_fwd(x, n, C, eps, gamma, beta, residual, act, momentum, y, mean, var, cnt, running_mean, running_var,
-                                   num_batches_tracked, ws, ws_bytes, stream);
+      int rc = bn_act_train_fwd_add(x, n, C, eps, gamma, beta, residual, act, momentum, y, mean, var, cnt, running_mean, running_var,
+                                    num_batches_tracked, add_inv, add_src, ws, ws_bytes, stream);
       if (rc == FC_OK && ao) rc = fc_amax(y, n * (int64_t)C, ao, stream);
       return rc;
     }
     int rc = fc_bn_stats_train(x, n, C, momentum, mean, var, cnt, running_mean, running_var, num_batches_tracked, ws, ws_bytes, stream);
     if (rc) return rc;
     t_fc_amax_out = ao;
-    return fc_norm_act_fwd(x, nullptr, 0, n, C, mean, var, eps, gamma, beta, residual, act, y, stream);
+    return fc_norm_act_add_fwd(x, nullptr, 0, n, C, mean, var, eps, gamma, beta, residual, act, add_inv, add_src, y, stream);
   }
   int threads; size_t sf, sb;
   if (stats_geometry(C, &threads, &sf, &sb)) return FC_EINVAL;
@@ -1113,7 +1232,8 @@
     if (CG != C && stats_geometry(CG, &threads, &sf, &sb)) return FC_EINVAL;
     const size_t smem = (size_t)(threads / (CG / 4)) * 2 * CG * sizeof(double);
     k_bn2_apply<<<dim3((unsigned)nb, C / CG), threads, smem, stream>>>(x, n, C, rpb, part, (int)nb_part, groups, eps, gamma, beta, residual, act,
-                                                        momentum, y, mean, var, cnt, running_mean, running_var, num_batches_tracked, CG, ao);
+                                                        momentum, y, mean, var, cnt, running_mean, running_var, num_batches_tracked, CG,
+                                                        add_inv, add_src, ao);
     FC_CHECK_LAUNCH();
     return FC_OK;
   }
@@ -1121,7 +1241,15 @@
                                                                  running_mean, running_var, num_batches_tracked);
   FC_CHECK_LAUNCH();
   t_fc_amax_out = ao;
-  return fc_norm_act_fwd(x, nullptr, 0, n, C, mean, var, eps, gamma, beta, residual, act, y, stream);
+  return fc_norm_act_add_fwd(x, nullptr, 0, n, C, mean, var, eps, gamma, beta, residual, act, add_inv, add_src, y, stream);
+}
+
+int fc_bn_train_fwd(const float* x, int64_t n, int C, float eps, const float* gamma, const float* beta, const float* residual,
+                    int act, float momentum, float* y, float* mean, float* var, float* cnt, float* running_mean,
+                    float* running_var, long long* num_batches_tracked, const float* part, int64_t nb_part, int groups,
+                    int64_t small_elems, void* ws, int64_t ws_bytes, hipStream_t stream) {
+  return fc_bn_train_add_fwd(x, n, C, eps, gamma, beta, residual, act, momentum, y, mean, var, cnt, running_mean, running_var,
+                             num_batches_tracked, part, nb_part, groups, small_elems, nullptr, nullptr, ws, ws_bytes, stream);
 }
 
 int fc_bn_train_bwd(const float* x, const float* y, const float* gy, const float* gy2, int64_t n, int C, const float* mean,
@@ -1139,7 +1267,7 @@
     if (ws_bytes < (small ? fc_bn_small_ws_bytes(C) : fc_norm_act_bwd_ws_bytes(n, C, 1))) return FC_EWS;
     int64_t rpb;
     if (small) bn1_plan(n, &np, &rpb); else red_plan(n, &np, &rpb);
-    k_norm_bwd_partial<<<(unsigned)np, threads, sb, stream>>>(x, y, gy, gy2, nullptr, 0, n, C, 1, mean, var, eps, act, gamma, beta, rpb,
+    k_norm_bwd_partial<false><<<(unsigned)np, threads, sb, stream>>>(x, y, gy, gy2, nullptr, nullptr, nullptr, 0, n, C, 1, mean, var, eps, act, gamma, beta, rpb,
                                                             (float*)ws);
     FC_CHECK_LAUNCH();
     p = (const float*)ws;
@@ -1157,8 +1285,8 @@
   }
   k_stats_final<<<(unsigned)((2 * C + FIN_CB - 1) / FIN_CB), FIN_CB * FIN_SL, 0, stream>>>(p, nullptr, np, 1, 2 * C, 2, sums, nullptr);
   FC_CHECK_LAUNCH();
-  k_norm_bwd_apply<<<(unsigned)fc_cdiv(n * (C / 4), 256), 256, 0, stream>>>(x, y, gy, gy2, nullptr, 0, n, C, mean, var, eps, gamma, beta,
-                                                                           sums, cnt, act, gx, gres, ao);
+  k_norm_bwd_apply<false><<<(unsigned)fc_cdiv(n * (C / 4), 256), 256, 0, stream>>>(x, y, gy, gy2, nullptr, nullptr, nullptr, 0, n, C, mean, var, eps, gamma,
+                                                                           beta, sums, cnt, act, gx, gres, ao);
   FC_CHECK_LAUNCH();
   return FC_OK;
 }
@@ -1204,4 +1332,53 @@
   return FC_OK;
 }
 
-}
+int fc_norm_act_maxpool8_fwd(const float* x, const int* seg, int seg_stride, int C, const float* mean, const float* var, float eps,
+                             const float* gamma, const float* beta, int act, const int* nbr, int64_t n_out, float* out,
+                             int* argrow, float* y, int* parent, hipStream_t stream) {
+  unsigned* ao = take_amax_out();
+  if (n_out < 0 || C < 4 || C % 4 || act < 0 || act > 2) return FC_EINVAL;
+  if (n_out == 0) return FC_OK;
+  k_norm_act_maxpool8_fwd<<<(unsigned)fc_cdiv(n_out * (C / 4), 256), 256, 0, stream>>>(x, seg, seg_stride, C, mean, var, eps, gamma, beta,
+                                                                                      act, nbr, n_out, out, argrow, y, parent, ao);
+  FC_CHECK_LAUNCH();
+  return FC_OK;
+}
+
+int64_t fc_maxpool8_norm_act_bwd_ws_bytes(int64_t n_in, int C, int nseg) { return fc_norm_act_bwd_ws_bytes(n_in, C, nseg); }
+
+int fc_maxpool8_norm_act_bwd(const float* x, const float* gout, const int* argrow, const int* parent, const int* seg, int seg_stride,
+                             int64_t n_in, int C, int nseg, const float* mean, const float* var, const float* cnt, float eps,
+                             const float* gamma, const float* beta, int act, float* gx, float* sums, void* ws, int64_t ws_bytes,
+                             hipStream_t stream) {
+  if (n_in < 0 || nseg < 1 || nseg > MAXSEG || act < 0 || act > 2 || !parent || !argrow) return FC_EINVAL;
+  int threads; size_t sf, sb;
+  if (stats_geometry(C, &threads, &sf, &sb)) return FC_EINVAL;
+  if (ws_bytes < fc_maxpool8_norm_act_bwd_ws_bytes(n_in, C, nseg)) return FC_EWS;
+  if (n_in == 0) {
+    FC_HIP(hipMemsetAsync(sums, 0, sizeof(float) * nseg * 2 * C, stream));
+    return FC_OK;
+  }
+  int64_t nb, rpb;
+  red_plan(n_in, &nb, &rpb);
+  float* part = (float*)ws;
+  k_norm_bwd_partial<true><<<(unsigned)nb, threads, sb, stream>>>(x, nullptr, gout, nullptr, parent, argrow, seg, seg_stride, n_in, C, nseg, mean, var,
+                                                          eps, act, gamma, beta, rpb, part);
+  FC_CHECK_LAUNCH();
+  k_stats_final<<<(unsigned)(nseg * ((2 * C + FIN_CB - 1) / FIN_CB)), FIN_CB * FIN_SL, 0, stream>>>(part, nullptr, nb, nseg, 2 * C, 2, sums, nullptr);
+  FC_CHECK_LAUNCH();
+  k_norm_bwd_apply<true><<<(unsigned)fc_cdiv(n_in * (C / 4), 256), 256, 0, stream>>>(x, nullptr, gout, nullptr, parent, argrow, seg, seg_stride, n_in, C,
+                                                                              mean, var, eps, gamma, beta, sums, cnt, act, gx, nullptr, nullptr);
+  FC_CHECK_LAUNCH();
+  return FC_OK;
+}
+
+int fc_inverse_rows(const int* rows, int64_t n, int64_t n_inv, int* inv, hipStream_t stream) {
+  if (n < 0 || n_inv < 0) return FC_EINVAL;
+  if (n_inv > 0) FC_HIP(hipMemsetAsync(inv, 0xff, sizeof(int) * n_inv, stream));
+  if (n == 0) return FC_OK;
+  k_inverse_rows<<<(unsigned)fc_cdiv(n, 256), 256, 0, stream>>>(rows, n, n_inv, inv);
+  FC_CHECK_LAUNCH();
+  return FC_OK;
+}
+
+}
diff --git a/fcaf3d_amd/executor.py b/fcaf3d_amd/executor.py
--- a/fcaf3d_amd/executor.py
+++ b/fcaf3d_amd/executor.py
@@ -15,7 +15,8 @@
 
 (OP_STEM_FWD, OP_COL_STATS, OP_NORM_FWD, OP_MAXPOOL_FWD, OP_CONV, OP_BN_FWD, OP_UNION_FWD, OP_HEAD_FWD, OP_RECORD, OP_WAIT,
  OP_HEAD_BWD, OP_WGRAD, OP_BN_BWD, OP_NORM_BWD, OP_MAXPOOL_BWD, OP_STEM_WGRAD, OP_GATHER, OP_ADD, OP_SMALL_GRADS,
- OP_PERMUTE_GENT, OP_HEAD_WFIN, OP_COPY, OP_COL_SUM, OP_ROW_SUM, OP_AMAX, OP_CLEAR) = range(1, 27)
+ OP_PERMUTE_GENT, OP_HEAD_WFIN, OP_COPY, OP_COL_SUM, OP_ROW_SUM, OP_AMAX, OP_CLEAR, OP_NORM_POOL_FWD, OP_POOL_NORM_BWD,
+ OP_INV_ROWS) = range(1, 30)
 OPW, MAPW = 24, 20
 ALIGN = 256
 S_MAIN, S_HEAD, S_WGRAD = 0, 1, 2
@@ -41,9 +42,10 @@
 
 
 class NetProgram:
-    def __init__(self, det, training, wgrad_async, head_overlap, tail0=False):
+    def __init__(self, det, training, wgrad_async, head_overlap, tail0=False, keep_state=None):
         self.det = det
         self.tail0 = tail0
+        self.keep_state = bool(KEEP_STATE if keep_state is None else keep_state)
         self.training = training
         self.wgrad_async = wgrad_async and training
         bb, nh = det.backbone, det.neck_with_head
@@ -321,7 +323,8 @@
                 tape.append((stream, bwd))
             return y
 
-        def bn(x, mod, act, rows, res=None, stream=S_MAIN):
+        def bn(x, mod, act, rows, res=None, stream=S_MAIN, add=None):
+            assert add is None or res is None
             b = mod.bn
             C = b.num_features
             y = self.T(rows, C)
@@ -340,7 +343,7 @@
                 ay = amax_of[y] = self.amax_slot()
             self.emit(F, OP_BN_FWD, stream, x, self.D(rows), C, _f(b.eps), self.S(b.weight), self.S(b.bias), -1 if res is None else res, act,
                       _f(b.momentum), y, mean, var, cnt, self.S(b.running_mean), self.S(b.running_var), self.S(b.num_batches_tracked),
-                      1 if tr else 0, prod_word, groups, ay + 1)
+                      1 if tr else 0, prod_word, groups, ay + 1, *((add[0] + 1, add[1] + 1) if add is not None else (0, 0)))
             if tr:
                 sums = torch.zeros((2, C), dtype=torch.float32, device=self.dev)
                 si = self.S(sums)
@@ -378,16 +381,17 @@
         self.emit(F, OP_STEM_FWD, S_MAIN, x0, self.S(stem.kernel), self.M('stem'), t_stem, col)
         mean_in, var_in, cnt_in = self.T('B', 64), self.T('B', 64), self.T('B', 1)
         self.emit(F, OP_COL_STATS, S_MAIN, t_stem, seg1, self.D('n1'), 64, self.D('B'), mean_in, var_in, cnt_in)
-        t_in = self.T('n1', 64)
-        self.emit(F, OP_NORM_FWD, S_MAIN, t_stem, seg1, self.D('n1'), 64, mean_in, var_in, _f(inorm.eps), self.S(inorm.weight),
-                  self.S(inorm.bias), -1, relu, t_in)
-        self.relu_outs.append((t_in, 'n1', 64))
+        t_in = self.T('n1', 64) if self.keep_state else -1
+        if self.keep_state:
+            self.relu_outs.append((t_in, 'n1', 64))
         t_pool, arg = self.T('n2', 64), self.T('n2', 64)
         self.pool_arg = (arg, 'n2', 64)
         ap = -1
         if AMAX:
             ap = amax_of[t_pool] = self.amax_slot()
-        self.emit(F, OP_MAXPOOL_FWD, S_MAIN, t_in, self.M('pool'), 64, t_pool, arg, ap + 1)
+        pool_parent = self.T('n1', 1) if tr else -1
+        self.emit(F, OP_NORM_POOL_FWD, S_MAIN, t_stem, seg1, 64, mean_in, var_in, _f(inorm.eps), self.S(inorm.weight), self.S(inorm.bias),
+                  relu, self.M('pool'), t_pool, arg, t_in, ap + 1, pool_parent)
         if tr:
             in_sums = self.T('B', 2 * 64, 'b')
             self.in_sums = in_sums
@@ -395,11 +399,9 @@
             def bwd_stem():
                 small_rows.append((None, 'B', 64, inorm.weight, inorm.bias))
                 g_pool = take(t_pool, 'n2', 64)
-                g_in = self.T('n1', 64, 'b')
-                self.emit(Bk, OP_MAXPOOL_BWD, S_MAIN, g_pool, arg, self.M('pool'), 64, g_in)
                 g_stem = self.T('n1', 64, 'b')
-                self.emit(Bk, OP_NORM_BWD, S_MAIN, t_stem, -1, g_in, seg1, self.D('n1'), 64, self.D('B'), mean_in, var_in, cnt_in,
-                          _f(inorm.eps), self.S(inorm.weight), self.S(inorm.bias), relu, g_stem, -1, in_sums)
+                self.emit(Bk, OP_POOL_NORM_BWD, S_MAIN, t_stem, g_pool, arg, pool_parent, seg1, self.D('n1'), 64, self.D('B'), mean_in,
+                          var_in, cnt_in, _f(inorm.eps), self.S(inorm.weight), self.S(inorm.bias), relu, g_stem, in_sums)
                 if self.wgrad_async:
                     self.emit(Bk, OP_RECORD, S_MAIN, EV_W0)
                     self.emit(Bk, OP_WAIT, S_WGRAD, EV_W0)
@@ -459,17 +461,14 @@
                 t = gemm(x, self.gent_w[gi], x_rows, x_C, 8 * Ci, gw_i)
                 t = bn(t, up[1], elu, g_rows)
                 t = conv(t, up[3], f'gsame{i}', g_rows, g_rows)
-                t = bn(t, up[4], elu, g_rows)
                 fb, fb_rows, fb_C = levels[i]
-                u = self.T(g_rows, Ci)
                 rows_i = self.DY(f'rows{i}')
-                self.emit(F, OP_UNION_FWD, S_MAIN, t, fb, rows_i, self.D(g_rows), self.D(fb_rows), self.D(g_rows), Ci, u)
-                if AMAX:
-                    amax_of[u] = self.amax_op(F, S_MAIN, u, g_rows, Ci)
+                inv_i = self.T(g_rows, 1)
+                self.emit(F, OP_INV_ROWS, S_MAIN, rows_i, self.D(fb_rows), self.D(g_rows), inv_i)
+                u = bn(t, up[4], elu, g_rows, add=(inv_i, fb))
                 if tr:
-                    def bwd_union(u=u, t=t, fb=fb, fb_rows=fb_rows, rows_i=rows_i, g_rows=g_rows, Ci=Ci):
+                    def bwd_union(u=u, fb=fb, fb_rows=fb_rows, rows_i=rows_i, g_rows=g_rows, Ci=Ci):
                         gu = take(u, g_rows, Ci)
-                        accumulate(t, gu, g_rows, Ci, S_MAIN)
                         gfb = self.T(fb_rows, Ci, 'b')
                         self.emit(Bk, OP_GATHER, S_MAIN, gu, rows_i, self.D(fb_rows), Ci, gfb)
                         accumulate(fb, gfb, fb_rows, Ci, S_MAIN)
@@ -692,6 +691,7 @@
             return
 
     def decisions(self, st):
+        assert self.keep_state, 'this program does not store the stem\'s normalised output: build it under executor.KEEP_STATE'
         fa, addr, dims = st['fa'], st['addr'], st['dims']
 
         def view(idx, rows, C, dtype):
@@ -886,13 +886,14 @@
     if tail0 and min(det.backbone.n_outs, 4) < 2:
         return None
     key = (bool(training), bool(Fn.WGRAD_ASYNC), bool(nh.head_overlap), bool(tail0))
+    keep = bool(KEEP_STATE)
     fuse = bool(Fn.BN_FUSE)
     mode = Fn.split_mode() if Fn.X6 else -1
     cache = det.__dict__.setdefault('_programs', {})
     sig = NetProgram.signature(det)
-    prog = cache.get(key + (fuse, mode))
+    prog = cache.get(key + (fuse, mode, keep))
     if prog is None or prog._sig != sig:
-        prog = cache[key + (fuse, mode)] = NetProgram(det, *key)
+        prog = cache[key + (fuse, mode, keep)] = NetProgram(det, *key, keep_state=keep)
     if getattr(prog.w, 'split_mode', mode) != mode:
         prog.w.fresh = False
     prog.w.split_mode = mode
diff --git a/include/fcaf3d_hip.h b/include/fcaf3d_hip.h
--- a/include/fcaf3d_hip.h
+++ b/include/fcaf3d_hip.h
@@ -10,7 +10,7 @@
 extern "C" {
 #endif
 
-#define FC_ABI_VERSION 8
+#define FC_ABI_VERSION 9
 #ifndef FC_AMAX_SLOT_BYTES
 #define FC_AMAX_SLOT_BYTES 2048
 #endif
@@ -189,6 +189,25 @@
                    hipStream_t stream);
 int fc_maxpool_bwd(const float* gout, const int* argrow, int64_t n_out, int C, float* gin, hipStream_t stream);
 
+int fc_norm_act_maxpool8_fwd(const float* x, const int* seg, int seg_stride, int C, const float* mean, const float* var, float eps,
+                             const float* gamma, const float* beta, int act, const int* nbr, int64_t n_out, float* out,
+                             int* argrow, float* y, int* parent, hipStream_t stream);
+int64_t fc_maxpool8_norm_act_bwd_ws_bytes(int64_t n_in, int C, int nseg);
+int fc_maxpool8_norm_act_bwd(const float* x, const float* gout, const int* argrow, const int* parent, const int* seg, int seg_stride,
+                             int64_t n_in, int C, int nseg, const float* mean, const float* var, const float* cnt, float eps,
+                             const float* gamma, const float* beta, int act, float* gx, float* sums, void* ws, int64_t ws_bytes,
+                             hipStream_t stream);
+
+int fc_inverse_rows(const int* rows, int64_t n, int64_t n_inv, int* inv, hipStream_t stream);
+int fc_norm_act_add_fwd(const float* x, const int* seg, int seg_stride, int64_t n, int C, const float* mean, const float* var,
+                        float eps, const float* gamma, const float* beta, const float* residual, int act, const int* add_inv,
+                        const float* add_src, float* y, hipStream_t stream);
+int fc_bn_train_add_fwd(const float* x, int64_t n, int C, float eps, const float* gamma, const float* beta, const float* residual,
+                        int act, float momentum, float* y, float* mean, float* var, float* cnt, float* running_mean,
+                        float* running_var, long long* num_batches_tracked, const float* part, int64_t nb_part, int groups,
+                        int64_t small_elems, const int* add_inv, const float* add_src, void* ws, int64_t ws_bytes,
+                        hipStream_t stream);
+
 int fc_gather_rows(const float* src, const int* idx, int64_t n, int C, float* dst, hipStream_t stream);
 int fc_scatter_rows_add(const float* src, const int* idx, int64_t n, int C, float* dst, hipStream_t stream);
 
```

New measurement: 518.7, median of 6. +1.1%, better.
